# apache/arrow

Hardware: AMD Instinct MI355X
Metric: filter_take_mrows_per_s (higher is better)
Workload: dtype int64; 1 GPU; Filter+Take int64[1000000000] + validity (10% null), boolean mask 10% true, FilterOptions::DROP; take indices = the mask's row numbers (monotonic; indices_nonzero: uint64 through CallFunction, GetTakeIndices: uint32 in the mirror), no boundscheck; inputs = splitmix64 streams of SURVEY.md 8(d) (seeds 1,2,3); rows=1000000000, selected_rows=99992053, parallelism=single-gpu

## Files before the change

arrow_amd/_lib.py:

```python
from __future__ import annotations

import ctypes as C
import os

_HERE = os.path.dirname(os.path.abspath(__file__))
LIB_PATH = os.path.join(_HERE, "libarrow_amd.so")

ARX_OK = 0
ARX_OUT_OF_MEMORY = -1
ARX_INVALID = -4
ARX_CAPACITY_ERROR = -6
ARX_INDEX_ERROR = -7
ARX_NOT_IMPLEMENTED = -10
ARX_DEVICE_ERROR = -100

ABI_VERSION = 5

FILTER_DROP, FILTER_EMIT_NULL = 0, 1
JOIN_COLUMN, JOIN_LITERAL, JOIN_NULL = 0, 1, 2
JOIN_NULL_HANDLING = {"emit_null": 0, "skip": 1, "replace": 2}
JOIN_MAX_OPERANDS = 32
SORT_ASCENDING, SORT_DESCENDING = 0, 1
NULLS_AT_START, NULLS_AT_END = 0, 1


class ArrowAmdError(Exception):
    """Base class; subclasses mirror pyarrow.lib.ArrowInvalid & friends."""


class ArrowInvalid(ArrowAmdError, ValueError):
    pass


class ArrowIndexError(ArrowAmdError, IndexError):
    pass


class ArrowCapacityError(ArrowAmdError):
    pass


class ArrowNotImplementedError(ArrowAmdError, NotImplementedError):
    pass


class ArrowDeviceError(ArrowAmdError, RuntimeError):
    pass


class ArrowMemoryError(ArrowAmdError, MemoryError):
    pass


_ERRORS = {
    ARX_INVALID: ArrowInvalid,
    ARX_CAPACITY_ERROR: ArrowCapacityError,
    ARX_INDEX_ERROR: ArrowIndexError,
    ARX_NOT_IMPLEMENTED: ArrowNotImplementedError,
    ARX_DEVICE_ERROR: ArrowDeviceError,
    ARX_OUT_OF_MEMORY: ArrowMemoryError,
}


class ArxSpan(C.Structure):

    _fields_ = [
        ("validity", C.c_void_p),
        ("data", C.c_void_p),
        ("offset", C.c_int64),
        ("length", C.c_int64),
        ("null_count", C.c_int64),
    ]


class ArxSortKeyWindow(C.Structure):

    _fields_ = [("key_min", C.c_uint64), ("shift", C.c_int32), ("reserved", C.c_int32)]


class ArxRangePlan(C.Structure):

    _fields_ = [("key_min", C.c_int32), ("width", C.c_int32), ("partitions", C.c_int32), ("reserved", C.c_int32),
                ("slots", C.c_int64), ("state_bytes", C.c_uint64), ("workspace_bytes", C.c_uint64)]


class ArxBinarySpan(C.Structure):

    _fields_ = [
        ("validity", C.c_void_p),
        ("offsets", C.c_void_p),
        ("data", C.c_void_p),
        ("offset", C.c_int64),
        ("length", C.c_int64),
        ("null_count", C.c_int64),
    ]


class ArxJoinOperand(C.Structure):

    _fields_ = [
        ("kind", C.c_int32),
        ("reserved", C.c_int32),
        ("column", ArxBinarySpan),
        ("literal", C.c_void_p),
        ("literal_length", C.c_int64),
    ]


_p, _i64, _int, _u64, _u32, _sz = C.c_void_p, C.c_int64, C.c_int, C.c_uint64, C.c_uint32, C.c_size_t
_span = C.POINTER(ArxSpan)
_bspan = C.POINTER(ArxBinarySpan)

SIGNATURES = {
    "arx_last_error": (C.c_char_p, []),
    "arx_abi_version": (_int, []),
    "arx_device_count": (_int, []),
    "arx_set_option": (_int, [C.c_char_p, _i64]),
    "arx_get_option": (_int, [C.c_char_p, C.POINTER(_i64)]),
    "arx_get_counter": (_i64, [C.c_char_p]),
    "arx_filter_workspace_bytes": (_sz, [_i64]),
    "arx_filter_count": (_int, [_span, _int, _p, _sz, C.POINTER(_i64), _p]),
    "arx_filter_count_async": (_int, [_span, _int, _p, _sz, _p]),
    "arx_filter_count_nulls": (_int, [_span, _span, _int, _p, _sz, C.POINTER(_i64), C.POINTER(_i64), _p]),
    "arx_filter_exec": (_int, [_span, _int, _span, _int, _p, _i64, _p, _p, _p]),
    "arx_mask_to_indices": (_int, [_span, _int, _p, _i64, _int, _p, _p, _p]),
    "arx_filter_compact_form": (_int, [_int, _int, _int, _int, _i64, _i64]),
    "arx_take_workspace_bytes": (_sz, []),
    "arx_check_index_bounds": (_int, [_span, _int, _u64, _p, _sz, _p]),
    "arx_take": (_int, [_span, _int, _span, _int, _p, _p, _p, _p]),
    "arx_take_rows": (_int, [_span, _i64, _span, _int, _p, _p, _p, _p]),
    "arx_take_bits": (_int, [_span, _span, _int, _p, _p, _p, _p]),
    "arx_binary_take_workspace_bytes": (_sz, [_i64]),
    "arx_binary_take_offsets": (_int, [_bspan, _span, _int, _p, _sz, _p, _p, _p, C.POINTER(_i64), _p]),
    "arx_binary_take_data": (_int, [_bspan, _i64, _p, _sz, _p, _i64, _p, _p]),
    "arx_large_binary_take_workspace_bytes": (_sz, [_i64]),
    "arx_large_binary_take_offsets": (_int, [_bspan, _span, _int, _p, _sz, _p, _p, _p, C.POINTER(_i64), _p]),
    "arx_large_binary_take_data": (_int, [_bspan, _i64, _p, _sz, _p, _i64, _p, _p]),
    "arx_list_take_data": (_int, [_bspan, _int, _i64, _p, _sz, _p, _i64, _p, _p]),
    "arx_large_list_take_data": (_int, [_bspan, _int, _i64, _p, _sz, _p, _i64, _p, _p]),
    "arx_plain_byte_array_offsets": (_int, [_p, _sz, _i64, C.c_int32, _p]),
    "arx_rle_scan_runs": (_int, [_p, _sz, _int, _i64, _u32, _u64, _p, _i64, C.POINTER(_i64), C.POINTER(_i64)]),
    "arx_rle_decode_u32": (_int, [_p, _sz, _p, _i64, _int, _i64, _p, _p]),
    "arx_rle_decode_equals_bitmap": (_int, [_p, _sz, _p, _i64, _int, _i64, _u32, _p, _p]),
    "arx_expand_by_mask": (_int, [_p, _int, _span, _p, _p, _p]),
    "arx_rle_levels_to_bitmap": (_int, [_p, _p, _i64, _p, _p, _p, _p]),
    "arx_rle_scan_runs_equals": (_int, [_p, _sz, _int, _i64, _u32, _u32, _u64, _p, _i64, C.POINTER(_i64), C.POINTER(_i64)]),
    "arx_levels_to_list_workspace_bytes": (_sz, [_i64]),
    "arx_def_rep_levels_to_list": (_int, [_p, _p, _i64, _int, _int, _int, _i64, _p, _p, _p, _p, _sz, _p]),
    "arx_levels_ge_bitmap": (_int, [_p, _i64, _u32, _p, _p, _p]),
    "arx_lz4_decompress_streams": (_int, [_p, _p, _p, _i64, _p, _p, _p]),
    "arx_lz4_frame_scan": (_int, [_p, _sz, _u64, _p, _i64, C.POINTER(_i64), C.POINTER(_u64)]),
    "arx_bitmap_copy": (_int, [_p, _i64, _i64, _p, _p]),
    "arx_buffer_copy": (_int, [_p, _p, _i64, _p]),
    "arx_delta_scan_miniblocks": (_int, [_p, _sz, _u64, _p, _i64, C.POINTER(_i64), C.POINTER(_i64), C.POINTER(_i64),
                                         C.POINTER(_i64), C.POINTER(_sz)]),
    "arx_delta_decode_workspace_bytes": (_sz, [_i64]),
    "arx_delta_decode": (_int, [_p, _p, _i64, _i64, _i64, _i64, _int, _p, _sz, _p, _p]),
    "arx_lengths_to_offsets_i32": (_int, [_p, _i64, C.c_int32, _p, _p, _sz, _p]),
    "arx_byte_stream_split_decode": (_int, [_p, _i64, _int, _p, _p]),
    "arx_delta_byte_array_lengths": (_int, [_p, _p, _i64, _p, _i64, _p, _p, _p]),
    "arx_delta_byte_array_expand": (_int, [_p, _p, _p, _i64, _p, C.c_int32, _p, _p, _i64, _p, _p, _p]),
    "arx_bitmap_copy_at": (_int, [_p, _i64, _i64, _p, _i64, _p]),
    "arx_binary_rebase_offsets": (_int, [_p, _i64, C.c_int32, _p, _p]),
    "arx_bitmap_and": (_int, [_p, _i64, _p, _i64, _i64, _p, _p]),
    "arx_reduce_i64_init": (_int, [_p, _p]),
    "arx_reduce_i64_consume": (_int, [_span, _p, _p]),
    "arx_reduce_float_minmax": (_int, [_span, _int, _p, _p]),
    "arx_coalesce2": (_int, [_int, _span, _span, _p, _i64, _p, _p, _p]),
    "arx_sum_float_workspace_bytes": (_sz, [_i64, _i64]),
    "arx_sum_float": (_int, [_span, _int, _p, _sz, C.POINTER(C.c_double), C.POINTER(_i64), _p]),
    "arx_boolean_kleene": (_int, [_int, _span, _span, _p, _p, _p]),
    "arx_boolean_invert": (_int, [_p, _i64, _i64, _p, _p]),
    "arx_bitmap_popcount": (_int, [_p, _i64, _i64, _p, _sz, C.POINTER(_i64), _p]),
    "arx_bytes_to_bitmap": (_int, [_p, _i64, _p, _p, _p]),
    "arx_groupby_key_range_i32": (_int, [_span, _p, _p]),
    "arx_groupby_range_plan": (_int, [_i64, C.c_int32, C.c_int32, _p]),
    "arx_groupby_key_range_sampled_i32": (_int, [_span, _i64, _p, _p]),
    "arx_groupby_range_sum_i64_consume": (_int, [_p, _p, _span, _span, _p, _sz, _p]),
    "arx_groupby_range_merge": (_int, [_p, _p, C.c_int32, _i64, _int, _i64, _p]),
    "arx_groupby_range_finalize_workspace_bytes": (_sz, [_i64]),
    "arx_groupby_range_finalize": (_int, [_p, C.c_int32, C.c_int32, _i64, C.c_uint32, _p, _sz, _p, _p, _p, _p, _p, _p]),
    "arx_hash_bool_finalize": (_int, [_p, _p, _p, _i64, _int, _int, C.c_uint32, _p, _p, _p, _p]),
    "arx_sort_indices_workspace_bytes": (_sz, [_i64]),
    "arx_sort_partition_records_global": (_int, [_span, _int, _int, _int, _p, _p, _int, C.c_uint32, _p, _sz, _p, _p, _p]),
    "arx_sort_records": (_int, [_p, _i64, _p, _sz, _p, _p]),
    "arx_sort_indices": (_int, [_span, _int, _int, _int, _p, _sz, _p, _p]),
    "arx_rank_workspace_bytes": (_sz, [_i64]),
    "arx_rank": (_int, [_span, _int, _p, _int, _p, _sz, _p, _p]),
    "arx_sort_indices_64": (_int, [_span, _int, _int, _int, _p, _sz, _p, _p]),
    "arx_sort_key_histogram": (_int, [_span, _int, _int, _int, _p, _p]),
    "arx_sort_partition_by_bins": (_int, [_span, _int, _int, _int, _p, _int, _p, _sz, _p, _p, _p,
                                          C.POINTER(_i64), _p]),
    "arx_bitmap_to_indices": (_int, [_p, _i64, _i64, _int, _p, _sz, _p, C.POINTER(_i64), _p]),
    "arx_sort_partition_records": (_int, [_span, _int, _int, _int, _int, _p, _int, _p, _sz, _p, _p, C.POINTER(_i64), _p]),
    "arx_sort_key_range": (_int, [_span, _int, _int, _p, _p]),
    "arx_sort_key_histogram_window": (_int, [_span, _int, _int, _int, _p, _p, _p]),
    "arx_sort_key_range_sampled": (_int, [_span, _int, _int, _int, _p, _p]),
    "arx_sort_key_histogram_window_sampled": (_int, [_span, _int, _int, _int, _p, _int, _p, _p]),
    "arx_sort_partition_records_window": (_int, [_span, _int, _int, _int, _int, _p, _p, _int, _p, _sz, _p, _p,
                                                 C.POINTER(_i64), _p]),
    "arx_sort_unpack_records": (_int, [_p, _i64, _p, _int, _int, _p, _p, _p, _p]),
    "arx_groupby_export_partitioned": (_int, [_p, _int, _p, _sz, _p, _p, _p]),
    "arx_groupby_partials_capacity": (_i64, [_i64, _i64, _int]),
    "arx_groupby_sum_i64_consume_partials": (_int, [_p, _i64, _span, _span, _p, _sz, _int, _p, _i64, _p, _p]),
    "arx_groupby_partition_rows": (_int, [_span, _span, _int, _p, _sz, _p, _p, _p]),
    "arx_groupby_unpack_rows": (_int, [_p, _i64, _p, _p, _p, _p, _p]),
    "arx_hash_sum_consume_workspace_bytes": (_sz, [_i64, _i64]),
    "arx_hash_sum_i64_consume_ws": (_int, [_span, _int, _i64, _p, _i64, _i64, _p, _p, _p, _p, _sz, _p]),
    "arx_hash_mean_i64_finalize": (_int, [_p, _p, _i64, C.c_uint64, _p, _p, _p]),
    "arx_compare_numeric": (_int, [_int, _int, _p, _p, _p, _p, _i64, _p, _p]),
    "arx_arith_numeric": (_int, [_int, _int, _int, _p, _p, _p, _i64, _p, _p, _p, _i64, _i64, _p, _p, _p]),
    "arx_divide_numeric": (_int, [_int, _int, _p, _p, _p, _i64, _p, _p, _p, _i64, _i64, _p, _p, _p]),
    "arx_unary_numeric": (_int, [_int, _int, _int, _span, _p, _p, _p]),
    "arx_round_numeric": (_int, [_int, _int, _int, _span, _i64, _p, _p, _p, _p]),
    "arx_round_status": (_int, [_int, _int, _int, _span, _i64, _p, _p, _p]),
    "arx_delta_decode_pages": (_int, [_p, _p, _p, _i64, _i64, _int, _p, _sz, _p, _p]),
    "arx_copy_segments": (_int, [_p, _i64, _u64, _p]),
    "arx_bitmap_copy_segments": (_int, [_p, _i64, _i64, _p]),
    "arx_take_columns": (_int, [_p, _p, _int, _span, _int, _p, _p, _p, _p]),
    "arx_grouper_state_bytes": (_sz, [_i64]),
    "arx_grouper_init": (_int, [_p, _i64, _p]),
    "arx_grouper_consume_workspace_bytes": (_sz, [_i64]),
    "arx_grouper_consume": (_int, [_p, _i64, _p, _p, _int, _p, _sz, _p, _p]),
    "arx_grouper_lookup": (_int, [_p, _i64, _p, _p, _int, _p, _sz, _p, _p, _p]),
    "arx_grouper_num_groups": (_int, [_p, _p, _p]),
    "arx_group_ids_skip_group": (_int, [_p, _i64, _u32, _p]),
    "arx_grouper_get_uniques": (_int, [_p, _i64, _p, _int, _int, _p, _p, _p, _p]),
    "arx_binary_key_lengths": (_int, [_bspan, _p, _p, _p, _p]),
    "arx_binary_key_chunk": (_int, [_bspan, _i64, _p, _p, _p]),
    "arx_binary_sort_chunk": (_int, [_bspan, _i64, _p, _p]),
    "arx_binary_key_hash": (_int, [_bspan, _int, _p, _p]),
    "arx_set_lookup_state_bytes": (_sz, [_i64, _int]),
    "arx_set_lookup_build": (_int, [_p, _span, _int, _p]),
    "arx_set_lookup_build_binary": (_int, [_p, _bspan, _int, _int, _p]),
    "arx_set_lookup_is_in": (_int, [_p, _i64, _int, _span, _int, _p, _p]),
    "arx_set_lookup_index_in": (_int, [_p, _i64, _int, _span, _int, _p, _p, _p]),
    "arx_set_lookup_is_in_binary": (_int, [_p, _bspan, _int, _int, _bspan, _int, _int, _p, _p]),
    "arx_set_lookup_index_in_binary": (_int, [_p, _bspan, _int, _int, _bspan, _int, _int, _p, _p, _p]),
    "arx_match_substring": (_int, [_bspan, _int, _int, _p, _i64, _i64, _int, _p, _p]),
    "arx_string_length": (_int, [_bspan, _int, _int, _i64, _int, _p, _p]),
    "arx_string_slice_workspace_bytes": (_sz, [_i64, _int]),
    "arx_string_slice_offsets": (_int, [_bspan, _int, _int, _i64, _i64, _i64, _int, _p, _sz, _p, C.POINTER(_i64), _p]),
    "arx_string_slice_data": (_int, [_bspan, _int, _p, _sz, _p, _i64, _p, _p]),
    "arx_string_trim_offsets": (_int, [_bspan, _int, _int, _int, _p, _i64, _p, _sz, _p, C.POINTER(_i64), _p]),
    "arx_replace_substring_workspace_bytes": (_sz, [_i64, _int]),
    "arx_replace_substring_offsets": (_int, [_bspan, _int, _p, _i64, _i64, _i64, _i64, _int, _p, _sz, _p, C.POINTER(_i64), _p]),
    "arx_replace_substring_data": (_int, [_bspan, _int, _p, _i64, _p, _i64, _i64, _int, _p, _sz, _p, _i64, _p, _p]),
    "arx_binary_join_workspace_bytes": (_sz, [_i64, _int]),
    "arx_binary_join_offsets": (_int, [C.POINTER(ArxJoinOperand), _int, _i64, _int, _int, _i64, _p, _sz, _p, _p, C.POINTER(_i64),
                                       C.POINTER(_i64), _p]),
    "arx_binary_join_data": (_int, [C.POINTER(ArxJoinOperand), _int, _i64, _int, _int, _p, _i64, _p, _i64, _p, _p]),
    "arx_compare_binary": (_int, [_int, _bspan, _bspan, _int, _p, _i64, _i64, _int, _p, _p]),
    "arx_if_else": (_int, [_int, _span, _span, _p, _span, _p, _i64, _p, _p, _p]),
    "arx_temporal_component": (_int, [_int, _int, _span, _i64, _int, _int, _p, _p, _p]),
    "arx_hash_join_workspace_bytes": (_sz, [_i64]),
    "arx_hash_join_key_validity": (_int, [_span, _int, _i64, _p, _p]),
    "arx_hash_join_bool_key": (_int, [_span, _p, _p]),
    "arx_hash_join_group_offsets": (_int, [_p, _p, _i64, _i64, _p, _p, _sz, _p]),
    "arx_hash_join_probe_count": (_int, [_p, _p, _i64, _p, _i64, _int, _p, _i64, _p, _p, _sz, C.POINTER(_i64), _p]),
    "arx_hash_join_expand": (_int, [_p, _p, _p, _i64, _p, _p, _int, _i64, _p, _p, _p, _p]),
    "arx_hash_join_build_mask": (_int, [_p, _p, _i64, _p, _int, _p, _p]),
    "arx_hash_join_append_build_rows": (_int, [_p, _i64, _i64, _p, _p, _p, _p, _p]),
    "arx_hash_join_filter_count": (_int, [_span, _p, _p, _i64, _int, _p, _p, _i64, _p, _p, _p, _p, _sz, C.POINTER(_i64), _p]),
    "arx_hash_join_filter_compact": (_int, [_p, _p, _i64, _p, _p, _i64, _p, _p, _int, _i64, _p, _p, _p, _p]),
    "arx_hash_join_flags_to_mask": (_int, [_p, _i64, _int, _p, _p]),
    "arx_binary_key_verify": (_int, [_bspan, _p, _p, C.POINTER(_i64), _p, _p]),
    "arx_group_first_rows": (_int, [_p, _i64, _i64, _p, _p]),
    "arx_group_edge_rows": (_int, [_p, _p, _i64, _i64, _i64, _int, _p, _p, _p]),
    "arx_ree_bool_expand": (_int, [_p, _int, _i64, _span, _i64, _i64, _p, _p, _p]),
    "arx_snappy_decompress_pages": (_int, [_p, _p, _i64, _p, _p, _p]),
    "arx_gzip_decompress_pages": (_int, [_p, _p, _i64, _p, _p, _p]),
    "arx_cast_numeric": (_int, [_span, _int, _int, _int, _int, _p, _sz, _p, _p]),
    "arx_groupby_mean_i64_finalize": (_int, [_p, _p, _p, _p, _p, _i64, _int, _u32, _p, _p, _p, _p]),
    "arx_groupby_sum_i64_merge_records": (_int, [_p, _i64, _p, _i64, _p]),
    "arx_groupby_state_bytes": (_sz, [_i64]),
    "arx_groupby_init": (_int, [_p, _i64, _p]),
# ... 78 lines not shown
```

arrow_amd/csrc/plugin/common.inc:

```

std::atomic<int64_t> g_gpu_calls{0};
std::atomic<int64_t> g_stock_calls{0};
std::atomic<int64_t> g_min_rows{1 << 16};
std::atomic<int64_t> g_min_rows_streaming{INT64_MAX};
std::atomic<int64_t> g_filter_morsel_rows{[] {
  const char* env = std::getenv("ARROW_AMD_FILTER_MORSEL_ROWS");
  return env != nullptr ? static_cast<int64_t>(std::strtoll(env, nullptr, 10)) : int64_t(1) << 20;
}()};

std::atomic<bool> g_parquet_pinned_staging{true};
std::atomic<bool> g_parquet_device_levels{true};
std::atomic<int> g_parquet_read_threads{4};
std::atomic<int64_t> g_parquet_read_part_bytes{int64_t(1) << 23};
std::atomic<bool> g_parquet_device_snappy{[] {
  const char* env = std::getenv("ARROW_AMD_PARQUET_DEVICE_SNAPPY");
  return env == nullptr || std::strtoll(env, nullptr, 10) != 0;
}()};
std::atomic<int64_t> g_parquet_device_snappy_pages{0};
std::atomic<bool> g_parquet_device_gzip{true};
std::atomic<int64_t> g_parquet_device_gzip_pages{0};
std::atomic<int64_t> g_parquet_copied_pages{0};

std::atomic<int64_t> g_aggregate_flush_rows{[] {
  const char* env = std::getenv("ARROW_AMD_AGGREGATE_FLUSH_ROWS");
// ... 6 lines not shown
std::atomic<int64_t> g_aggregate_range_sample_rows{int64_t(1) << 20};
std::atomic<int64_t> g_aggregate_range_plans{0};
std::atomic<int64_t> g_aggregate_range_declined{0};
std::atomic<int64_t> g_select_k_min_rows{int64_t(1) << 22};
std::atomic<int64_t> g_select_k_threshold_runs{0};
std::atomic<bool> g_sharded_range_state{true};
std::atomic<int64_t> g_sharded_range_min_rows{int64_t(1) << 22};
std::atomic<int64_t> g_sharded_range_runs{0};
std::atomic<int64_t> g_sharded_range_declined{0};
std::atomic<bool> g_sharded_sort_records{true};
std::atomic<int> g_sharded_sort_sample_shift{4};
std::atomic<int64_t> g_sharded_sort_sample_min_rows{int64_t(1) << 20};
std::atomic<int64_t> g_sharded_sort_records_runs{0};
std::atomic<int64_t> g_coalesce_rows{int64_t(1) << 26};
std::atomic<int64_t> g_coalesced_batches{0};
std::atomic<int64_t> g_table_source_rows{int64_t(1) << 27};
std::atomic<bool> g_pinned_results{[] {
  const char* env = std::getenv("ARROW_AMD_PINNED_RESULTS");
  return env == nullptr || std::strtoll(env, nullptr, 10) != 0;
}()};
std::atomic<bool> g_results_kernel_copy{true};
std::atomic<bool> g_aggregate_device_output{false};
std::atomic<bool> g_aggregate_stage_nulls{true};
std::atomic<int64_t> g_aggregate_flushes{0};
std::atomic<int64_t> g_string_key_hash_bits{64};
std::atomic<int64_t> g_string_key_hash_collisions{0};

enum Fn { kFnFilter = 0, kFnTake, kFnGreater, kFnSort, kFnCast, kFnHashSum, kFnAdd, kFnBoolean, kFnCompare, kFnParquet,
          kFnReduce, kFnOrderBy, kFnTakeColumns, kFnUnique, kFnCoalesce, kFnIsIn, kFnIndexIn, kFnHashJoin,
          kFnMatchSubstring, kFnStartsWith, kFnEndsWith, kFnIfElse, kFnYear, kFnQuarter, kFnMonth, kFnDay, kFnDayOfWeek,
          kFnDayOfYear, kFnIsoYear, kFnIsoWeek, kFnHour, kFnMinute, kFnSecond, kFnMillisecond, kFnMicrosecond, kFnNanosecond,
          kFnBinaryLength, kFnUtf8Length, kFnBinarySlice, kFnUtf8SliceCodeunits, kFnAsciiTrimWhitespace, kFnAsciiLtrimWhitespace,
          kFnAsciiRtrimWhitespace, kFnUtf8TrimWhitespace, kFnUtf8LtrimWhitespace, kFnUtf8RtrimWhitespace, kFnAsciiTrim, kFnAsciiLtrim,
          kFnAsciiRtrim, kFnUtf8Trim, kFnUtf8Ltrim, kFnUtf8Rtrim, kFnCompareString, kFnReplaceSubstring, kFnUnaryArith, kFnRound,
          kFnBinaryJoinElementWise,
          kNumFn };
const char* const kFnNames[kNumFn] = {"array_filter", "array_take", "greater", "array_sort_indices",
                                      "cast", "hash_sum", "add", "boolean", "compare", "parquet", "reduce", "order_by",
                                      "take_columns", "unique", "coalesce", "is_in", "index_in", "hashjoin",
                                      "match_substring", "starts_with", "ends_with", "if_else", "year", "quarter", "month", "day",
                                      "day_of_week", "day_of_year", "iso_year", "iso_week", "hour", "minute", "second",
                                      "millisecond", "microsecond", "nanosecond", "binary_length", "utf8_length", "binary_slice",
                                      "utf8_slice_codeunits", "ascii_trim_whitespace", "ascii_ltrim_whitespace",
                                      "ascii_rtrim_whitespace", "utf8_trim_whitespace", "utf8_ltrim_whitespace",
                                      "utf8_rtrim_whitespace", "ascii_trim", "ascii_ltrim", "ascii_rtrim", "utf8_trim", "utf8_ltrim",
                                      "utf8_rtrim", "compare_string", "replace_substring", "unary_arith", "round",
                                      "binary_join_element_wise"};
std::atomic<int64_t> g_fn_gpu[kNumFn];
std::atomic<int64_t> g_fn_stock[kNumFn];
void CountGpu(Fn f) {
  g_gpu_calls.fetch_add(1, std::memory_order_relaxed);
  g_fn_gpu[f].fetch_add(1, std::memory_order_relaxed);
}
void CountStock(Fn f) {
  g_stock_calls.fetch_add(1, std::memory_order_relaxed);
  g_fn_stock[f].fetch_add(1, std::memory_order_relaxed);
}
thread_local std::string t_error;

Status FromArx(int rc) {
  if (rc == ARX_OK) return Status::OK();
  const std::string msg = arx_last_error();
  switch (rc) {
    case ARX_INVALID: return Status::Invalid(msg);
    case ARX_CAPACITY_ERROR: return Status::CapacityError(msg);
    case ARX_INDEX_ERROR: return Status::IndexError(msg);
    case ARX_NOT_IMPLEMENTED: return Status::NotImplemented(msg);
    case ARX_OUT_OF_MEMORY: return Status::OutOfMemory(msg);
    default: return Status::UnknownError(msg);
  }
}

#define HIP_RETURN_NOT_OK(call)                                                        \
  do {                                                                                 \
    hipError_t e__ = (call);                                                           \
    if (e__ != hipSuccess)                                                             \
      return Status::IOError("HIP: ", hipGetErrorString(e__), " in " #call);           \
  } while (0)

thread_local hipStream_t t_stream = nullptr;

class DeviceScratch {
 public:
  ~DeviceScratch() {
    for (auto& s : slots_) {
      if (s.ptr) (void)hipFree(s.ptr);
    }
  }
  hipStream_t PeekStream() const { return stream_; }
  Status Stream(hipStream_t* out) {
    if (!stream_) {
      HIP_RETURN_NOT_OK(hipStreamCreateWithFlags(&stream_, hipStreamNonBlocking));
      t_stream = stream_;
    }
    *out = stream_;
    return Status::OK();
  }
  Status Get(int slot, size_t bytes, void** out) {
    if (slots_.size() <= static_cast<size_t>(slot)) slots_.resize(slot + 1);
    Slot& s = slots_[slot];
    bytes = (bytes + 255) & ~size_t(255);
    if (s.size < bytes) {
      if (s.ptr) HIP_RETURN_NOT_OK(hipFree(s.ptr));
      s.ptr = nullptr;
      s.size = 0;
      const size_t want = std::max<size_t>(bytes + bytes / 4, 1 << 20);
      HIP_RETURN_NOT_OK(hipMalloc(&s.ptr, want));
      s.size = want;
    }
    *out = s.ptr;
    return Status::OK();
  }

 private:
  struct Slot { void* ptr = nullptr; size_t size = 0; };
  std::vector<Slot> slots_;
  hipStream_t stream_ = nullptr;
};
thread_local DeviceScratch t_scratch;

class PinnedStaging {
 public:
  ~PinnedStaging() {
    if (ptr_) (void)hipHostFree(ptr_);
  }
  Status Reserve(size_t bytes, uint8_t** out) {
    if (size_ < bytes) {
      if (ptr_) HIP_RETURN_NOT_OK(hipHostFree(ptr_));
      ptr_ = nullptr;
      size_ = 0;
      const size_t want = std::max<size_t>(bytes + bytes / 4, size_t(1) << 20);
      HIP_RETURN_NOT_OK(hipHostMalloc(&ptr_, want, hipHostMallocDefault));
      size_ = want;
    }
    *out = static_cast<uint8_t*>(ptr_);
    return Status::OK();
  }
  void Trim(size_t keep_at_most) {
    if (size_ > keep_at_most && ptr_ != nullptr) {
      (void)hipHostFree(ptr_);
      ptr_ = nullptr;
      size_ = 0;
    }
  }

 private:
  void* ptr_ = nullptr;
  size_t size_ = 0;
};
thread_local PinnedStaging t_pinned;

enum Slot { kValues = 0, kValidity, kArg2, kArg2Validity, kOutData, kOutValidity, kWs, kCounter, kBinWs, kFlag };

Status Upload(const ArraySpan& a, int byte_width_or_0_for_bool, int data_slot, int validity_slot,
              hipStream_t st, ArxSpan* out) {
  const int64_t o8 = a.offset % 8;
  const int64_t first = a.offset - o8;
  out->offset = o8;
  out->length = a.length;
  out->null_count = a.null_count;
  out->validity = nullptr;
  out->data = nullptr;
  const int64_t span_elems = o8 + a.length;
  if (a.buffers[1].data != nullptr && a.length > 0) {
    const uint8_t* src;
    size_t bytes;
    if (byte_width_or_0_for_bool == 0) {
      src = a.buffers[1].data + first / 8;
      bytes = static_cast<size_t>(arrow::bit_util::BytesForBits(span_elems));
    } else {
      src = a.buffers[1].data + first * byte_width_or_0_for_bool;
      bytes = static_cast<size_t>(span_elems) * byte_width_or_0_for_bool;
    }
    void* d = nullptr;
    ARROW_RETURN_NOT_OK(t_scratch.Get(data_slot, bytes + 16, &d));
    HIP_RETURN_NOT_OK(hipMemcpyAsync(d, src, bytes, hipMemcpyHostToDevice, st));
    out->data = d;
  }
  if (a.buffers[0].data != nullptr && a.null_count != 0 && a.length > 0) {
    const size_t bytes = static_cast<size_t>(arrow::bit_util::BytesForBits(span_elems));
    void* d = nullptr;
    ARROW_RETURN_NOT_OK(t_scratch.Get(validity_slot, bytes + 16, &d));
    HIP_RETURN_NOT_OK(hipMemcpyAsync(d, a.buffers[0].data + first / 8, bytes, hipMemcpyHostToDevice, st));
    out->validity = d;
  } else if (a.null_count != 0 && a.buffers[0].data == nullptr) {
    out->null_count = 0;
  }
  return Status::OK();
}

bool IsHost(const ArraySpan& a) {
  for (int i = 0; i < 2; ++i) {
    if (a.buffers[i].owner != nullptr && *a.buffers[i].owner != nullptr &&
        !(*a.buffers[i].owner)->is_cpu()) {
      return false;
    }
  }
  return true;
}

int FixedByteWidth(const arrow::DataType& t) {
  switch (t.id()) {
    case Type::INT8: case Type::UINT8: return 1;
    case Type::INT16: case Type::UINT16: case Type::HALF_FLOAT: return 2;
    case Type::INT32: case Type::UINT32: case Type::FLOAT: case Type::DATE32: case Type::TIME32:
    case Type::INTERVAL_MONTHS: case Type::DECIMAL32: return 4;
    case Type::INT64: case Type::UINT64: case Type::DOUBLE: case Type::DATE64: case Type::TIME64:
    case Type::TIMESTAMP: case Type::DURATION: case Type::INTERVAL_DAY_TIME: case Type::DECIMAL64: return 8;
    case Type::DECIMAL128: case Type::INTERVAL_MONTH_DAY_NANO: return 16;
    case Type::DECIMAL256: return 32;
    case Type::FIXED_SIZE_BINARY: {
      const int w = static_cast<const arrow::FixedSizeBinaryType&>(t).byte_width();
      return (w == 1 || w == 2 || w == 4 || w == 8 || w == 16 || w == 32) ? w : 0;
    }
    default: return 0;
  }
}

int BinaryOffsetWidth(Type::type id) { return (id == Type::LARGE_STRING || id == Type::LARGE_BINARY) ? 8 : 4; }

template <typename Options>
struct ShimState : public cp::KernelState {
  std::unique_ptr<cp::KernelState> stock;
  Options options;
};

struct StockKernel {
  cp::KernelInit init;
  cp::ArrayKernelExec exec = nullptr;
  cp::VectorKernel::ChunkedExec exec_chunked = nullptr;
};

template <class Exec, class Batch, class Out>
Status RunStock(Fn fn, Exec exec, std::optional<cp::KernelState*> stock_state, cp::KernelContext* ctx, const Batch& batch,
                Out* out) {
  CountStock(fn);
  if (!stock_state.has_value()) return exec(ctx, batch, out);
  cp::KernelState* mine = ctx->state();
  ctx->SetState(*stock_state);
  Status st = exec(ctx, batch, out);
  ctx->SetState(mine);
  return st;
}
Status RunStock(Fn fn, const StockKernel& k, cp::KernelState* stock_state, cp::KernelContext* ctx,
                const cp::ExecSpan& batch, cp::ExecResult* out) {
  return RunStock(fn, k.exec, std::optional<cp::KernelState*>(stock_state), ctx, batch, out);
}
```

arrow_amd/csrc/plugin/parquet.inc:

```

class RunTable {
 public:
  const ArxRleRun* data() const { return runs_.get(); }
  ArxRleRun* data() { return runs_.get(); }
  size_t size() const { return size_; }
  void clear() { size_ = 0; }
  void push_back(const ArxRleRun& r) {
    Reserve(size_ + 1);
    runs_[size_++] = r;
  }
  void Reserve(size_t n) {
    if (n <= cap_) return;
    const size_t cap = std::max(n, cap_ + cap_ / 2);
    std::unique_ptr<ArxRleRun[]> grown(new ArxRleRun[cap]);
    if (size_ > 0) std::memcpy(grown.get(), runs_.get(), size_ * sizeof(ArxRleRun));
    runs_ = std::move(grown);
    cap_ = cap;
  }
  void SetSize(size_t n) { size_ = n; }

 private:
  std::unique_ptr<ArxRleRun[]> runs_;
  size_t size_ = 0, cap_ = 0;
};
// ... 63 lines not shown
                      int64_t prefix_len, uint8_t* out) {
  if (prefix_len > 0) std::memcpy(out, prefix, static_cast<size_t>(prefix_len));
  ARROW_ASSIGN_OR_RAISE(const int64_t got, codec->Decompress(n, src, len, out + prefix_len));
  if (got != len) return Status::IOError("Corrupt snappy compressed data.");
  return Status::OK();
}

Status PrefetchBodies(const std::vector<std::shared_ptr<parquet::Page>>& pages, int max_def, PrefetchedBodies* out,
                      const uint8_t** arena_out, size_t* arena_bytes_out) {
  const arrow::Compression::type raw_codec = t_raw_codec;
  *arena_out = nullptr;
  *arena_bytes_out = 0;
  struct Job { const uint8_t* src; int64_t n, want, len; const uint8_t* prefix; int64_t prefix_len; size_t at; };
  std::vector<Job> jobs;
  size_t arena_bytes = 0;
  int64_t packed_bytes = 0;
  auto add = [&](const uint8_t* src, int64_t n, int64_t want, const uint8_t* prefix, int64_t prefix_len) {
    if (src == nullptr || n <= 0) return;
    PrefetchedBody& e = (*out)[src];
    e.src_len = n;
    e.want_len = want;
    e.prefix_len = prefix_len;
    auto len = SnappyBodyLength(src, n, want, raw_codec);
    if (!len.ok()) {
      e.status = len.status();
      return;
    }
    jobs.push_back(Job{src, n, want, *len, prefix, prefix_len, arena_bytes});
    arena_bytes += (static_cast<size_t>(prefix_len + *len) + 63) & ~size_t(63);
    packed_bytes += n;
  };
  for (const auto& page : pages) {
    if (page->type() == parquet::PageType::DICTIONARY_PAGE) {
      const auto& dp = static_cast<const parquet::DictionaryPage&>(*page);
      add(dp.data(), dp.size(), -1, nullptr, 0);
    } else if (page->type() == parquet::PageType::DATA_PAGE) {
      const auto& dp = static_cast<const parquet::DataPage&>(*page);
      if (!(max_def == 0 && dp.encoding() == parquet::Encoding::PLAIN)) add(dp.data(), dp.size(), dp.uncompressed_size(), nullptr, 0);
    } else if (page->type() == parquet::PageType::DATA_PAGE_V2) {
      const auto& v2 = static_cast<const parquet::DataPageV2&>(*page);
      const int64_t lev = static_cast<int64_t>(v2.definition_levels_byte_length()) + v2.repetition_levels_byte_length();
      if (lev < 0 || lev > v2.size() || lev > v2.uncompressed_size()) continue;
      if (v2.is_compressed() && v2.size() - lev > 0 && v2.encoding() != parquet::Encoding::PLAIN) {
        add(v2.data() + lev, v2.size() - lev, v2.uncompressed_size() - lev, v2.data(), lev);
      }
    }
  }
  if (jobs.empty()) return Status::OK();
  uint8_t* arena = nullptr;
  std::shared_ptr<std::vector<uint8_t>> pageable;
  if (g_parquet_pinned_staging.load()) {
    ARROW_RETURN_NOT_OK(t_pinned_bodies.Reserve(arena_bytes + 64, &arena));
  } else {
    thread_local std::vector<uint8_t> t_pageable_bodies;
    if (t_pageable_bodies.size() < arena_bytes + 64) t_pageable_bodies.resize(arena_bytes + arena_bytes / 4 + 64);
    arena = t_pageable_bodies.data();
  }
  const int threads = static_cast<int>(std::max<int64_t>(
      1, std::min<int64_t>({static_cast<int64_t>(g_parquet_read_threads.load()), static_cast<int64_t>(jobs.size()),
                            packed_bytes / std::max<int64_t>(1, g_parquet_read_part_bytes.load() / 8) + 1})));
  std::vector<Status> job_status(jobs.size());
  std::atomic<size_t> next{0};
  auto work = [&]() {
    auto codec = arrow::util::Codec::Create(raw_codec);
    for (size_t j = next.fetch_add(1); j < jobs.size(); j = next.fetch_add(1)) {
      const Job& job = jobs[j];
      job_status[j] = codec.ok() ? SnappyBodyInto(codec->get(), job.src, job.n, job.len, job.prefix, job.prefix_len, arena + job.at)
                                 : codec.status();
    }
  };
  std::vector<std::thread> helpers;
  for (int t = 1; t < threads; ++t) helpers.emplace_back(work);
  work();
  for (auto& t : helpers) t.join();
  *arena_out = arena;
  *arena_bytes_out = arena_bytes;
  for (size_t j = 0; j < jobs.size(); ++j) {
    PrefetchedBody& e = (*out)[jobs[j].src];
    e.status = job_status[j];
    e.body = HostBody{arena + jobs[j].at, jobs[j].prefix_len + jobs[j].len, pageable};
  }
  return Status::OK();
}

class UploadArena {
 public:
  ~UploadArena() {
    if (ptr_) (void)hipHostFree(ptr_);
  }
  struct Scope {
    explicit Scope(UploadArena* a) : arena(a) { arena->Begin(); }
    ~Scope() {
      if (hipStream_t st = t_scratch.PeekStream()) (void)hipStreamSynchronize(st);
      arena->active_ = false;
      t_pinned.Trim(size_t(1) << 30);
      t_pinned_bodies.Trim(size_t(1) << 30);
    }
    UploadArena* arena;
  };
  const void* Stage(const void* src, size_t nbytes) {
    if (!active_ || nbytes < (size_t(1) << 16)) return src;
    const size_t need = (nbytes + 63) & ~size_t(63);
    wanted_ += need;
    if (used_ + need > size_) return src;
    uint8_t* dst = static_cast<uint8_t*>(ptr_) + used_;
    std::memcpy(dst, src, nbytes);
    used_ += need;
    return dst;
  }

 private:
  void Begin() {
    if (wanted_ > size_ && g_parquet_pinned_staging.load()) {
      if (ptr_) (void)hipHostFree(ptr_);
      ptr_ = nullptr;
      size_ = 0;
      const size_t want = wanted_ + wanted_ / 4;
      if (hipHostMalloc(&ptr_, want, hipHostMallocDefault) == hipSuccess) size_ = want; else ptr_ = nullptr;
    }
    used_ = 0;
    wanted_ = 0;
    active_ = g_parquet_pinned_staging.load();
  }
  void* ptr_ = nullptr;
  size_t size_ = 0, used_ = 0, wanted_ = size_t(8) << 20;
  bool active_ = false;
};
thread_local UploadArena t_upload;

arrow::Result<std::shared_ptr<Buffer>> ToDevice(const void* host, size_t nbytes, hipStream_t st) {
  ARROW_ASSIGN_OR_RAISE(auto buf, AllocDevice(static_cast<int64_t>(nbytes)));
  if (nbytes > 0) {
    HIP_RETURN_NOT_OK(hipMemcpyAsync(reinterpret_cast<void*>(buf->mutable_address()), t_upload.Stage(host, nbytes), nbytes,
                                     hipMemcpyHostToDevice, st));
  }
  return buf;
}

Status ParquetValidity(const ParquetStream& levels, int max_def, int64_t rows, int64_t dense, hipStream_t st,
                       std::shared_ptr<Buffer>* validity, ArxSpan* mask, void** ws, std::shared_ptr<Buffer> keep[2]) {
  ARROW_ASSIGN_OR_RAISE(keep[0], ToDevice(levels.bytes.data(), levels.bytes.size(), st));
  ARROW_ASSIGN_OR_RAISE(keep[1], ToDevice(levels.runs.data(), levels.runs.size() * sizeof(ArxRleRun), st));
  ARROW_ASSIGN_OR_RAISE(*validity, AllocDevice(((rows + 63) / 64) * 8));
  void* d_valid = reinterpret_cast<void*>((*validity)->mutable_address());
  ARROW_RETURN_NOT_OK(FromArx(arx_rle_decode_equals_bitmap(reinterpret_cast<const void*>(keep[0]->address()),
                                                           levels.bytes.size(),
                                                           reinterpret_cast<const ArxRleRun*>(keep[1]->address()),
                                                           static_cast<int64_t>(levels.runs.size()), 1, rows,
                                                           static_cast<uint32_t>(max_def), d_valid, st)));
  *mask = ArxSpan{nullptr, d_valid, 0, rows, 0};
  const size_t ws_bytes = arx_filter_workspace_bytes(rows);
  ARROW_RETURN_NOT_OK(t_scratch.Get(kBinWs, ws_bytes, ws));
  int64_t counted = 0;
  ARROW_RETURN_NOT_OK(FromArx(arx_filter_count(mask, ARX_FILTER_DROP, *ws, ws_bytes, &counted, st)));
  if (counted != dense) return Status::Invalid("Parquet: ", counted, " non-null levels but ", dense, " values");
  return Status::OK();
}

struct ByteArrayPage {
  std::vector<uint8_t> bytes;
  int64_t count;
  bool delta_length;
  bool delta_byte_array = false;
};

Status DecodeInt32DeltaStreams(const std::vector<const uint8_t*>& bytes, const std::vector<size_t>& sizes,
                               const std::vector<int64_t>& expect, const char* what, int32_t* d_out, std::vector<size_t>* used,
                               hipStream_t st) {
  std::vector<uint8_t> all;
  std::vector<ArxDeltaMiniblock> mbs;
  std::vector<ArxDeltaPage> table(bytes.size());
  used->assign(bytes.size(), 0);
  int64_t start = 0, tiles = 0;
  for (size_t j = 0; j < bytes.size(); ++j) {
    int64_t nmb = 0, vpm = 0, total = 0, first_value = 0;
    size_t u = 0;
    ARROW_RETURN_NOT_OK(FromArx(arx_delta_scan_miniblocks(bytes[j], sizes[j], all.size(), nullptr, 0, &nmb, &vpm, &total, &first_value, &u)));
    if (total != expect[j]) return Status::Invalid("Parquet: DELTA_BYTE_ARRAY page holds ", total, " ", what, ", its header says ", expect[j]);
    const size_t at = mbs.size();
    mbs.resize(at + static_cast<size_t>(nmb));
    ARROW_RETURN_NOT_OK(FromArx(arx_delta_scan_miniblocks(bytes[j], sizes[j], all.size(), mbs.data() + at, nmb, &nmb, &vpm, &total,
                                                          &first_value, nullptr)));
    table[j] = ArxDeltaPage{start, static_cast<int64_t>(at), std::max<int64_t>(vpm, 1), first_value, total, tiles};
    all.insert(all.end(), bytes[j], bytes[j] + u);
    all.resize((all.size() + 7) & ~size_t(7), 0);
    (*used)[j] = u;
    start += total;
    tiles += (total + 4095) / 4096;
  }
  if (start == 0) return Status::OK();
  all.resize(all.size() + 16, 0);
  if (mbs.empty()) mbs.push_back(ArxDeltaMiniblock{});
  ARROW_ASSIGN_OR_RAISE(auto d_all, ToDevice(all.data(), all.size(), st));
  ARROW_ASSIGN_OR_RAISE(auto d_mbs, ToDevice(mbs.data(), mbs.size() * sizeof(ArxDeltaMiniblock), st));
  ARROW_ASSIGN_OR_RAISE(auto d_table, ToDevice(table.data(), table.size() * sizeof(ArxDeltaPage), st));
  const size_t ws_bytes = arx_delta_decode_workspace_bytes(std::max<int64_t>(tiles, 1) * 4096);
  void* ws = nullptr;
  ARROW_RETURN_NOT_OK(t_scratch.Get(kWs, ws_bytes, &ws));
  ARROW_RETURN_NOT_OK(FromArx(arx_delta_decode_pages(reinterpret_cast<const void*>(d_all->address()),
                                                     reinterpret_cast<const ArxDeltaMiniblock*>(d_mbs->address()),
                                                     reinterpret_cast<const ArxDeltaPage*>(d_table->address()),
                                                     static_cast<int64_t>(table.size()), tiles, 4, ws, ws_bytes, d_out, st)));
  HIP_RETURN_NOT_OK(hipStreamSynchronize(st));
  return Status::OK();
}

arrow::Result<std::shared_ptr<ArrayData>> ParquetBitsOrBytesToDevice(
    const std::shared_ptr<arrow::DataType>& type, bool is_bool, int max_def, int64_t rows, int64_t dense,
    int64_t dense_from_dict, const std::vector<uint8_t>& dict, int64_t dict_count, const ParquetStream& levels,
    const ParquetStream& indices, const ParquetStream& bools,
    const std::vector<ByteArrayPage>& plain_ba, hipStream_t st) {
  std::shared_ptr<Buffer> keep[12];
  std::vector<std::shared_ptr<Buffer>> keep_more;
  std::vector<uint32_t> page_entries;
  ArxSpan bool_src{};
  ArxBinarySpan bin_src{};
  if (is_bool) {
    ARROW_ASSIGN_OR_RAISE(keep[0], AllocDevice(((std::max<int64_t>(dense, 1) + 63) / 64) * 8));
    if (dense > 0) {
      ARROW_ASSIGN_OR_RAISE(keep[1], ToDevice(bools.bytes.data(), bools.bytes.size(), st));
      ARROW_ASSIGN_OR_RAISE(keep[2], ToDevice(bools.runs.data(), bools.runs.size() * sizeof(ArxRleRun), st));
      ARROW_RETURN_NOT_OK(FromArx(arx_rle_decode_equals_bitmap(
          reinterpret_cast<const void*>(keep[1]->address()), bools.bytes.size(),
          reinterpret_cast<const ArxRleRun*>(keep[2]->address()), static_cast<int64_t>(bools.runs.size()), 1, dense, 1u,
          reinterpret_cast<void*>(keep[0]->mutable_address()), st)));
    }
    bool_src = ArxSpan{nullptr, reinterpret_cast<const void*>(keep[0]->address()), 0, dense, 0};
  } else {
    std::vector<int32_t> offs(1, 0);
    std::vector<uint8_t> data;
    size_t pos = 0;
    for (int64_t i = 0; i < dict_count; ++i) {
      if (pos + 4 > dict.size()) return Status::Invalid("Parquet: byte-array dictionary entry runs past the page");
      const uint32_t len = arrow::util::SafeLoadAs<uint32_t>(dict.data() + pos);
      if (len > dict.size() - pos - 4) return Status::Invalid("Parquet: byte-array dictionary entry runs past the page");
      data.insert(data.end(), dict.begin() + pos + 4, dict.begin() + pos + 4 + len);
      pos += 4 + len;
      offs.push_back(static_cast<int32_t>(data.size()));
    }
    struct DeltaLengthFixup { size_t entry; int32_t base; const ByteArrayPage* page; size_t header_bytes; };
    std::vector<DeltaLengthFixup> fixups;
    std::vector<const ByteArrayPage*> dba_pages;
    int64_t dba_total = 0;
    constexpr uint32_t kDbaMark = 0x80000000u;
    for (const auto& page : plain_ba) {
      const int32_t base = static_cast<int32_t>(data.size());
      const size_t first = offs.size() - 1;
      if (page.delta_byte_array) {
        if (page.count == 0) continue;
        for (int64_t j = 0; j < page.count; ++j) page_entries.push_back(kDbaMark | static_cast<uint32_t>(dba_total + j));
        dba_pages.push_back(&page);
        dba_total += page.count;
        continue;
      }
      if (!page.delta_length) {
        offs.resize(first + 2 * page.count + 1);
        ARROW_RETURN_NOT_OK(FromArx(arx_plain_byte_array_offsets(page.bytes.data(), page.bytes.size(), page.count, base,
                                                                 offs.data() + first)));
        data.insert(data.end(), page.bytes.begin(), page.bytes.begin() + (offs.back() - base));
        for (int64_t j = 0; j < page.count; ++j) page_entries.push_back(static_cast<uint32_t>(first + 1 + 2 * j));
        continue;
      }
      if (page.count == 0) continue;
      int64_t nmb = 0, vpm = 0, total = 0, first_value = 0;
      size_t header_bytes = 0;
      ARROW_RETURN_NOT_OK(FromArx(arx_delta_scan_miniblocks(page.bytes.data(), page.bytes.size(), 0, nullptr, 0, &nmb, &vpm,
                                                            &total, &first_value, &header_bytes)));
      if (total != page.count) {
        return Status::Invalid("Parquet: DELTA_LENGTH_BYTE_ARRAY page holds ", total, " lengths, its header says ", page.count);
      }
      if (data.size() + (page.bytes.size() - header_bytes) > static_cast<size_t>(INT32_MAX)) {
        return Status::Invalid("Parquet: column chunk exceeds the int32 offset range");
      }
      fixups.push_back(DeltaLengthFixup{first, base, &page, header_bytes});
      offs.resize(first + page.count + 1, 0);
      data.insert(data.end(), page.bytes.begin() + header_bytes, page.bytes.end());
      offs.back() = static_cast<int32_t>(data.size());
      for (int64_t j = 0; j < page.count; ++j) page_entries.push_back(static_cast<uint32_t>(first + j));
    }
    const size_t host_entries = offs.size() - 1;
    if (dba_total > 0) {
      if (host_entries + static_cast<size_t>(dba_total) >= kDbaMark) return Status::Invalid("Parquet: too many byte-array values in one chunk");
      for (auto& e : page_entries) {
        if (e & kDbaMark) e = static_cast<uint32_t>(host_entries) + (e & ~kDbaMark);
      }
      offs.resize(host_entries + dba_total + 1, static_cast<int32_t>(data.size()));
    }
    ARROW_ASSIGN_OR_RAISE(keep[0], ToDevice(offs.data(), offs.size() * 4, st));
    if (dba_total == 0) {
      ARROW_ASSIGN_OR_RAISE(keep[1], ToDevice(data.data(), data.size(), st));
    } else {
      const int64_t npages = static_cast<int64_t>(dba_pages.size());
      ARROW_ASSIGN_OR_RAISE(auto d_prefix, AllocDevice(dba_total * 4));
      ARROW_ASSIGN_OR_RAISE(auto d_slen, AllocDevice(dba_total * 4));
      std::vector<int64_t> firsts(1, 0), suffix_firsts(1, 0);
      std::vector<uint8_t> suffix;
      {
        std::vector<const uint8_t*> heads, rests;
        std::vector<size_t> head_sizes, rest_sizes, used, sused;
        std::vector<int64_t> counts;
        for (const ByteArrayPage* page : dba_pages) {
          heads.push_back(page->bytes.data());
          head_sizes.push_back(page->bytes.size());
          counts.push_back(page->count);
        }
        ARROW_RETURN_NOT_OK(DecodeInt32DeltaStreams(heads, head_sizes, counts, "prefix lengths",
                                                    reinterpret_cast<int32_t*>(d_prefix->mutable_address()), &used, st));
// ... 609 lines not shown
                  std::to_string(prefetch_misses) + " | ";
  }
  std::shared_ptr<Buffer> dense_buf = dense_early;
  if (!raw) {
    ARROW_ASSIGN_OR_RAISE(dense_buf, AllocDevice(dense * width));
  }
  if (raw && dense > cc->num_values()) return Status::Invalid("Parquet: more values in the pages than the chunk announces");
  uint8_t* d_dense = reinterpret_cast<uint8_t*>(dense_buf->mutable_address());
  std::shared_ptr<Buffer> keep[8];
  std::shared_ptr<Buffer> keep_snappy[3];
  std::shared_ptr<Buffer> keep_segs;
  if (!plain_segs.empty()) {
    ARROW_ASSIGN_OR_RAISE(keep_segs, ToDevice(plain_segs.data(), plain_segs.size() * sizeof(ArxCopySeg), st));
    ARROW_RETURN_NOT_OK(FromArx(arx_copy_segments(reinterpret_cast<const ArxCopySeg*>(keep_segs->address()),
                                                  static_cast<int64_t>(plain_segs.size()), plain_seg_max, st)));
  }
  if (!snappy_pages.empty()) {
    if (raw_plain_values != dense - dense_from_dict || !delta_pages.empty() || !split_pages.empty()) {
      return Status::NotImplemented("arrow_amd: PLAIN and DELTA_BINARY_PACKED / BYTE_STREAM_SPLIT pages in one column chunk");
    }
    std::memset(snappy_src + snappy_len, 0, 8);
    if (chunk_dev) {
      keep_snappy[0] = chunk_dev;
      if (snappy_len > chunk_bytes + 8) {
        HIP_RETURN_NOT_OK(hipMemcpyAsync(reinterpret_cast<uint8_t*>(chunk_dev->mutable_address()) + chunk_bytes + 8,
                                         snappy_src + chunk_bytes + 8, snappy_len - chunk_bytes, hipMemcpyHostToDevice, st));
      }
    } else {
      ARROW_ASSIGN_OR_RAISE(keep_snappy[0], ToDevice(snappy_src, snappy_len + 8, st));
    }
    ARROW_ASSIGN_OR_RAISE(keep_snappy[1], ToDevice(snappy_pages.data(), snappy_pages.size() * sizeof(ArxSnappyPage), st));
    ARROW_ASSIGN_OR_RAISE(keep_snappy[2], AllocDevice(static_cast<int64_t>(snappy_pages.size()) * 4));
    ARROW_RETURN_NOT_OK(FromArx((gzip_chunk ? arx_gzip_decompress_pages : arx_snappy_decompress_pages)(
        reinterpret_cast<const void*>(keep_snappy[0]->address()), reinterpret_cast<const ArxSnappyPage*>(keep_snappy[1]->address()),
        static_cast<int64_t>(snappy_pages.size()), d_dense, reinterpret_cast<uint32_t*>(keep_snappy[2]->mutable_address()), st)));
    std::vector<uint32_t> status(snappy_pages.size());
    HIP_RETURN_NOT_OK(hipMemcpyAsync(status.data(), reinterpret_cast<const void*>(keep_snappy[2]->address()), status.size() * 4,
                                     hipMemcpyDeviceToHost, st));
    HIP_RETURN_NOT_OK(hipStreamSynchronize(st));
    for (uint32_t code : status) {
      if (code != 0 && gzip_chunk) {
        return Status::IOError("zlib inflate failed: invalid deflate stream (device decoder status ", code, ")");
      }
      if (code != 0) return Status::IOError("Corrupt snappy compressed data.");
    }
    (gzip_chunk ? g_parquet_device_gzip_pages : g_parquet_device_snappy_pages).fetch_add(static_cast<int64_t>(snappy_pages.size()));
  }
  if (dense_from_dict > 0) {
    ARROW_ASSIGN_OR_RAISE(keep[0], ToDevice(indices.bytes.data(), indices.bytes.size(), st));
    ARROW_ASSIGN_OR_RAISE(keep[1], ToDevice(indices.runs.data(), indices.runs.size() * sizeof(ArxRleRun), st));
    ARROW_ASSIGN_OR_RAISE(keep[2], ToDevice(dict.data(), static_cast<size_t>(dict_count) * width, st));
    ARROW_ASSIGN_OR_RAISE(keep[3], AllocDevice(dense_from_dict * 4));
    uint32_t* d_idx = reinterpret_cast<uint32_t*>(keep[3]->mutable_address());
    ARROW_RETURN_NOT_OK(FromArx(arx_rle_decode_u32(reinterpret_cast<const void*>(keep[0]->address()), indices.bytes.size(),
                                                   reinterpret_cast<const ArxRleRun*>(keep[1]->address()),
                                                   static_cast<int64_t>(indices.runs.size()), 0, dense_from_dict, d_idx, st)));
    ArxSpan dv{nullptr, reinterpret_cast<const void*>(keep[2]->address()), 0, dict_count, 0};
    ArxSpan di{nullptr, d_idx, 0, dense_from_dict, 0};
    void* bws = nullptr;
    ARROW_RETURN_NOT_OK(t_scratch.Get(kWs, arx_take_workspace_bytes(), &bws));
    ARROW_RETURN_NOT_OK(FromArx(arx_check_index_bounds(&di, ARX_UINT32, static_cast<uint64_t>(dict_count), bws,
                                                       arx_take_workspace_bytes(), st)));
    ARROW_RETURN_NOT_OK(FromArx(arx_take(&dv, width, &di, ARX_UINT32, d_dense, nullptr, nullptr, st)));
  }
  std::shared_ptr<Buffer> keep_split;
  if (!split_pages.empty()) {
    ARROW_ASSIGN_OR_RAISE(keep_split, ToDevice(split_bytes.data(), split_bytes.size(), st));
    for (const auto& sp : split_pages) {
      ARROW_RETURN_NOT_OK(FromArx(arx_byte_stream_split_decode(
          reinterpret_cast<const uint8_t*>(keep_split->address()) + sp.byte_start, sp.count, width,
          d_dense + sp.dense_start * width, st)));
    }
  }
  if (!plain.empty()) {
    if (!delta_pages.empty() || !split_pages.empty()) {
      return Status::NotImplemented("arrow_amd: PLAIN and DELTA_BINARY_PACKED / BYTE_STREAM_SPLIT pages in one column chunk");
    }
    HIP_RETURN_NOT_OK(hipMemcpyAsync(d_dense + dense_from_dict * width, plain.data(), plain.size(), hipMemcpyHostToDevice, st));
  }
  if (!delta_pages.empty()) {
    delta_bytes.resize(delta_bytes.size() + 16, 0);
    if (delta_mbs.empty()) delta_mbs.push_back(ArxDeltaMiniblock{});
    ARROW_ASSIGN_OR_RAISE(keep[6], ToDevice(delta_bytes.data(), delta_bytes.size(), st));
    ARROW_ASSIGN_OR_RAISE(keep[7], ToDevice(delta_mbs.data(), delta_mbs.size() * sizeof(ArxDeltaMiniblock), st));
    std::vector<ArxDeltaPage> table(delta_pages.size());
    int64_t tiles = 0;
    for (size_t j = 0; j < delta_pages.size(); ++j) {
      const auto& dp = delta_pages[j];
      table[j] = ArxDeltaPage{dp.dense_start, dp.first_mb, std::max<int64_t>(dp.per_miniblock, 1), dp.first_value, dp.count, tiles};
      tiles += (dp.count + 4095) / 4096;
    }
    std::shared_ptr<Buffer> keep_pages;
    ARROW_ASSIGN_OR_RAISE(keep_pages, ToDevice(table.data(), table.size() * sizeof(ArxDeltaPage), st));
    const size_t ws_bytes = arx_delta_decode_workspace_bytes(std::max<int64_t>(tiles, 1) * 4096);
    void* ws = nullptr;
    ARROW_RETURN_NOT_OK(t_scratch.Get(kWs, ws_bytes, &ws));
    ARROW_RETURN_NOT_OK(FromArx(arx_delta_decode_pages(
        reinterpret_cast<const void*>(keep[6]->address()), reinterpret_cast<const ArxDeltaMiniblock*>(keep[7]->address()),
        reinterpret_cast<const ArxDeltaPage*>(keep_pages->address()), static_cast<int64_t>(table.size()), tiles, width, ws,
        ws_bytes, d_dense, st)));
    HIP_RETURN_NOT_OK(hipStreamSynchronize(st));
  }
  std::shared_ptr<Buffer> validity, values = dense_buf;
  int64_t null_count = 0;
  if (levels_on_device && !level_pages.empty()) {
    if (!chunk_dev) {
      ARROW_ASSIGN_OR_RAISE(chunk_dev, AllocDevice(static_cast<int64_t>(chunk_bytes) + 8));
      HIP_RETURN_NOT_OK(hipMemcpyAsync(reinterpret_cast<void*>(chunk_dev->mutable_address()), snappy_src, chunk_bytes + 8,
                                       hipMemcpyHostToDevice, st));
    }
    const size_t np = level_pages.size();
    ARROW_ASSIGN_OR_RAISE(validity, AllocDevice(((rows + 63) / 64) * 8 + 8));
    HIP_RETURN_NOT_OK(hipMemsetAsync(reinterpret_cast<void*>(validity->mutable_address()), 0,
                                     static_cast<size_t>((rows + 63) / 64) * 8 + 8, st));
    ARROW_ASSIGN_OR_RAISE(keep[4], ToDevice(level_pages.data(), np * sizeof(ArxLevelPage), st));
    ARROW_ASSIGN_OR_RAISE(keep[5], AllocDevice(static_cast<int64_t>(np) * 8));
    uint32_t* d_ones = reinterpret_cast<uint32_t*>(keep[5]->mutable_address());
    ARROW_RETURN_NOT_OK(FromArx(arx_rle_levels_to_bitmap(reinterpret_cast<const void*>(chunk_dev->address()),
                                                         reinterpret_cast<const ArxLevelPage*>(keep[4]->address()),
                                                         static_cast<int64_t>(np),
                                                         reinterpret_cast<void*>(validity->mutable_address()), d_ones,
                                                         d_ones + np, st)));
    std::vector<uint32_t> back(2 * np);
    HIP_RETURN_NOT_OK(hipMemcpyAsync(back.data(), d_ones, 2 * np * 4, hipMemcpyDeviceToHost, st));
    HIP_RETURN_NOT_OK(hipStreamSynchronize(st));
    for (size_t i = 0; i < np; ++i) {
      if (back[np + i] != 0) return Status::Invalid("Parquet: RLE block ended before all its values (corrupt data page?)");
      if (back[i] != level_valid[i]) {
        return Status::Invalid("Parquet: ", back[i], " non-null levels in a page whose header announces ", level_valid[i]);
      }
    }
    if (dense == rows) validity = nullptr;
  }
  if (max_def > 0 && dense < rows) {
    void* d_valid = nullptr;
    if (levels_on_device) {
      d_valid = reinterpret_cast<void*>(validity->mutable_address());
    } else {
      ARROW_ASSIGN_OR_RAISE(keep[4], ToDevice(levels.bytes.data(), levels.bytes.size(), st));
      ARROW_ASSIGN_OR_RAISE(keep[5], ToDevice(levels.runs.data(), levels.runs.size() * sizeof(ArxRleRun), st));
      ARROW_ASSIGN_OR_RAISE(validity, AllocDevice(((rows + 63) / 64) * 8));
      d_valid = reinterpret_cast<void*>(validity->mutable_address());
      ARROW_RETURN_NOT_OK(FromArx(arx_rle_decode_equals_bitmap(reinterpret_cast<const void*>(keep[4]->address()),
                                                               levels.bytes.size(),
                                                               reinterpret_cast<const ArxRleRun*>(keep[5]->address()),
                                                               static_cast<int64_t>(levels.runs.size()), 1, rows,
                                                               static_cast<uint32_t>(max_def), d_valid, st)));
    }
    ArxSpan mask{nullptr, d_valid, 0, rows, 0};
    const size_t ws_bytes = arx_filter_workspace_bytes(rows);
    void* ws = nullptr;
    ARROW_RETURN_NOT_OK(t_scratch.Get(kBinWs, ws_bytes, &ws));
    int64_t counted = 0;
    ARROW_RETURN_NOT_OK(FromArx(arx_filter_count(&mask, ARX_FILTER_DROP, ws, ws_bytes, &counted, st)));
    if (counted != dense) return Status::Invalid("Parquet: ", counted, " non-null levels but ", dense, " values");
    ARROW_ASSIGN_OR_RAISE(values, AllocDevice(rows * width));
    ARROW_RETURN_NOT_OK(FromArx(arx_expand_by_mask(d_dense, width, &mask, ws,
                                                   reinterpret_cast<void*>(values->mutable_address()), st)));
    null_count = rows - dense;
  }
  HIP_RETURN_NOT_OK(hipStreamSynchronize(st));
  trace.Lap("uploads + device decode");
  CountGpu(kFnParquet);
  return ArrayData::Make(std::move(type), rows, {std::move(validity), std::move(values)}, null_count);
}
```

arrow_amd/csrc/plugin/selection.inc:

```
StockKernel g_stock_filter;

arrow::Result<std::unique_ptr<cp::KernelState>> FilterInit(cp::KernelContext* ctx,
                                                           const cp::KernelInitArgs& args) {
  auto state = std::make_unique<ShimState<cp::FilterOptions>>();
  if (g_stock_filter.init) {
    ARROW_ASSIGN_OR_RAISE(state->stock, g_stock_filter.init(ctx, args));
  }
  if (args.options != nullptr) {
    state->options = *static_cast<const cp::FilterOptions*>(args.options);
  }
  return state;
}

Status BooleanTakeOnDevice(const ArxSpan& dv, const ArxSpan& di, int tid, hipStream_t st, ArrayData* out_arr) {
  const int64_t m = di.length;
  const int64_t bytes = ((m + 63) / 64) * 8;
  const bool allocate_validity = dv.null_count != 0 || di.null_count != 0;
  out_arr->length = m;
  out_arr->buffers.resize(2);
  out_arr->buffers[0] = nullptr;
  ARROW_ASSIGN_OR_RAISE(out_arr->buffers[1], AllocDevice(bytes));
  void* d_valid = nullptr;
  void* d_counter = nullptr;
  if (allocate_validity) {
    ARROW_ASSIGN_OR_RAISE(out_arr->buffers[0], AllocDevice(bytes));
    d_valid = reinterpret_cast<void*>(out_arr->buffers[0]->mutable_address());
    ARROW_RETURN_NOT_OK(t_scratch.Get(kCounter, 64, &d_counter));
    HIP_RETURN_NOT_OK(hipMemsetAsync(d_counter, 0, 8, st));
  }
  ARROW_RETURN_NOT_OK(FromArx(arx_take_bits(&dv, &di, tid, reinterpret_cast<void*>(out_arr->buffers[1]->mutable_address()),
                                            d_valid, static_cast<int64_t*>(d_counter), st)));
  int64_t valid_count = m;
  if (allocate_validity) HIP_RETURN_NOT_OK(hipMemcpyAsync(&valid_count, d_counter, 8, hipMemcpyDeviceToHost, st));
  HIP_RETURN_NOT_OK(hipStreamSynchronize(st));
  out_arr->null_count = m - valid_count;
  return Status::OK();
}

bool ReeFilterOnRocm(const ArraySpan& filter) {
  return filter.type->id() == Type::RUN_END_ENCODED && filter.child_data.size() == 2 &&
         OnRocm(filter.child_data[0]) && OnRocm(filter.child_data[1]);
}
Status ExpandReeFilterOnDevice(const ArraySpan& filter, hipStream_t st, ArxSpan* dm) {
  const ArraySpan& run_ends = filter.child_data[0];
  const ArraySpan& run_values = filter.child_data[1];
  const int rw = FixedByteWidth(*run_ends.type);
  if (run_values.type->id() != Type::BOOL || (rw != 2 && rw != 4 && rw != 8)) {
    return Status::NotImplemented("arrow_amd: filter of type ", filter.type->ToString());
  }
  ArxSpan ends{}, vals{};
  ARROW_RETURN_NOT_OK(DeviceSpan(run_ends, &ends));
  ARROW_RETURN_NOT_OK(DeviceSpan(run_values, &vals));
  const int64_t n = filter.length;
  const size_t bytes = static_cast<size_t>((n + 63) / 64) * 8 + 64;
  void *d_bits = nullptr, *d_valid = nullptr;
  ARROW_RETURN_NOT_OK(t_scratch.Get(kArg2, bytes, &d_bits));
  const bool may_have_nulls = vals.validity != nullptr && vals.null_count != 0;
  if (may_have_nulls) ARROW_RETURN_NOT_OK(t_scratch.Get(kArg2Validity, bytes, &d_valid));
  ARROW_RETURN_NOT_OK(FromArx(arx_ree_bool_expand(static_cast<const uint8_t*>(ends.data) + ends.offset * rw, rw, run_ends.length,
                                                  &vals, filter.offset, n, d_bits, d_valid, st)));
  *dm = ArxSpan{d_valid, d_bits, 0, n, may_have_nulls ? arrow::kUnknownNullCount : 0};
  return Status::OK();
}

Status FilterExec(cp::KernelContext* ctx, const cp::ExecSpan& batch, cp::ExecResult* out) {
  auto* state = static_cast<ShimState<cp::FilterOptions>*>(ctx->state());
  const ArraySpan& values = batch[0].array;
  const ArraySpan& filter = batch[1].array;
  const int w = FixedByteWidth(*values.type);
  const int null_sel = state->options.null_selection_behavior == cp::FilterOptions::EMIT_NULL
                           ? ARX_FILTER_EMIT_NULL : ARX_FILTER_DROP;
  const bool ree = filter.type->id() == Type::RUN_END_ENCODED;
  const bool on_device = OnRocm(values) || OnRocm(filter) || (ree && ReeFilterOnRocm(filter));
  if (on_device && ree && (!OnRocm(values) || !ReeFilterOnRocm(filter))) {
    return Status::NotImplemented("arrow_amd: a run-end encoded filter and its values must both be device-resident");
  }
  if (on_device) {
    if (values.type->id() == Type::BOOL && ree) {
      return Status::NotImplemented("arrow_amd: run-end encoded filter of boolean values on device-resident arrays");
    }
    if (values.type->id() == Type::BOOL && filter.type->id() == Type::BOOL) {
      if (filter.length > 0xFFFFFFFFll) {
        return Status::NotImplemented("Filter length exceeds UINT32_MAX, consider a different strategy for selecting elements");
      }
      hipStream_t st;
      ARROW_RETURN_NOT_OK(t_scratch.Stream(&st));
      ArxSpan dv{}, dm{};
      ARROW_RETURN_NOT_OK(DeviceSpan(values, &dv));
      ARROW_RETURN_NOT_OK(DeviceSpan(filter, &dm));
      const size_t ws_bytes = arx_filter_workspace_bytes(filter.length);
      void* ws = nullptr;
      ARROW_RETURN_NOT_OK(t_scratch.Get(kWs, ws_bytes, &ws));
      int64_t out_len = 0;
      ARROW_RETURN_NOT_OK(FromArx(arx_filter_count(&dm, null_sel, ws, ws_bytes, &out_len, st)));
      const bool emit = null_sel == ARX_FILTER_EMIT_NULL && dm.null_count != 0;
      void* d_idx = nullptr;
      void* d_idx_valid = nullptr;
      ARROW_RETURN_NOT_OK(t_scratch.Get(kArg2, static_cast<size_t>(out_len) * 4 + 64, &d_idx));
      if (emit) ARROW_RETURN_NOT_OK(t_scratch.Get(kArg2Validity, static_cast<size_t>((out_len + 63) / 64) * 8 + 64, &d_idx_valid));
      ARROW_RETURN_NOT_OK(FromArx(arx_mask_to_indices(&dm, null_sel, ws, out_len, 4, d_idx, d_idx_valid, st)));
      ArxSpan di{d_idx_valid, d_idx, 0, out_len, emit ? arrow::kUnknownNullCount : 0};
      ARROW_RETURN_NOT_OK(BooleanTakeOnDevice(dv, di, ARX_UINT32, st, out->array_data().get()));
      CountGpu(kFnFilter);
      return Status::OK();
    }
    if (w == 0 || (filter.type->id() != Type::BOOL && !ree)) {
      return Status::NotImplemented("arrow_amd: filter of ", values.type->ToString(),
                                    " on device-resident arrays");
    }
    hipStream_t st;
    ARROW_RETURN_NOT_OK(t_scratch.Stream(&st));
    ArxSpan dv{}, dm{};
    ARROW_RETURN_NOT_OK(DeviceSpan(values, &dv));
    if (ree) {
      ARROW_RETURN_NOT_OK(ExpandReeFilterOnDevice(filter, st, &dm));
    } else {
      ARROW_RETURN_NOT_OK(DeviceSpan(filter, &dm));
    }
    const size_t ws_bytes = arx_filter_workspace_bytes(filter.length);
    void* ws = nullptr;
    ARROW_RETURN_NOT_OK(t_scratch.Get(kWs, ws_bytes, &ws));
    ArrayData* out_arr = out->array_data().get();
    const bool allocate_validity = dv.null_count != 0 || dm.null_count != 0;
    if (filter.length > 0 && filter.length <= g_filter_morsel_rows.load()) {
      const int64_t n = filter.length;
      ARROW_RETURN_NOT_OK(FromArx(arx_filter_count_async(&dm, null_sel, ws, ws_bytes, st)));
      out_arr->buffers.resize(2);
      ARROW_ASSIGN_OR_RAISE(out_arr->buffers[1], AllocDevice(n * w));
      out_arr->buffers[0] = nullptr;
      void* d_valid = nullptr;
      if (allocate_validity) {
        ARROW_ASSIGN_OR_RAISE(out_arr->buffers[0], AllocDevice(((n + 63) / 64) * 8));
        d_valid = reinterpret_cast<void*>(out_arr->buffers[0]->mutable_address());
      }
      ARROW_RETURN_NOT_OK(FromArx(arx_filter_exec(&dv, w, &dm, null_sel, ws, n,
                                                  reinterpret_cast<void*>(out_arr->buffers[1]->mutable_address()),
                                                  d_valid, st)));
      int64_t selected = 0, set_bits = 0;
      HIP_RETURN_NOT_OK(hipMemcpyAsync(&selected, ws, 8, hipMemcpyDeviceToHost, st));
      if (allocate_validity) {
        void* cws = nullptr;
        ARROW_RETURN_NOT_OK(t_scratch.Get(kCounter, 64, &cws));
        ARROW_RETURN_NOT_OK(FromArx(arx_bitmap_popcount(d_valid, 0, n, cws, 64, &set_bits, st)));
      } else {
        HIP_RETURN_NOT_OK(hipStreamSynchronize(st));
      }
      out_arr->length = selected;
      out_arr->null_count = allocate_validity ? selected - set_bits : 0;
      static_cast<RocmBuffer*>(out_arr->buffers[1].get())->Shrink(selected * w);
      if (allocate_validity) static_cast<RocmBuffer*>(out_arr->buffers[0].get())->Shrink(((selected + 63) / 64) * 8);
      CountGpu(kFnFilter);
      return Status::OK();
    }
    int64_t out_len = 0, out_nulls = 0;
    if (allocate_validity) {
      ARROW_RETURN_NOT_OK(FromArx(arx_filter_count_nulls(&dv, &dm, null_sel, ws, ws_bytes, &out_len, &out_nulls, st)));
    } else {
      ARROW_RETURN_NOT_OK(FromArx(arx_filter_count(&dm, null_sel, ws, ws_bytes, &out_len, st)));
    }
    out_arr->length = out_len;
    out_arr->buffers.resize(2);
    ARROW_ASSIGN_OR_RAISE(out_arr->buffers[1], AllocDevice(out_len * w));
    out_arr->buffers[0] = nullptr;
    void* d_valid = nullptr;
    if (allocate_validity) {
      ARROW_ASSIGN_OR_RAISE(out_arr->buffers[0], AllocDevice(((out_len + 63) / 64) * 8));
      d_valid = reinterpret_cast<void*>(out_arr->buffers[0]->mutable_address());
    }
    ARROW_RETURN_NOT_OK(FromArx(arx_filter_exec(&dv, w, &dm, null_sel, ws, out_len,
                                                reinterpret_cast<void*>(out_arr->buffers[1]->mutable_address()),
                                                d_valid, st)));
    out_arr->null_count = allocate_validity ? out_nulls : 0;
    HIP_RETURN_NOT_OK(hipStreamSynchronize(st));
    CountGpu(kFnFilter);
    return Status::OK();
  }
  if (w == 0 || filter.type->id() != Type::BOOL || values.length < g_min_rows.load() ||
      !IsHost(values) || !IsHost(filter)) {
    return RunStock(kFnFilter, g_stock_filter, state->stock.get(), ctx, batch, out);
  }
  hipStream_t st;
  ARROW_RETURN_NOT_OK(t_scratch.Stream(&st));
  ArxSpan dv{}, dm{};
  ARROW_RETURN_NOT_OK(Upload(values, w, kValues, kValidity, st, &dv));
  ARROW_RETURN_NOT_OK(Upload(filter, 0, kArg2, kArg2Validity, st, &dm));
  const size_t ws_bytes = arx_filter_workspace_bytes(filter.length);
  void* ws = nullptr;
  ARROW_RETURN_NOT_OK(t_scratch.Get(kWs, ws_bytes, &ws));
  int64_t out_len = 0;
  ARROW_RETURN_NOT_OK(FromArx(arx_filter_count(&dm, null_sel, ws, ws_bytes, &out_len, st)));

  ArrayData* out_arr = out->array_data().get();
  const bool filter_null_count_is_zero = filter.null_count == 0;
  if (values.null_count == 0 && (null_sel == ARX_FILTER_DROP || filter_null_count_is_zero)) {
    out_arr->null_count = 0;
  } else {
    out_arr->null_count = arrow::kUnknownNullCount;
  }
  const bool allocate_validity = values.null_count != 0 || !filter_null_count_is_zero;
  out_arr->length = out_len;
  out_arr->buffers.resize(2);
  ARROW_ASSIGN_OR_RAISE(out_arr->buffers[1], ctx->Allocate(out_len * w));
  void* d_out = nullptr;
  void* d_out_valid = nullptr;
  ARROW_RETURN_NOT_OK(t_scratch.Get(kOutData, static_cast<size_t>(out_len) * w + 16, &d_out));
  const size_t vbytes = static_cast<size_t>((out_len + 63) / 64) * 8;
  if (allocate_validity) {
    ARROW_ASSIGN_OR_RAISE(out_arr->buffers[0], ctx->AllocateBitmap(out_len));
    ARROW_RETURN_NOT_OK(t_scratch.Get(kOutValidity, vbytes + 16, &d_out_valid));
  } else {
    out_arr->buffers[0] = nullptr;
  }
  ARROW_RETURN_NOT_OK(FromArx(arx_filter_exec(&dv, w, &dm, null_sel, ws, out_len, d_out, d_out_valid, st)));
  if (out_len > 0) {
    HIP_RETURN_NOT_OK(hipMemcpyAsync(out_arr->buffers[1]->mutable_data(), d_out,
                                     static_cast<size_t>(out_len) * w, hipMemcpyDeviceToHost, st));
    if (allocate_validity) {
      HIP_RETURN_NOT_OK(hipMemcpyAsync(out_arr->buffers[0]->mutable_data(), d_out_valid,
                                       static_cast<size_t>(arrow::bit_util::BytesForBits(out_len)),
                                       hipMemcpyDeviceToHost, st));
    }
  }
  HIP_RETURN_NOT_OK(hipStreamSynchronize(st));
  CountGpu(kFnFilter);
  return Status::OK();
}

int IndexTypeId(const arrow::DataType& t);

StockKernel g_stock_filter_bin, g_stock_take_bin, g_stock_filter_large_bin, g_stock_take_large_bin;

arrow::Result<std::unique_ptr<cp::KernelState>> BinaryFilterInit(cp::KernelContext* ctx,
                                                                 const cp::KernelInitArgs& args) {
  auto state = std::make_unique<ShimState<cp::FilterOptions>>();
  const bool large_in = !args.inputs.empty() && args.inputs[0].type != nullptr && BinaryOffsetWidth(args.inputs[0].type->id()) == 8;
  const StockKernel& stock_k = large_in ? g_stock_filter_large_bin : g_stock_filter_bin;
  if (stock_k.init) {
    ARROW_ASSIGN_OR_RAISE(state->stock, stock_k.init(ctx, args));
  }
  if (args.options != nullptr) state->options = *static_cast<const cp::FilterOptions*>(args.options);
  return state;
}

arrow::Result<std::unique_ptr<cp::KernelState>> BinaryTakeInit(cp::KernelContext* ctx,
                                                               const cp::KernelInitArgs& args) {
  auto state = std::make_unique<ShimState<cp::TakeOptions>>();
  const bool large_in = !args.inputs.empty() && args.inputs[0].type != nullptr && BinaryOffsetWidth(args.inputs[0].type->id()) == 8;
  const StockKernel& stock_k = large_in ? g_stock_take_large_bin : g_stock_take_bin;
  if (stock_k.init) {
    ARROW_ASSIGN_OR_RAISE(state->stock, stock_k.init(ctx, args));
  }
  if (args.options != nullptr) state->options = *static_cast<const cp::TakeOptions*>(args.options);
  return state;
}

Status CheckBoundsOnDevice(const ArxSpan& indices, int index_type, int64_t values_length, hipStream_t st) {
  void* ws = nullptr;
  ARROW_RETURN_NOT_OK(t_scratch.Get(kWs, arx_take_workspace_bytes(), &ws));
  return FromArx(arx_check_index_bounds(&indices, index_type, static_cast<uint64_t>(values_length), ws,
                                        arx_take_workspace_bytes(), st));
}

bool OnRocm3(const ArraySpan& a) {
  if (OnRocm(a)) return true;
  return a.buffers[2].owner != nullptr && *a.buffers[2].owner != nullptr &&
         (*a.buffers[2].owner)->device_type() == arrow::DeviceAllocationType::kROCM;
}

Status DeviceBinarySpan(const ArraySpan& a, ArxBinarySpan* out) {
  const void* addr[3] = {nullptr, nullptr, nullptr};
  for (int i = 0; i < 3; ++i) {
    const auto* owner = a.buffers[i].owner;
    if (owner == nullptr || *owner == nullptr) continue;
    if ((*owner)->device_type() != arrow::DeviceAllocationType::kROCM) {
      return Status::Invalid("arrow_amd: mixed host / device buffers in one array");
    }
    addr[i] = reinterpret_cast<const void*>((*owner)->address());
  }
  out->validity = addr[0];
  out->offsets = static_cast<const int32_t*>(addr[1]);
  out->data = addr[2];
  out->offset = a.offset;
  out->length = a.length;
  out->null_count = addr[0] == nullptr ? 0 : (a.null_count > 0 ? a.null_count : arrow::kUnknownNullCount);
  return Status::OK();
}

Status BinaryTakeOnDevice(const ArxBinarySpan& dv, const ArxSpan& di, int tid, hipStream_t st, ArrayData* out_arr, bool large = false) {
  const int64_t m = di.length;
  const bool allocate_validity = dv.null_count != 0 || di.null_count != 0;
  out_arr->length = m;
  out_arr->buffers.resize(3);
  out_arr->buffers[0] = nullptr;
  ARROW_ASSIGN_OR_RAISE(out_arr->buffers[1], AllocDevice((m + 1) * (large ? 8 : 4)));
  void* d_valid = nullptr;
  void* d_counter = nullptr;
  if (allocate_validity) {
    ARROW_ASSIGN_OR_RAISE(out_arr->buffers[0], AllocDevice(((m + 63) / 64) * 8));
    d_valid = reinterpret_cast<void*>(out_arr->buffers[0]->mutable_address());
    ARROW_RETURN_NOT_OK(t_scratch.Get(kCounter, 64, &d_counter));
    HIP_RETURN_NOT_OK(hipMemsetAsync(d_counter, 0, 8, st));
  }
  const size_t ws_bytes = large ? arx_large_binary_take_workspace_bytes(m) : arx_binary_take_workspace_bytes(m);
  void* ws = nullptr;
  ARROW_RETURN_NOT_OK(t_scratch.Get(kBinWs, ws_bytes, &ws));
  void* d_off = reinterpret_cast<void*>(out_arr->buffers[1]->mutable_address());
  int64_t total = 0;
  if (large) {
    ARROW_RETURN_NOT_OK(FromArx(arx_large_binary_take_offsets(&dv, &di, tid, ws, ws_bytes, static_cast<int64_t*>(d_off), d_valid,
                                                              static_cast<int64_t*>(d_counter), &total, st)));
  } else {
    ARROW_RETURN_NOT_OK(FromArx(arx_binary_take_offsets(&dv, &di, tid, ws, ws_bytes, static_cast<int32_t*>(d_off), d_valid,
                                                        static_cast<int64_t*>(d_counter), &total, st)));
  }
  ARROW_ASSIGN_OR_RAISE(out_arr->buffers[2], AllocDevice(total));
  void* d_data = reinterpret_cast<void*>(out_arr->buffers[2]->mutable_address());
  if (large) {
    ARROW_RETURN_NOT_OK(FromArx(arx_large_binary_take_data(&dv, m, ws, ws_bytes, static_cast<const int64_t*>(d_off), total, d_data, st)));
  } else {
    ARROW_RETURN_NOT_OK(FromArx(arx_binary_take_data(&dv, m, ws, ws_bytes, static_cast<const int32_t*>(d_off), total, d_data, st)));
  }
  int64_t valid_count = m;
  if (allocate_validity) {
    HIP_RETURN_NOT_OK(hipMemcpyAsync(&valid_count, d_counter, 8, hipMemcpyDeviceToHost, st));
  }
  HIP_RETURN_NOT_OK(hipStreamSynchronize(st));
  out_arr->null_count = m - valid_count;
  return Status::OK();
}

bool IsInt32Binary(const arrow::DataType& t) { return t.id() == Type::STRING || t.id() == Type::BINARY; }

Status BinaryTakeExec(cp::KernelContext* ctx, const cp::ExecSpan& batch, cp::ExecResult* out) {
  auto* state = static_cast<ShimState<cp::TakeOptions>*>(ctx->state());
  const ArraySpan& values = batch[0].array;
  const ArraySpan& indices = batch[1].array;
  if (!OnRocm3(values) && !OnRocm(indices)) {
    return RunStock(kFnTake, BinaryOffsetWidth(values.type->id()) == 8 ? g_stock_take_large_bin : g_stock_take_bin, state->stock.get(), ctx, batch, out);
  }
  const int tid = IndexTypeId(*indices.type);
  const bool large = BinaryOffsetWidth(values.type->id()) == 8;
  if (tid < 0 || !(IsInt32Binary(*values.type) || large)) {
    return Status::NotImplemented("arrow_amd: take of ", values.type->ToString(), " by ",
                                  indices.type->ToString(), " on device-resident arrays");
  }
  hipStream_t st;
  ARROW_RETURN_NOT_OK(t_scratch.Stream(&st));
  ArxBinarySpan dv{};
  ArxSpan di{};
  ARROW_RETURN_NOT_OK(DeviceBinarySpan(values, &dv));
  ARROW_RETURN_NOT_OK(DeviceSpan(indices, &di));
  if (state->options.boundscheck) ARROW_RETURN_NOT_OK(CheckBoundsOnDevice(di, tid, values.length, st));
  ARROW_RETURN_NOT_OK(BinaryTakeOnDevice(dv, di, tid, st, out->array_data().get(), large));
  CountGpu(kFnTake);
  return Status::OK();
}

Status BinaryFilterExec(cp::KernelContext* ctx, const cp::ExecSpan& batch, cp::ExecResult* out) {
  auto* state = static_cast<ShimState<cp::FilterOptions>*>(ctx->state());
  const ArraySpan& values = batch[0].array;
  const ArraySpan& filter = batch[1].array;
  if (!OnRocm3(values) && !OnRocm(filter)) {
    return RunStock(kFnFilter, BinaryOffsetWidth(values.type->id()) == 8 ? g_stock_filter_large_bin : g_stock_filter_bin, state->stock.get(), ctx, batch, out);
  }
  const bool large = BinaryOffsetWidth(values.type->id()) == 8;
  if (filter.type->id() != Type::BOOL || !(IsInt32Binary(*values.type) || large)) {
    return Status::NotImplemented("arrow_amd: filter of ", values.type->ToString(), " on device-resident arrays");
  }
  if (filter.length > 0xFFFFFFFFll) {
    return Status::NotImplemented("Filter length exceeds UINT32_MAX, consider a different strategy for selecting elements");
  }
  const int null_sel = state->options.null_selection_behavior == cp::FilterOptions::EMIT_NULL
                           ? ARX_FILTER_EMIT_NULL : ARX_FILTER_DROP;
  hipStream_t st;
  ARROW_RETURN_NOT_OK(t_scratch.Stream(&st));
  ArxBinarySpan dv{};
  ArxSpan dm{};
  ARROW_RETURN_NOT_OK(DeviceBinarySpan(values, &dv));
  ARROW_RETURN_NOT_OK(DeviceSpan(filter, &dm));
  const size_t ws_bytes = arx_filter_workspace_bytes(filter.length);
  void* ws = nullptr;
  ARROW_RETURN_NOT_OK(t_scratch.Get(kWs, ws_bytes, &ws));
  int64_t out_len = 0;
  ARROW_RETURN_NOT_OK(FromArx(arx_filter_count(&dm, null_sel, ws, ws_bytes, &out_len, st)));
  const bool emit = null_sel == ARX_FILTER_EMIT_NULL && dm.null_count != 0;
  void* d_idx = nullptr;
  void* d_idx_valid = nullptr;
  ARROW_RETURN_NOT_OK(t_scratch.Get(kArg2, static_cast<size_t>(out_len) * 4 + 64, &d_idx));
  if (emit) ARROW_RETURN_NOT_OK(t_scratch.Get(kArg2Validity, static_cast<size_t>((out_len + 63) / 64) * 8 + 64, &d_idx_valid));
  ARROW_RETURN_NOT_OK(FromArx(arx_mask_to_indices(&dm, null_sel, ws, out_len, 4, d_idx, d_idx_valid, st)));
  ArxSpan di{d_idx_valid, d_idx, 0, out_len, emit ? arrow::kUnknownNullCount : 0};
  ARROW_RETURN_NOT_OK(BinaryTakeOnDevice(dv, di, ARX_UINT32, st, out->array_data().get(), large));
  CountGpu(kFnFilter);
  return Status::OK();
}

StockKernel g_stock_take;

arrow::Result<std::unique_ptr<cp::KernelState>> TakeInit(cp::KernelContext* ctx,
                                                         const cp::KernelInitArgs& args) {
  auto state = std::make_unique<ShimState<cp::TakeOptions>>();
  if (g_stock_take.init) {
    ARROW_ASSIGN_OR_RAISE(state->stock, g_stock_take.init(ctx, args));
  }
  if (args.options != nullptr) state->options = *static_cast<const cp::TakeOptions*>(args.options);
  return state;
}

int IndexTypeId(const arrow::DataType& t) {
  switch (t.id()) {
    case Type::UINT8: return ARX_UINT8;
    case Type::INT8: return ARX_INT8;
    case Type::UINT16: return ARX_UINT16;
    case Type::INT16: return ARX_INT16;
    case Type::UINT32: return ARX_UINT32;
    case Type::INT32: return ARX_INT32;
    case Type::UINT64: return ARX_UINT64;
    case Type::INT64: return ARX_INT64;
    default: return -1;
  }
}

Status TakeExec(cp::KernelContext* ctx, const cp::ExecSpan& batch, cp::ExecResult* out) {
  auto* state = static_cast<ShimState<cp::TakeOptions>*>(ctx->state());
  const ArraySpan& values = batch[0].array;
  const ArraySpan& indices = batch[1].array;
  const int w = FixedByteWidth(*values.type);
  const int tid = IndexTypeId(*indices.type);
  static const int kIdxWidth[8] = {1, 1, 2, 2, 4, 4, 8, 8};
  if (OnRocm(values) || OnRocm(indices)) {
    if (values.type->id() == Type::BOOL && tid >= 0) {
      hipStream_t st;
      ARROW_RETURN_NOT_OK(t_scratch.Stream(&st));
      ArxSpan dv{}, di{};
      ARROW_RETURN_NOT_OK(DeviceSpan(values, &dv));
      ARROW_RETURN_NOT_OK(DeviceSpan(indices, &di));
      if (state->options.boundscheck) ARROW_RETURN_NOT_OK(CheckBoundsOnDevice(di, tid, values.length, st));
      ARROW_RETURN_NOT_OK(BooleanTakeOnDevice(dv, di, tid, st, out->array_data().get()));
      CountGpu(kFnTake);
      return Status::OK();
    }
    if (w == 0 || tid < 0) {
      return Status::NotImplemented("arrow_amd: take of ", values.type->ToString(), " by ",
                                    indices.type->ToString(), " on device-resident arrays");
    }
    hipStream_t st;
    ARROW_RETURN_NOT_OK(t_scratch.Stream(&st));
    ArxSpan dv{}, di{};
    ARROW_RETURN_NOT_OK(DeviceSpan(values, &dv));
    ARROW_RETURN_NOT_OK(DeviceSpan(indices, &di));
    if (state->options.boundscheck) ARROW_RETURN_NOT_OK(CheckBoundsOnDevice(di, tid, values.length, st));
    const int64_t m = indices.length;
    const bool allocate_validity = dv.null_count != 0 || di.null_count != 0;
    ArrayData* out_arr = out->array_data().get();
    out_arr->length = m;
    out_arr->buffers.resize(2);
    ARROW_ASSIGN_OR_RAISE(out_arr->buffers[1], AllocDevice(m * w));
    out_arr->buffers[0] = nullptr;
    void* d_valid = nullptr;
    void* d_counter = nullptr;
    if (allocate_validity) {
      ARROW_ASSIGN_OR_RAISE(out_arr->buffers[0], AllocDevice(((m + 63) / 64) * 8));
      d_valid = reinterpret_cast<void*>(out_arr->buffers[0]->mutable_address());
      ARROW_RETURN_NOT_OK(t_scratch.Get(kCounter, 64, &d_counter));
      HIP_RETURN_NOT_OK(hipMemsetAsync(d_counter, 0, 8, st));
    }
    ARROW_RETURN_NOT_OK(FromArx(arx_take(&dv, w, &di, tid,
                                         reinterpret_cast<void*>(out_arr->buffers[1]->mutable_address()), d_valid,
                                         static_cast<int64_t*>(d_counter), st)));
    int64_t valid_count = m;
    if (allocate_validity) {
      HIP_RETURN_NOT_OK(hipMemcpyAsync(&valid_count, d_counter, 8, hipMemcpyDeviceToHost, st));
    }
    HIP_RETURN_NOT_OK(hipStreamSynchronize(st));
    out_arr->null_count = m - valid_count;
    CountGpu(kFnTake);
    return Status::OK();
  }
  if (w == 0 || tid < 0 || indices.length < g_min_rows.load() || !IsHost(values) || !IsHost(indices)) {
    return RunStock(kFnTake, g_stock_take, state->stock.get(), ctx, batch, out);
  }
  hipStream_t st;
  ARROW_RETURN_NOT_OK(t_scratch.Stream(&st));
  ArxSpan dv{}, di{};
  ARROW_RETURN_NOT_OK(Upload(values, w, kValues, kValidity, st, &dv));
  ARROW_RETURN_NOT_OK(Upload(indices, kIdxWidth[tid], kArg2, kArg2Validity, st, &di));
  if (state->options.boundscheck) ARROW_RETURN_NOT_OK(CheckBoundsOnDevice(di, tid, values.length, st));
  const int64_t m = indices.length;
  const bool allocate_validity = values.MayHaveNulls() || indices.MayHaveNulls();
  ArrayData* out_arr = out->array_data().get();
  out_arr->length = m;
  out_arr->buffers.resize(2);
  ARROW_ASSIGN_OR_RAISE(out_arr->buffers[1], ctx->Allocate(m * w));
  void* d_out = nullptr;
  void* d_out_valid = nullptr;
  void* d_counter = nullptr;
  ARROW_RETURN_NOT_OK(t_scratch.Get(kOutData, static_cast<size_t>(m) * w + 16, &d_out));
  if (allocate_validity) {
    ARROW_ASSIGN_OR_RAISE(out_arr->buffers[0], ctx->AllocateBitmap(m));
    ARROW_RETURN_NOT_OK(t_scratch.Get(kOutValidity, static_cast<size_t>((m + 63) / 64) * 8 + 16, &d_out_valid));
    ARROW_RETURN_NOT_OK(t_scratch.Get(kCounter, 64, &d_counter));
    HIP_RETURN_NOT_OK(hipMemsetAsync(d_counter, 0, 8, st));
  } else {
    out_arr->buffers[0] = nullptr;
  }
  ARROW_RETURN_NOT_OK(FromArx(arx_take(&dv, w, &di, tid, d_out, d_out_valid,
                                       static_cast<int64_t*>(d_counter), st)));
  HIP_RETURN_NOT_OK(hipMemcpyAsync(out_arr->buffers[1]->mutable_data(), d_out, static_cast<size_t>(m) * w,
                                   hipMemcpyDeviceToHost, st));
  int64_t valid_count = m;
  if (allocate_validity) {
    HIP_RETURN_NOT_OK(hipMemcpyAsync(out_arr->buffers[0]->mutable_data(), d_out_valid,
                                     static_cast<size_t>(arrow::bit_util::BytesForBits(m)),
                                     hipMemcpyDeviceToHost, st));
    HIP_RETURN_NOT_OK(hipMemcpyAsync(&valid_count, d_counter, 8, hipMemcpyDeviceToHost, st));
  }
  HIP_RETURN_NOT_OK(hipStreamSynchronize(st));
  out_arr->null_count = m - valid_count;
  CountGpu(kFnTake);
  return Status::OK();
}
```

arrow_amd/csrc/plugin/selection_nested.inc:

```
StockKernel g_stock_filter_fsl, g_stock_take_fsl, g_stock_filter_list, g_stock_take_list, g_stock_filter_large_list, g_stock_take_large_list;

const StockKernel& NestedStock(Type::type id, bool take) {
  switch (id) {
    case Type::FIXED_SIZE_LIST: return take ? g_stock_take_fsl : g_stock_filter_fsl;
    case Type::LARGE_LIST: return take ? g_stock_take_large_list : g_stock_filter_large_list;
    default: return take ? g_stock_take_list : g_stock_filter_list;
  }
}

arrow::Result<std::unique_ptr<cp::KernelState>> NestedFilterInit(cp::KernelContext* ctx, const cp::KernelInitArgs& args) {
  auto state = std::make_unique<ShimState<cp::FilterOptions>>();
  const Type::type id = !args.inputs.empty() && args.inputs[0].type != nullptr ? args.inputs[0].type->id() : Type::LIST;
  const StockKernel& stock_k = NestedStock(id, false);
  if (stock_k.init) {
    ARROW_ASSIGN_OR_RAISE(state->stock, stock_k.init(ctx, args));
  }
  if (args.options != nullptr) state->options = *static_cast<const cp::FilterOptions*>(args.options);
  return state;
}

arrow::Result<std::unique_ptr<cp::KernelState>> NestedTakeInit(cp::KernelContext* ctx, const cp::KernelInitArgs& args) {
  auto state = std::make_unique<ShimState<cp::TakeOptions>>();
  const Type::type id = !args.inputs.empty() && args.inputs[0].type != nullptr ? args.inputs[0].type->id() : Type::LIST;
  const StockKernel& stock_k = NestedStock(id, true);
  if (stock_k.init) {
    ARROW_ASSIGN_OR_RAISE(state->stock, stock_k.init(ctx, args));
  }
  if (args.options != nullptr) state->options = *static_cast<const cp::TakeOptions*>(args.options);
  return state;
}

arrow::Result<const void*> DeviceAddress(const arrow::BufferSpan& b) {
  if (b.owner == nullptr || *b.owner == nullptr) return nullptr;
  if ((*b.owner)->device_type() != arrow::DeviceAllocationType::kROCM) {
    return Status::Invalid("arrow_amd: mixed host / device buffers in one array");
  }
  return reinterpret_cast<const void*>((*b.owner)->address());
}

Status RequireNoNulls(const ArraySpan& child, const arrow::DataType& outer, hipStream_t st) {
  if (child.buffers[0].owner == nullptr || *child.buffers[0].owner == nullptr) return Status::OK();
  int64_t nulls = child.null_count;
  if (nulls <= 0) {
    const auto& bitmap = **child.buffers[0].owner;
    if (bitmap.device_type() != arrow::DeviceAllocationType::kROCM) return Status::Invalid("arrow_amd: mixed host / device buffers in one array");
    void* ws = nullptr;
    ARROW_RETURN_NOT_OK(t_scratch.Get(kCounter, 64, &ws));
    int64_t set_bits = 0;
    ARROW_RETURN_NOT_OK(FromArx(arx_bitmap_popcount(reinterpret_cast<const void*>(bitmap.address()), child.offset, child.length, ws, 64,
                                                    &set_bits, st)));
    nulls = child.length - set_bits;
  }
  if (nulls != 0) {
    return Status::NotImplemented("arrow_amd: filter / take of device-resident ", outer.ToString(), " whose nested values have nulls");
  }
  return Status::OK();
}

Status FixedRowLayout(const ArraySpan& a, hipStream_t st, int64_t* row_bytes, const uint8_t** row0, const arrow::DataType** leaf_type) {
  const arrow::DataType& t = *a.type;
  if (t.id() != Type::FIXED_SIZE_LIST) {
    const int w = t.id() == Type::FIXED_SIZE_BINARY ? static_cast<const arrow::FixedSizeBinaryType&>(t).byte_width() : FixedByteWidth(t);
    if (w <= 0) return Status::NotImplemented("arrow_amd: filter / take of device-resident fixed_size_list with ", t.ToString(), " values");
    ARROW_ASSIGN_OR_RAISE(const void* base_addr, DeviceAddress(a.buffers[1]));
    const uint8_t* base = static_cast<const uint8_t*>(base_addr);
    if (base == nullptr && a.length > 0) return Status::Invalid("arrow_amd: a fixed-width array without a data buffer");
    *row_bytes = w;
    *row0 = base != nullptr ? base + a.offset * w : nullptr;
    *leaf_type = &t;
    return Status::OK();
  }
  const int64_t k = static_cast<const arrow::FixedSizeListType&>(t).list_size();
  const ArraySpan& child = a.child_data[0];
  ARROW_RETURN_NOT_OK(RequireNoNulls(child, t, st));
  int64_t child_bytes = 0;
  const uint8_t* child0 = nullptr;
  ARROW_RETURN_NOT_OK(FixedRowLayout(child, st, &child_bytes, &child0, leaf_type));
  *row_bytes = k * child_bytes;
  *row0 = child0 != nullptr ? child0 + a.offset * *row_bytes : nullptr;
  return Status::OK();
}

std::shared_ptr<ArrayData> NestFixedChildren(const arrow::DataType& t, int64_t rows, std::shared_ptr<Buffer> data) {
  if (t.id() != Type::FIXED_SIZE_LIST) {
    return ArrayData::Make(t.GetSharedPtr(), rows, {nullptr, std::move(data)}, 0);
  }
  const auto& fsl = static_cast<const arrow::FixedSizeListType&>(t);
  auto child = NestFixedChildren(*fsl.value_type(), rows * fsl.list_size(), std::move(data));
  return ArrayData::Make(t.GetSharedPtr(), rows, {nullptr}, {std::move(child)}, 0);
}

Status FslTakeOnDevice(const ArraySpan& values, const ArxSpan& di, int tid, hipStream_t st, ArrayData* out_arr) {
  int64_t row_bytes = 0;
  const uint8_t* row0 = nullptr;
  const arrow::DataType* leaf = nullptr;
  const ArraySpan& child = values.child_data[0];
  ARROW_RETURN_NOT_OK(RequireNoNulls(child, *values.type, st));
  int64_t child_bytes = 0;
  ARROW_RETURN_NOT_OK(FixedRowLayout(child, st, &child_bytes, &row0, &leaf));
  const int64_t k = static_cast<const arrow::FixedSizeListType&>(*values.type).list_size();
  row_bytes = k * child_bytes;
  if (row_bytes == 0) return Status::NotImplemented("arrow_amd: filter / take of device-resident ", values.type->ToString(), " (rows of 0 bytes)");
  ARROW_ASSIGN_OR_RAISE(const void* validity, DeviceAddress(values.buffers[0]));
  ArxSpan dv{validity, row0, values.offset, values.length,
             validity == nullptr ? 0 : (values.null_count > 0 ? values.null_count : arrow::kUnknownNullCount)};
  const int64_t m = di.length;
  const bool allocate_validity = dv.validity != nullptr || di.null_count != 0;
  ARROW_ASSIGN_OR_RAISE(auto data, AllocDevice(std::max<int64_t>(m * row_bytes, 1) + 16));
  std::shared_ptr<Buffer> valid_buf;
  void* d_valid = nullptr;
  void* d_counter = nullptr;
  if (allocate_validity) {
    ARROW_ASSIGN_OR_RAISE(valid_buf, AllocDevice(((m + 63) / 64) * 8));
    d_valid = reinterpret_cast<void*>(valid_buf->mutable_address());
    ARROW_RETURN_NOT_OK(t_scratch.Get(kCounter, 64, &d_counter));
    HIP_RETURN_NOT_OK(hipMemsetAsync(d_counter, 0, 8, st));
  }
  if (m > 0) {
    ARROW_RETURN_NOT_OK(FromArx(arx_take_rows(&dv, row_bytes, &di, tid, reinterpret_cast<void*>(data->mutable_address()), d_valid,
                                              static_cast<int64_t*>(d_counter), st)));
  }
  int64_t valid_count = m;
  if (allocate_validity) HIP_RETURN_NOT_OK(hipMemcpyAsync(&valid_count, d_counter, 8, hipMemcpyDeviceToHost, st));
  HIP_RETURN_NOT_OK(hipStreamSynchronize(st));
  const auto& fsl = static_cast<const arrow::FixedSizeListType&>(*values.type);
  out_arr->length = m;
  out_arr->offset = 0;
  out_arr->buffers = {valid_buf};
  out_arr->child_data = {NestFixedChildren(*fsl.value_type(), m * k, std::move(data))};
  out_arr->null_count = m - valid_count;
  return Status::OK();
}

Status ListTakeOnDevice(const ArraySpan& values, const ArxSpan& di, int tid, hipStream_t st, ArrayData* out_arr) {
  const bool large = values.type->id() == Type::LARGE_LIST;
  const ArraySpan& child = values.child_data[0];
  const int w = FixedByteWidth(*child.type);
  int shift = 0;
  while ((1 << shift) < w) ++shift;
  if (w <= 0 || (1 << shift) != w) {
    return Status::NotImplemented("arrow_amd: filter / take of device-resident ", values.type->ToString(),
                                  " (nested values of a fixed width of 1 .. 32 bytes)");
  }
  ARROW_RETURN_NOT_OK(RequireNoNulls(child, *values.type, st));
  ARROW_ASSIGN_OR_RAISE(const void* child_addr, DeviceAddress(child.buffers[1]));
  const uint8_t* child0 = static_cast<const uint8_t*>(child_addr);
  ArxBinarySpan dv{};
  ARROW_ASSIGN_OR_RAISE(dv.validity, DeviceAddress(values.buffers[0]));
  ARROW_ASSIGN_OR_RAISE(const void* offsets_addr, DeviceAddress(values.buffers[1]));
  dv.offsets = static_cast<const int32_t*>(offsets_addr);
  dv.data = child0 != nullptr ? child0 + child.offset * w : nullptr;
  dv.offset = values.offset;
  dv.length = values.length;
  dv.null_count = dv.validity == nullptr ? 0 : (values.null_count > 0 ? values.null_count : arrow::kUnknownNullCount);
  if (dv.offsets == nullptr) return Status::Invalid("arrow_amd: a list array without an offsets buffer");
  const int64_t m = di.length;
  const bool allocate_validity = dv.null_count != 0 || di.null_count != 0;
  std::shared_ptr<Buffer> valid_buf, off_buf, data_buf;
  ARROW_ASSIGN_OR_RAISE(off_buf, AllocDevice((m + 1) * (large ? 8 : 4)));
  void* d_valid = nullptr;
  void* d_counter = nullptr;
  if (allocate_validity) {
    ARROW_ASSIGN_OR_RAISE(valid_buf, AllocDevice(((m + 63) / 64) * 8));
    d_valid = reinterpret_cast<void*>(valid_buf->mutable_address());
    ARROW_RETURN_NOT_OK(t_scratch.Get(kCounter, 64, &d_counter));
    HIP_RETURN_NOT_OK(hipMemsetAsync(d_counter, 0, 8, st));
  }
  const size_t ws_bytes = large ? arx_large_binary_take_workspace_bytes(m) : arx_binary_take_workspace_bytes(m);
  void* ws = nullptr;
  ARROW_RETURN_NOT_OK(t_scratch.Get(kBinWs, ws_bytes, &ws));
  void* d_off = reinterpret_cast<void*>(off_buf->mutable_address());
  int64_t total = 0;
  if (large) {
    ARROW_RETURN_NOT_OK(FromArx(arx_large_binary_take_offsets(&dv, &di, tid, ws, ws_bytes, static_cast<int64_t*>(d_off), d_valid,
                                                              static_cast<int64_t*>(d_counter), &total, st)));
  } else {
    ARROW_RETURN_NOT_OK(FromArx(arx_binary_take_offsets(&dv, &di, tid, ws, ws_bytes, static_cast<int32_t*>(d_off), d_valid,
                                                        static_cast<int64_t*>(d_counter), &total, st)));
  }
  ARROW_ASSIGN_OR_RAISE(data_buf, AllocDevice(std::max<int64_t>(total * w, 1) + 16));
  void* d_data = reinterpret_cast<void*>(data_buf->mutable_address());
  if (large) {
    ARROW_RETURN_NOT_OK(FromArx(arx_large_list_take_data(&dv, shift, m, ws, ws_bytes, static_cast<const int64_t*>(d_off), total, d_data, st)));
  } else {
    ARROW_RETURN_NOT_OK(FromArx(arx_list_take_data(&dv, shift, m, ws, ws_bytes, static_cast<const int32_t*>(d_off), total, d_data, st)));
  }
  int64_t valid_count = m;
  if (allocate_validity) HIP_RETURN_NOT_OK(hipMemcpyAsync(&valid_count, d_counter, 8, hipMemcpyDeviceToHost, st));
  HIP_RETURN_NOT_OK(hipStreamSynchronize(st));
  out_arr->length = m;
  out_arr->offset = 0;
  out_arr->buffers = {valid_buf, off_buf};
  out_arr->child_data = {ArrayData::Make(child.type->GetSharedPtr(), total, {nullptr, std::move(data_buf)}, 0)};
  out_arr->null_count = m - valid_count;
  return Status::OK();
}

Status NestedTakeOnDevice(const ArraySpan& values, const ArxSpan& di, int tid, hipStream_t st, ArrayData* out_arr) {
  if (values.type->id() == Type::FIXED_SIZE_LIST) return FslTakeOnDevice(values, di, tid, st, out_arr);
  return ListTakeOnDevice(values, di, tid, st, out_arr);
}

Status NestedTakeExec(cp::KernelContext* ctx, const cp::ExecSpan& batch, cp::ExecResult* out) {
  auto* state = static_cast<ShimState<cp::TakeOptions>*>(ctx->state());
  const ArraySpan& values = batch[0].array;
  const ArraySpan& indices = batch[1].array;
  if (!SpanTouchesRocm(values) && !OnRocm(indices)) {
    return RunStock(kFnTake, NestedStock(values.type->id(), true), state->stock.get(), ctx, batch, out);
  }
  const int tid = IndexTypeId(*indices.type);
  if (tid < 0) {
    return Status::NotImplemented("arrow_amd: take of ", values.type->ToString(), " by ", indices.type->ToString(), " on device-resident arrays");
  }
  hipStream_t st;
  ARROW_RETURN_NOT_OK(t_scratch.Stream(&st));
  ArxSpan di{};
  ARROW_RETURN_NOT_OK(DeviceSpan(indices, &di));
  if (state->options.boundscheck) ARROW_RETURN_NOT_OK(CheckBoundsOnDevice(di, tid, values.length, st));
  ARROW_RETURN_NOT_OK(NestedTakeOnDevice(values, di, tid, st, out->array_data().get()));
  CountGpu(kFnTake);
  return Status::OK();
}

Status NestedFilterExec(cp::KernelContext* ctx, const cp::ExecSpan& batch, cp::ExecResult* out) {
  auto* state = static_cast<ShimState<cp::FilterOptions>*>(ctx->state());
  const ArraySpan& values = batch[0].array;
  const ArraySpan& filter = batch[1].array;
  if (!SpanTouchesRocm(values) && !OnRocm(filter)) {
    return RunStock(kFnFilter, NestedStock(values.type->id(), false), state->stock.get(), ctx, batch, out);
  }
  if (filter.type->id() != Type::BOOL) {
    return Status::NotImplemented("arrow_amd: filter of ", values.type->ToString(), " by ", filter.type->ToString(), " on device-resident arrays");
  }
  if (filter.length > 0xFFFFFFFFll) {
    return Status::NotImplemented("Filter length exceeds UINT32_MAX, consider a different strategy for selecting elements");
  }
  const int null_sel = state->options.null_selection_behavior == cp::FilterOptions::EMIT_NULL ? ARX_FILTER_EMIT_NULL : ARX_FILTER_DROP;
  hipStream_t st;
  ARROW_RETURN_NOT_OK(t_scratch.Stream(&st));
  ArxSpan dm{};
  ARROW_RETURN_NOT_OK(DeviceSpan(filter, &dm));
  const size_t ws_bytes = arx_filter_workspace_bytes(filter.length);
  void* ws = nullptr;
  ARROW_RETURN_NOT_OK(t_scratch.Get(kWs, ws_bytes, &ws));
  int64_t out_len = 0;
  ARROW_RETURN_NOT_OK(FromArx(arx_filter_count(&dm, null_sel, ws, ws_bytes, &out_len, st)));
  const bool emit = null_sel == ARX_FILTER_EMIT_NULL && dm.null_count != 0;
  void* d_idx = nullptr;
  void* d_idx_valid = nullptr;
  ARROW_RETURN_NOT_OK(t_scratch.Get(kArg2, static_cast<size_t>(out_len) * 4 + 64, &d_idx));
  if (emit) ARROW_RETURN_NOT_OK(t_scratch.Get(kArg2Validity, static_cast<size_t>((out_len + 63) / 64) * 8 + 64, &d_idx_valid));
  ARROW_RETURN_NOT_OK(FromArx(arx_mask_to_indices(&dm, null_sel, ws, out_len, 4, d_idx, d_idx_valid, st)));
  ArxSpan di{d_idx_valid, d_idx, 0, out_len, emit ? arrow::kUnknownNullCount : 0};
  ARROW_RETURN_NOT_OK(NestedTakeOnDevice(values, di, ARX_UINT32, st, out->array_data().get()));
  CountGpu(kFnFilter);
  return Status::OK();
}
```

arrow_amd/csrc/plugin/vector_hash.inc:

```
enum HashVectorKind { kHashUnique = 0, kHashValueCounts, kHashDictEncode };

struct DeviceHashState : public cp::KernelState {
  HashVectorKind kind = kHashUnique;
  std::unique_ptr<cp::KernelState> stock;
  bool used_stock = false, used_device = false;
  bool encode_nulls = false;
  std::shared_ptr<arrow::DataType> type;
  int width = 0;
  std::shared_ptr<Buffer> table_buf, counts_buf;
  void* table = nullptr;
  int64_t max_groups = 0, num_groups = 0, counts_cap = 0;
};

StockKernel g_stock_unique, g_stock_value_counts, g_stock_dict_encode;
cp::VectorKernel::FinalizeFunc g_stock_unique_finalize = nullptr, g_stock_value_counts_finalize = nullptr,
                               g_stock_dict_encode_finalize = nullptr;

template <HashVectorKind KIND>
const StockKernel& StockHashKernel() {
  return KIND == kHashUnique ? g_stock_unique : KIND == kHashValueCounts ? g_stock_value_counts : g_stock_dict_encode;
}

Status HashUniques(DeviceHashState* s, hipStream_t st, std::shared_ptr<Buffer>* values, std::shared_ptr<Buffer>* validity,
                   int64_t* null_count) {
// ... 19 lines not shown
    int64_t nulls = 0;
    ARROW_RETURN_NOT_OK(HashUniques(s, st, &values, &validity, &nulls));
    ArxSpan sp{reinterpret_cast<const void*>(validity->address()), reinterpret_cast<const void*>(values->address()), 0,
               s->num_groups, nulls};
    const int32_t w = s->width;
    const size_t ws_bytes = arx_grouper_consume_workspace_bytes(s->num_groups);
    void *ws = nullptr, *ids = nullptr;
    ARROW_RETURN_NOT_OK(t_scratch.Get(kWs, ws_bytes + 256, &ws));
    ws = Align256(ws);
    ARROW_RETURN_NOT_OK(t_scratch.Get(kArg2, static_cast<size_t>(s->num_groups) * 4 + 64, &ids));
    ARROW_RETURN_NOT_OK(FromArx(arx_grouper_consume(fresh, fresh_max, &sp, &w, 1, ws, ws_bytes, static_cast<uint32_t*>(ids), st)));
  }
  s->table_buf = std::move(fresh_table.buffer);
  s->table = fresh;
  s->max_groups = fresh_max;
  return Status::OK();
}

template <HashVectorKind KIND>
Status HashVectorExec(cp::KernelContext* ctx, const cp::ExecSpan& batch, cp::ExecResult* out) {
  auto* s = static_cast<DeviceHashState*>(ctx->state());
  const ArraySpan& values = batch[0].array;
  if (!OnRocm(values)) {
    if (s->used_device) return Status::NotImplemented("arrow_amd: host and device-resident chunks in one hash kernel call");
    s->used_stock = true;
    return RunStock(kFnUnique, StockHashKernel<KIND>(), s->stock.get(), ctx, batch, out);
  }
  if (s->used_stock) return Status::NotImplemented("arrow_amd: host and device-resident chunks in one hash kernel call");
  if (s->width != 1 && s->width != 2 && s->width != 4 && s->width != 8) {
    return Status::NotImplemented("arrow_amd: ", KIND == kHashUnique ? "unique" : KIND == kHashValueCounts ? "value_counts" : "dictionary_encode",
                                  " of device-resident ", values.type->ToString(), " arrays");
  }
  s->used_device = true;
  const int64_t n = values.length;
  hipStream_t st;
  ARROW_RETURN_NOT_OK(t_scratch.Stream(&st));
  ArrayData* out_arr = out->array_data().get();
  if (KIND == kHashDictEncode) {
    out_arr->type = arrow::int32();
    out_arr->length = n;
    out_arr->null_count = 0;
    out_arr->buffers.assign(2, nullptr);
    ARROW_ASSIGN_OR_RAISE(out_arr->buffers[1], AllocDevice(std::max<int64_t>(n, 1) * 4));
  }
  if (n == 0) return Status::OK();
  ARROW_RETURN_NOT_OK(HashEnsureCapacity(s, n, st));
  ArxSpan sp{};
  ARROW_RETURN_NOT_OK(DeviceSpan(values, &sp));
  const int32_t w = s->width;
  const size_t ws_bytes = arx_grouper_consume_workspace_bytes(n);
  void *ws = nullptr, *ids = nullptr;
  ARROW_RETURN_NOT_OK(t_scratch.Get(kWs, ws_bytes + 256, &ws));
  ws = Align256(ws);
  if (KIND == kHashDictEncode) {
    ids = reinterpret_cast<void*>(out_arr->buffers[1]->mutable_address());
  } else {
    ARROW_RETURN_NOT_OK(t_scratch.Get(kArg2, static_cast<size_t>(n) * 4 + 64, &ids));
  }
  ARROW_RETURN_NOT_OK(FromArx(arx_grouper_consume(s->table, s->max_groups, &sp, &w, 1, ws, ws_bytes, static_cast<uint32_t*>(ids), st)));
  ARROW_RETURN_NOT_OK(FromArx(arx_grouper_num_groups(s->table, &s->num_groups, st)));
  if (KIND == kHashValueCounts) {
    if (s->num_groups > s->counts_cap) {
      const int64_t cap = std::max<int64_t>({s->num_groups, 2 * s->counts_cap, 1 << 12});
      ARROW_ASSIGN_OR_RAISE(auto fresh, AllocDevice(cap * 8));
      HIP_RETURN_NOT_OK(hipMemsetAsync(reinterpret_cast<void*>(fresh->mutable_address()), 0, static_cast<size_t>(cap) * 8, st));
      if (s->counts_buf != nullptr && s->counts_cap > 0) {
        HIP_RETURN_NOT_OK(hipMemcpyAsync(reinterpret_cast<void*>(fresh->mutable_address()),
                                         reinterpret_cast<const void*>(s->counts_buf->address()),
                                         static_cast<size_t>(s->counts_cap) * 8, hipMemcpyDeviceToDevice, st));
      }
      HIP_RETURN_NOT_OK(hipStreamSynchronize(st));
      s->counts_buf = std::move(fresh);
      s->counts_cap = cap;
    }
    ARROW_RETURN_NOT_OK(FromArx(arx_hash_count_consume(nullptr, 0, 0, ARX_COUNT_ALL, static_cast<const uint32_t*>(ids), n,
                                                       reinterpret_cast<int64_t*>(s->counts_buf->mutable_address()), st)));
  }
  if (KIND == kHashDictEncode && !s->encode_nulls && sp.validity != nullptr) {
    if (values.offset == 0) {
      out_arr->buffers[0] = values.GetBuffer(0);
    } else {
      ARROW_ASSIGN_OR_RAISE(out_arr->buffers[0], AllocDevice(((n + 63) / 64) * 8));
      ARROW_RETURN_NOT_OK(FromArx(arx_bitmap_copy(sp.validity, sp.offset, n,
                                                  reinterpret_cast<void*>(out_arr->buffers[0]->mutable_address()), st)));
    }
    ARROW_ASSIGN_OR_RAISE(out_arr->null_count, DeviceNullCount(*out_arr->buffers[0], n, st));
    if (out_arr->null_count == 0) out_arr->buffers[0] = nullptr;
  }
  HIP_RETURN_NOT_OK(hipStreamSynchronize(st));
  CountGpu(kFnUnique);
  return Status::OK();
}

arrow::Result<std::shared_ptr<ArrayData>> HashDictionary(DeviceHashState* s, bool drop_null, hipStream_t st, int64_t* null_id);

template <HashVectorKind KIND>
Status HashVectorFinalize(cp::KernelContext* ctx, std::vector<arrow::Datum>* out) {
  auto* s = static_cast<DeviceHashState*>(ctx->state());
  if (!s->used_device) {
    cp::VectorKernel::FinalizeFunc stock = KIND == kHashUnique ? g_stock_unique_finalize
                                           : KIND == kHashValueCounts ? g_stock_value_counts_finalize
                                                                      : g_stock_dict_encode_finalize;
    ctx->SetState(s->stock.get());
    Status status = stock(ctx, out);
    ctx->SetState(s);
    return status;
  }
  hipStream_t st;
  ARROW_RETURN_NOT_OK(t_scratch.Stream(&st));
  int64_t null_id = -1;
  if (KIND == kHashUnique) {
    ARROW_ASSIGN_OR_RAISE(auto uniques, HashDictionary(s, false, st, &null_id));
    *out = {arrow::Datum(std::move(uniques))};
  } else if (KIND == kHashValueCounts) {
    ARROW_ASSIGN_OR_RAISE(auto uniques, HashDictionary(s, false, st, &null_id));
    const int64_t g = s->num_groups;
    ARROW_ASSIGN_OR_RAISE(auto counts_buf, AllocDevice(std::max<int64_t>(g, 1) * 8));
    if (g > 0) {
      ARROW_RETURN_NOT_OK(FromArx(arx_buffer_copy(reinterpret_cast<const void*>(s->counts_buf->address()),
                                                  reinterpret_cast<void*>(counts_buf->mutable_address()), g * 8, st)));
      HIP_RETURN_NOT_OK(hipStreamSynchronize(st));
    }
    auto counts = ArrayData::Make(arrow::int64(), g, {nullptr, std::move(counts_buf)}, 0);
    auto type = arrow::struct_({arrow::field("values", s->type), arrow::field("counts", arrow::int64())});
    auto boxed = ArrayData::Make(std::move(type), g, {nullptr}, {std::move(uniques), std::move(counts)}, 0);
    *out = {arrow::Datum(std::move(boxed))};
  } else {
    ARROW_ASSIGN_OR_RAISE(auto dict, HashDictionary(s, !s->encode_nulls, st, &null_id));
    auto dict_type = arrow::dictionary(arrow::int32(), s->type);
    for (auto& datum : *out) {
      std::shared_ptr<ArrayData> idx = datum.array();
      if (null_id >= 0 && idx->length > 0) {
        ARROW_RETURN_NOT_OK(FromArx(arx_group_ids_skip_group(reinterpret_cast<uint32_t*>(idx->buffers[1]->mutable_address()),
                                                             idx->length, static_cast<uint32_t>(null_id), st)));
      }
      auto encoded = idx->Copy();
      encoded->type = dict_type;
      encoded->dictionary = dict;
      datum = arrow::Datum(std::move(encoded));
    }
    HIP_RETURN_NOT_OK(hipStreamSynchronize(st));
  }
  return Status::OK();
}

Status CompactByBitmap(const ArxSpan& dv, int width, const void* mask_bits, int64_t mask_offset, int64_t n, hipStream_t st,
                       std::shared_ptr<Buffer>* out_values, std::shared_ptr<Buffer>* out_validity, int64_t* out_length,
                       int64_t* out_null_count) {
  ArxSpan dm{nullptr, mask_bits, mask_offset, n, 0};
  const size_t ws_bytes = arx_filter_workspace_bytes(n);
  void* ws = nullptr;
  ARROW_RETURN_NOT_OK(t_scratch.Get(kWs, ws_bytes, &ws));
  int64_t out_len = 0;
  ARROW_RETURN_NOT_OK(FromArx(arx_filter_count(&dm, ARX_FILTER_DROP, ws, ws_bytes, &out_len, st)));
  ARROW_ASSIGN_OR_RAISE(*out_values, AllocDevice(std::max<int64_t>(out_len, 1) * width));
  void* d_valid = nullptr;
  *out_validity = nullptr;
  if (dv.validity != nullptr && dv.null_count != 0) {
    ARROW_ASSIGN_OR_RAISE(*out_validity, AllocDevice(((out_len + 63) / 64) * 8 + 8));
    d_valid = reinterpret_cast<void*>((*out_validity)->mutable_address());
  }
  ARROW_RETURN_NOT_OK(FromArx(arx_filter_exec(&dv, width, &dm, ARX_FILTER_DROP, ws, out_len,
                                              reinterpret_cast<void*>((*out_values)->mutable_address()), d_valid, st)));
  *out_length = out_len;
  *out_null_count = 0;
  if (d_valid != nullptr) {
    ARROW_ASSIGN_OR_RAISE(*out_null_count, DeviceNullCount(**out_validity, out_len, st));
  }
  HIP_RETURN_NOT_OK(hipStreamSynchronize(st));
  return Status::OK();
}

arrow::Result<std::shared_ptr<ArrayData>> HashDictionary(DeviceHashState* s, bool drop_null, hipStream_t st, int64_t* null_id) {
  std::shared_ptr<Buffer> values, validity;
  int64_t nulls = 0;
  ARROW_RETURN_NOT_OK(HashUniques(s, st, &values, &validity, &nulls));
  HIP_RETURN_NOT_OK(hipStreamSynchronize(st));
  const int64_t g = s->num_groups;
  *null_id = -1;
  if (nulls == 0) return ArrayData::Make(s->type, g, {nullptr, std::move(values)}, 0);
  if (!drop_null) return ArrayData::Make(s->type, g, {std::move(validity), std::move(values)}, nulls);
  void* d_idx = nullptr;
  ARROW_RETURN_NOT_OK(t_scratch.Get(kArg2, 256, &d_idx));
  {
    ARROW_ASSIGN_OR_RAISE(auto inv, AllocDevice(((g + 63) / 64) * 8 + 8));
    ARROW_RETURN_NOT_OK(FromArx(arx_boolean_invert(reinterpret_cast<const void*>(validity->address()), 0, g,
                                                   reinterpret_cast<void*>(inv->mutable_address()), st)));
    ArxSpan dm{nullptr, reinterpret_cast<const void*>(inv->address()), 0, g, 0};
    const size_t ws_bytes = arx_filter_workspace_bytes(g);
    void* ws = nullptr;
    ARROW_RETURN_NOT_OK(t_scratch.Get(kWs, ws_bytes, &ws));
    int64_t cnt = 0;
    ARROW_RETURN_NOT_OK(FromArx(arx_filter_count(&dm, ARX_FILTER_DROP, ws, ws_bytes, &cnt, st)));
    if (cnt != 1) return Status::Invalid("arrow_amd: internal error (", cnt, " null entries among the unique values)");
    ARROW_RETURN_NOT_OK(FromArx(arx_mask_to_indices(&dm, ARX_FILTER_DROP, ws, cnt, 4, d_idx, nullptr, st)));
    uint32_t pos = 0;
    HIP_RETURN_NOT_OK(hipMemcpyAsync(&pos, d_idx, 4, hipMemcpyDeviceToHost, st));
    HIP_RETURN_NOT_OK(hipStreamSynchronize(st));
    *null_id = pos;
  }
  ArxSpan dv{nullptr, reinterpret_cast<const void*>(values->address()), 0, g, 0};
  std::shared_ptr<Buffer> kept, kept_validity;
  int64_t kept_len = 0, kept_nulls = 0;
  ARROW_RETURN_NOT_OK(CompactByBitmap(dv, s->width, reinterpret_cast<const void*>(validity->address()), 0, g, st, &kept,
                                      &kept_validity, &kept_len, &kept_nulls));
  return ArrayData::Make(s->type, kept_len, {nullptr, std::move(kept)}, 0);
}

class RocmDropNullMetaFunction : public cp::MetaFunction {
 public:
  explicit RocmDropNullMetaFunction(std::shared_ptr<cp::Function> stock)
      : cp::MetaFunction("drop_null", cp::Arity::Unary(), stock->doc()), stock_(std::move(stock)) {}

  arrow::Result<arrow::Datum> ExecuteImpl(const std::vector<arrow::Datum>& args, const cp::FunctionOptions* options,
                                          cp::ExecContext* ctx) const override {
    if (args.size() == 1 && args[0].is_array() && DataOnRocm(*args[0].array())) {
      const ArrayData& in = *args[0].array();
      const int w = FixedByteWidth(*in.type);
      if (w == 0) return Status::NotImplemented("arrow_amd: drop_null of device-resident ", in.type->ToString(), " arrays");
      if (in.buffers[0] == nullptr || in.null_count.load() == 0 || in.length == 0) return args[0];
      hipStream_t st;
      ARROW_RETURN_NOT_OK(t_scratch.Stream(&st));
      ArxSpan dv{};
      ARROW_RETURN_NOT_OK(DeviceSpan(ArraySpan(in), &dv));
      const void* bits = dv.validity;
      dv.validity = nullptr;
      dv.null_count = 0;
      std::shared_ptr<Buffer> values, validity;
      int64_t len = 0, nulls = 0;
      ARROW_RETURN_NOT_OK(CompactByBitmap(dv, w, bits, in.offset, in.length, st, &values, &validity, &len, &nulls));
      CountGpu(kFnFilter);
      return arrow::Datum(ArrayData::Make(in.type, len, {nullptr, std::move(values)}, 0));
    }
    return stock_->Execute(args, options, ctx);
  }

 private:
  std::shared_ptr<cp::Function> stock_;
};

StockKernel g_stock_nonzero;

int NonZeroNumericTypeId(Type::type id) {
  switch (id) {
    case Type::INT8: return ARX_NUM_INT8;
    case Type::UINT8: return ARX_NUM_UINT8;
    case Type::INT16: return ARX_NUM_INT16;
    case Type::UINT16: return ARX_NUM_UINT16;
    case Type::INT32: return ARX_NUM_INT32;
    case Type::UINT32: return ARX_NUM_UINT32;
    case Type::INT64: return ARX_NUM_INT64;
    case Type::UINT64: return ARX_NUM_UINT64;
    case Type::FLOAT: return ARX_NUM_FLOAT32;
    case Type::DOUBLE: return ARX_NUM_FLOAT64;
    default: return -1;
  }
}

Status IndicesNonZeroExecRocm(cp::KernelContext* ctx, const cp::ExecSpan& batch, cp::ExecResult* out) {
  const ArraySpan& in = batch[0].array;
  if (!OnRocm(in)) {
    CountStock(kFnFilter);
    return g_stock_nonzero.exec(ctx, batch, out);
  }
  const int64_t n = in.length;
  if (n > 0xFFFFFFFFll) return Status::NotImplemented("arrow_amd: indices_nonzero of more than UINT32_MAX device rows");
  hipStream_t st;
  ARROW_RETURN_NOT_OK(t_scratch.Stream(&st));
  ArxSpan dv{};
  ARROW_RETURN_NOT_OK(DeviceSpan(in, &dv));
  ArxSpan dm{dv.validity, nullptr, dv.offset, n, dv.null_count};
  std::shared_ptr<Buffer> bits, rebased;
  if (in.type->id() == Type::BOOL) {
    dm.data = dv.data;
  } else {
    const int num = NonZeroNumericTypeId(in.type->id());
    if (num < 0) return Status::NotImplemented("arrow_amd: indices_nonzero of device-resident ", in.type->ToString(), " arrays");
    static const int widths[10] = {1, 1, 2, 2, 4, 4, 8, 8, 4, 8};
    ARROW_ASSIGN_OR_RAISE(bits, AllocDevice(((n + 63) / 64) * 8 + 8));
    const uint64_t zero = 0;
    const uint8_t* base = static_cast<const uint8_t*>(dv.data) + dv.offset * widths[num];
    if (n > 0) {
      ARROW_RETURN_NOT_OK(FromArx(arx_compare_numeric(ARX_CMP_NOT_EQUAL, num, base, nullptr, nullptr, &zero, n,
                                                      reinterpret_cast<uint64_t*>(bits->mutable_address()), st)));
    }
    dm.data = reinterpret_cast<const void*>(bits->address());
    dm.offset = 0;
    if (dm.validity != nullptr && dv.offset != 0) {
      ARROW_ASSIGN_OR_RAISE(rebased, AllocDevice(((n + 63) / 64) * 8 + 8));
      ARROW_RETURN_NOT_OK(FromArx(arx_bitmap_copy(dv.validity, dv.offset, n, reinterpret_cast<void*>(rebased->mutable_address()), st)));
      dm.validity = reinterpret_cast<const void*>(rebased->address());
    }
  }
  const size_t ws_bytes = arx_filter_workspace_bytes(n);
  void* ws = nullptr;
  ARROW_RETURN_NOT_OK(t_scratch.Get(kWs, ws_bytes, &ws));
  int64_t cnt = 0;
  if (n > 0) ARROW_RETURN_NOT_OK(FromArx(arx_filter_count(&dm, ARX_FILTER_DROP, ws, ws_bytes, &cnt, st)));
  void* d_idx = nullptr;
  ARROW_RETURN_NOT_OK(t_scratch.Get(kArg2, static_cast<size_t>(cnt) * 4 + 64, &d_idx));
  ARROW_ASSIGN_OR_RAISE(auto out_values, AllocDevice(std::max<int64_t>(cnt, 1) * 8));
  bool direct = false;
  if (cnt > 0) {
    direct = arx_mask_to_indices(&dm, ARX_FILTER_DROP, ws, cnt, 8, reinterpret_cast<void*>(out_values->mutable_address()), nullptr, st) == ARX_OK;
  }
  if (cnt > 0 && !direct) {
    ARROW_RETURN_NOT_OK(FromArx(arx_mask_to_indices(&dm, ARX_FILTER_DROP, ws, cnt, 4, d_idx, nullptr, st)));
    ArxSpan di{nullptr, d_idx, 0, cnt, 0};
    void* flag = nullptr;
    ARROW_RETURN_NOT_OK(t_scratch.Get(kFlag, 64, &flag));
    ARROW_RETURN_NOT_OK(FromArx(arx_cast_numeric(&di, ARX_NUM_UINT32, ARX_NUM_UINT64, 1, 1, flag, 64,
                                                 reinterpret_cast<void*>(out_values->mutable_address()), st)));
  }
  HIP_RETURN_NOT_OK(hipStreamSynchronize(st));
  CountGpu(kFnFilter);
  out->value = ArrayData::Make(arrow::uint64(), cnt, {nullptr, std::move(out_values)}, 0);
  return Status::OK();
}

Status RegisterIndicesNonZero(cp::FunctionRegistry* reg) {
  ARROW_ASSIGN_OR_RAISE(auto fn, reg->GetFunction("indices_nonzero"));
  if (fn->kind() != cp::Function::VECTOR) return Status::Invalid("indices_nonzero is not a vector function");
  auto* vfn = static_cast<cp::VectorFunction*>(fn.get());
  for (const auto& ty : {arrow::boolean(), arrow::int8(), arrow::uint8(), arrow::int16(), arrow::uint16(), arrow::int32(),
                         arrow::uint32(), arrow::int64(), arrow::uint64(), arrow::float32(), arrow::float64()}) {
    ARROW_ASSIGN_OR_RAISE(const cp::Kernel* k0, vfn->DispatchExact({ty}));
    cp::VectorKernel copy = *static_cast<const cp::VectorKernel*>(k0);
    if (g_stock_nonzero.exec == nullptr) g_stock_nonzero.exec = copy.exec;
    if (g_stock_nonzero.exec != copy.exec) continue;
    copy.exec = IndicesNonZeroExecRocm;
    ARROW_RETURN_NOT_OK(vfn->AddKernel(std::move(copy)));
  }
  return Status::OK();
}

struct HashValueType {
  std::shared_ptr<arrow::DataType> probe;
  cp::InputType match;
};
std::vector<HashValueType> HashVectorTypes() {
  using arrow::TimeUnit;
  std::vector<HashValueType> t;
  for (const auto& ty : {arrow::int8(), arrow::uint8(), arrow::int16(), arrow::uint16(), arrow::int32(), arrow::uint32(),
                         arrow::int64(), arrow::uint64(), arrow::float32(), arrow::float64(), arrow::date32(), arrow::date64()}) {
    t.push_back({ty, cp::InputType(ty)});
  }
  t.push_back({arrow::time32(TimeUnit::SECOND), cp::InputType(Type::TIME32)});
  t.push_back({arrow::time64(TimeUnit::NANO), cp::InputType(Type::TIME64)});
  t.push_back({arrow::timestamp(TimeUnit::NANO), cp::InputType(Type::TIMESTAMP)});
  t.push_back({arrow::duration(TimeUnit::NANO), cp::InputType(Type::DURATION)});
  return t;
}

template <HashVectorKind KIND>
Status RegisterHashVector(cp::FunctionRegistry* reg, const char* name, StockKernel* stock,
                          cp::VectorKernel::FinalizeFunc* stock_finalize) {
  ARROW_ASSIGN_OR_RAISE(auto fn, reg->GetFunction(name));
  if (fn->kind() != cp::Function::VECTOR) return Status::Invalid(name, " is not a vector function");
  auto* vfn = static_cast<cp::VectorFunction*>(fn.get());
  const std::vector<HashValueType> types = HashVectorTypes();
  for (const auto& vt : types) {
    ARROW_ASSIGN_OR_RAISE(const cp::Kernel* k0, vfn->DispatchExact({vt.probe}));
    cp::VectorKernel copy = *static_cast<const cp::VectorKernel*>(k0);
    if (stock->exec == nullptr) {
      stock->exec = copy.exec;
      *stock_finalize = copy.finalize;
    } else if (stock->exec != copy.exec) {
      continue;
    }
    stock->init = nullptr;
    const cp::KernelInit stock_init = copy.init;
    copy.init = [stock_init](cp::KernelContext* ctx, const cp::KernelInitArgs& args)
        -> arrow::Result<std::unique_ptr<cp::KernelState>> {
      auto state = std::make_unique<DeviceHashState>();
      state->kind = KIND;
      state->type = args.inputs[0].GetSharedPtr();
      state->width = FixedByteWidth(*state->type);
      if (KIND == kHashDictEncode && args.options != nullptr) {
        state->encode_nulls = static_cast<const cp::DictionaryEncodeOptions*>(args.options)->null_encoding_behavior ==
                              cp::DictionaryEncodeOptions::ENCODE;
      }
      ARROW_ASSIGN_OR_RAISE(state->stock, stock_init(ctx, args));
      return state;
    };
    copy.signature = cp::KernelSignature::Make({vt.match}, copy.signature->out_type());
    copy.exec = HashVectorExec<KIND>;
    copy.finalize = HashVectorFinalize<KIND>;
    copy.mem_allocation = cp::MemAllocation::NO_PREALLOCATE;
    ARROW_RETURN_NOT_OK(vfn->AddKernel(std::move(copy)));
  }
  return Status::OK();
}
```

arrow_amd/csrc/selection.hip:

```cpp
#include "arx_common.h"

#include <string.h>

#include <algorithm>
#include <type_traits>

namespace arx {

struct FilterWsHeader {
  int64_t total;
  int64_t ntiles;
  int64_t ngroups;
  int64_t length;
  int64_t valid;
  int64_t pad[3];
};
static_assert(sizeof(FilterWsHeader) == 64, "header is one 64-byte line");

struct FilterWsView {
  FilterWsHeader* hdr;
  int64_t* group_excl;
  int64_t* group_total;
  uint32_t* tile_counts;
  int64_t* group_valid;
};

static inline int64_t num_tiles(int64_t length) { return ceil_div(length, kTileRows); }
static inline int64_t num_groups(int64_t length) {
  return ceil_div(num_tiles(length), kTilesPerGroup);
}

static inline FilterWsView ws_view(void* ws, int64_t length) {
  FilterWsView v;
  const int64_t ng = num_groups(length);
  uint8_t* p = static_cast<uint8_t*>(ws);
  v.hdr = reinterpret_cast<FilterWsHeader*>(p);
  v.group_excl = reinterpret_cast<int64_t*>(p + 64);
  v.group_total = v.group_excl + ng;
  v.tile_counts = reinterpret_cast<uint32_t*>(v.group_total + ng);
  v.group_valid = reinterpret_cast<int64_t*>(v.tile_counts + ng * kTilesPerGroup);
  return v;
}

__device__ __forceinline__ uint64_t emit_word(const Bits& mask, const Bits& mvalid, int64_t w,
                                              bool emit_null, bool invert,
                                              uint64_t* mask_valid_out) {
  uint64_t m = load_word(mask, w);
  const uint64_t mv = load_word(mvalid, w);
  *mask_valid_out = mv;
  if (emit_null || invert) {
    const uint64_t in_range = load_word(Bits{nullptr, 0, mask.length, 0}, w);
    if (invert) m = ~m & in_range;
    if (emit_null) return (m | ~mv) & in_range;
  }
  return m & mv;
}

template <bool VALID>
__global__ __launch_bounds__(kBlock) void count_kernel(Bits mask, Bits mvalid, Bits vvalid, int emit_null,
                                                       int invert, int64_t ntiles,
                                                       uint32_t* tile_counts,
                                                       int64_t* group_total, int64_t* group_valid) {
  __shared__ uint32_t wave_sums[kWavesPerBlock];
  __shared__ uint32_t wave_valid[kWavesPerBlock];
  const int lane = lane_id();
  const int wave = threadIdx.x >> 6;
  const int64_t group = blockIdx.x;
  const int64_t t0 = group * kTilesPerGroup + wave * 16;
  uint32_t mine = 0;
  uint32_t kv = 0;
#pragma unroll 4
  for (int i = 0; i < 16; ++i) {
    const int64_t t = t0 + i;
    uint32_t k = 0;
    if (t < ntiles) {
      uint64_t mv;
      const uint64_t e = emit_word(mask, mvalid, t * 64 + lane, emit_null != 0, invert != 0, &mv);
      k = __popcll(e);
      if constexpr (VALID) kv += __popcll(e & mv & load_word(vvalid, t * 64 + lane));
    }
    const uint32_t s = wave_reduce_sum_u32(k);
    if (lane == i) mine = s;
  }
  if (lane < 16) tile_counts[t0 + lane] = mine;
  const uint32_t wsum = wave_reduce_sum_u32(lane < 16 ? mine : 0u);
  if (lane == 0) wave_sums[wave] = wsum;
  if constexpr (VALID) {
    const uint32_t vsum = wave_reduce_sum_u32(kv);
    if (lane == 0) wave_valid[wave] = vsum;
  }
  __syncthreads();
  if (threadIdx.x == 0) {
    int64_t s = 0, v = 0;
    for (int i = 0; i < kWavesPerBlock; ++i) {
      s += wave_sums[i];
      if constexpr (VALID) v += wave_valid[i];
    }
    group_total[group] = s;
    if constexpr (VALID) group_valid[group] = v;
  }
}

__global__ __launch_bounds__(1024) void scan_kernel(const int64_t* group_total, int64_t ngroups,
                                                    int64_t* group_excl, FilterWsHeader* hdr,
                                                    const int64_t* group_valid = nullptr) {
  __shared__ int64_t wave_tot[16];
  __shared__ int64_t carry_s;
  __shared__ unsigned long long valid_s;
  const int tid = threadIdx.x;
  const int lane = tid & 63;
  const int wave = tid >> 6;
  if (tid == 0) carry_s = 0;
  if (tid == 0) valid_s = 0;
  __syncthreads();
  if (group_valid != nullptr) {
    int64_t mine = 0;
    for (int64_t i = tid; i < ngroups; i += 1024) mine += group_valid[i];
#pragma unroll
    for (int d = 32; d >= 1; d >>= 1) mine += __shfl_xor(mine, d, 64);
    if (lane == 0 && mine != 0) atomicAdd(&valid_s, static_cast<unsigned long long>(mine));
    __syncthreads();
  }
  for (int64_t base = 0; base < ngroups; base += 1024) {
    const int64_t i = base + tid;
    const int64_t v = i < ngroups ? group_total[i] : 0;
    int64_t x = v;
#pragma unroll
    for (int d = 1; d < 64; d <<= 1) {
      const int64_t n = __shfl_up(x, d, 64);
      if (lane >= d) x += n;
    }
    if (lane == 63) wave_tot[wave] = x;
    __syncthreads();
    int64_t wave_prefix = 0;
    for (int k = 0; k < wave; ++k) wave_prefix += wave_tot[k];
    const int64_t carry = carry_s;
    if (i < ngroups) group_excl[i] = carry + wave_prefix + x - v;
    __syncthreads();
    if (tid == 1023) carry_s = carry + wave_prefix + x;
    __syncthreads();
  }
  if (tid == 0) {
    hdr->total = carry_s;
    hdr->valid = static_cast<int64_t>(valid_s);
  }
}

struct CompactArgs {
  const uint8_t* values;
  Bits mask;
  Bits mvalid;
  Bits vvalid;
  int64_t length;
  int64_t ntiles;
  const uint32_t* tile_counts;
  const int64_t* group_excl;
  uint8_t* out_data;
  uint64_t* out_validity;
  int emit_null;
  int invert;
  int values_aligned16;
};

constexpr int kFlushBytes = 2048;

template <int RING>
struct __attribute__((aligned(16))) CompactLds {
  uint8_t ring[kWavesPerBlock][RING];
  uint64_t vbits[kWavesPerBlock][72];
};

template <int W>
struct ElemT;
template <> struct ElemT<1> { using type = uint8_t; };
template <> struct ElemT<2> { using type = uint16_t; };
template <> struct ElemT<4> { using type = uint32_t; };
template <> struct ElemT<8> { using type = uint64_t; };
template <> struct ElemT<16> { using type = uint4; };
struct Elem32 { uint4 lo, hi; };
template <> struct ElemT<32> { using type = Elem32; };

template <int W>
__device__ __forceinline__ typename ElemT<W>::type zero_elem() {
  if constexpr (W == 32) {
    return Elem32{make_uint4(0, 0, 0, 0), make_uint4(0, 0, 0, 0)};
  } else if constexpr (W == 16) {
    return make_uint4(0, 0, 0, 0);
  } else {
    return 0;
  }
}

constexpr int kSelNt = 3;

template <int W>
__device__ __forceinline__ typename ElemT<W>::type sel_load(const typename ElemT<W>::type* p, bool nt) {
  using E = typename ElemT<W>::type;
  if constexpr (W == 32) {
    return *p;
  } else if constexpr (W == 16) {
    return nt ? nt_load16(p) : *p;
  } else {
    return nt ? nt_load<E>(p) : *p;
  }
}
template <int W>
__device__ __forceinline__ void sel_store(typename ElemT<W>::type* p, typename ElemT<W>::type v) {
  using E = typename ElemT<W>::type;
  if constexpr (W == 32) {
    *p = v;
  } else if constexpr (W == 16) {
    if constexpr ((kSelNt & 2) != 0) nt_store16(p, v); else *p = v;
  } else {
    if constexpr ((kSelNt & 2) != 0) nt_store<E>(p, v); else *p = v;
  }
}

__device__ __forceinline__ void wave_lds_sync() {
  __builtin_amdgcn_fence(__ATOMIC_RELEASE, "wavefront");
  __builtin_amdgcn_wave_barrier();
  __builtin_amdgcn_fence(__ATOMIC_ACQUIRE, "wavefront");
}

template <int W, int RING>
__device__ __forceinline__ void flush_region(const uint8_t* ring, uint8_t* gbase, int64_t F,
                                             int64_t lo, int64_t hi, int lane) {
  using E = typename ElemT<W>::type;
  constexpr int R = 16 / W;
  const int ring_off = static_cast<int>(F & (RING - 1));
#pragma unroll
  for (int h = 0; h < kFlushBytes / (16 * kWave); ++h) {
    const int g = h * kWave + lane;
    const int64_t gs = F + g * 16;
    const int64_t ge = gs + 16;
    if (ge <= lo || gs >= hi) continue;
    const uint8_t* src = ring + ring_off + g * 16;
    uint8_t* dst = gbase + gs;
    if (gs >= lo && ge <= hi) {
      sel_store<16>(reinterpret_cast<uint4*>(dst), *reinterpret_cast<const uint4*>(src));
    } else {
#pragma unroll
      for (int e = 0; e < R; ++e) {
        const int64_t es = gs + e * W;
        if (es >= lo && es + W <= hi) {
          *reinterpret_cast<E*>(dst + e * W) = *reinterpret_cast<const E*>(src + e * W);
        }
      }
    }
  }
}

template <int W, int B>
struct Batch {
  using E = typename ElemT<W>::type;
  static constexpr int R = 16 / W;
  uint32_t bits[B];
  uint32_t zbits[B];
  uint32_t rank[B];
  E v[B][R];
};

template <int R, bool EMIT>
__device__ __forceinline__ void select_words(uint64_t Ew, uint32_t p, uint64_t Zw,
                                             int widx_base, int lane, uint64_t* wE, uint32_t* wp,
                                             uint64_t* wZ) {
  constexpr int kLanesPerWord = 64 / R;
  const int q_mine = lane / kLanesPerWord;
  uint64_t e = 0, z = 0;
  uint32_t pp = 0;
#pragma unroll
  for (int q = 0; q < R; ++q) {
    const int src = widx_base + q;
    const uint32_t lo = __builtin_amdgcn_readlane(static_cast<uint32_t>(Ew), src);
    const uint32_t hi = __builtin_amdgcn_readlane(static_cast<uint32_t>(Ew >> 32), src);
    const uint32_t pq = __builtin_amdgcn_readlane(p, src);
    uint64_t zq = 0;
    if constexpr (EMIT) {
      const uint32_t zlo = __builtin_amdgcn_readlane(static_cast<uint32_t>(Zw), src);
      const uint32_t zhi = __builtin_amdgcn_readlane(static_cast<uint32_t>(Zw >> 32), src);
      zq = (static_cast<uint64_t>(zhi) << 32) | zlo;
    }
    if (q == q_mine) {
      e = (static_cast<uint64_t>(hi) << 32) | lo;
      pp = pq;
      z = zq;
    }
  }
  *wE = e;
  *wp = pp;
  *wZ = z;
}

struct TileCtx {
  uint64_t Ew, Zw;
  uint32_t p;
  int lane;
  int64_t tile_row0;
// ... 602 lines not shown

template <typename IdxT, bool HAS_IV>
__global__ __launch_bounds__(kBlock) void take_columns_kernel(TakeColsArgs a) {
  constexpr int U = 4;
  const int lane = lane_id();
  const int64_t nwaves = static_cast<int64_t>(gridDim.x) * kWavesPerBlock;
  const int64_t wave_g = static_cast<int64_t>(blockIdx.x) * kWavesPerBlock +
                         __builtin_amdgcn_readfirstlane(threadIdx.x >> 6);
  const int64_t nchunks = (a.length + 64 * U - 1) / (64 * U);
  const int64_t last = a.length - 1;
  const IdxT* __restrict__ indices = reinterpret_cast<const IdxT*>(a.indices);
  uint64_t nvalid[kTakeMaxCols];
  for (int c = 0; c < kTakeMaxCols; ++c) nvalid[c] = 0;
  for (int64_t ch = wave_g; ch < nchunks; ch += nwaves) {
    const int64_t base = ch * (64 * U);
    int64_t pos[U];
    uint64_t idx[U];
    bool ok0[U];
#pragma unroll
    for (int u = 0; u < U; ++u) {
      const int64_t p = base + u * 64 + lane;
      pos[u] = p <= last ? p : last;
      idx[u] = static_cast<uint64_t>(indices[pos[u]]);
    }
#pragma unroll
    for (int u = 0; u < U; ++u) {
      ok0[u] = (base + u * 64 + lane) <= last;
      if constexpr (HAS_IV) {
        const uint64_t wbits = load_word_nb(a.ivalid, (base >> 6) + u);
        ok0[u] = ok0[u] && ((wbits >> lane) & 1ull);
      }
    }
    for (int c = 0; c < a.num_cols; ++c) {
      uint64_t nv;
      switch (a.width[c]) {
        case 1: nv = take_one_column<1, U>(a, c, pos, idx, ok0, base, last, lane); break;
        case 2: nv = take_one_column<2, U>(a, c, pos, idx, ok0, base, last, lane); break;
        case 4: nv = take_one_column<4, U>(a, c, pos, idx, ok0, base, last, lane); break;
        case 8: nv = take_one_column<8, U>(a, c, pos, idx, ok0, base, last, lane); break;
        case 16: nv = take_one_column<16, U>(a, c, pos, idx, ok0, base, last, lane); break;
        default: nv = take_one_column<32, U>(a, c, pos, idx, ok0, base, last, lane); break;
      }
      nvalid[c] += nv;
    }
  }
  if (a.valid_counts != nullptr && lane == 0) {
    for (int c = 0; c < a.num_cols; ++c) {
      if (nvalid[c] != 0) atomicAdd(a.valid_counts + c, nvalid[c]);
    }
  }
}

template <typename IdxT>
__global__ __launch_bounds__(kBlock) void take_bits_kernel(TakeArgs a, int64_t value_bit_offset) {
  const int lane = lane_id();
  const int64_t nwaves = static_cast<int64_t>(gridDim.x) * kWavesPerBlock;
  const int64_t wave_g = static_cast<int64_t>(blockIdx.x) * kWavesPerBlock +
                         __builtin_amdgcn_readfirstlane(threadIdx.x >> 6);
  const int64_t nwords = (a.length + 63) >> 6;
  const int64_t last = a.length - 1;
  const IdxT* __restrict__ indices = reinterpret_cast<const IdxT*>(a.indices);
  uint64_t* __restrict__ out = reinterpret_cast<uint64_t*>(a.out_data);
  uint64_t nvalid = 0;
  for (int64_t w = wave_g; w < nwords; w += nwaves) {
    const int64_t p = (w << 6) + lane;
    const int64_t pc = p <= last ? p : last;
    const uint64_t idx = static_cast<uint64_t>(indices[pc]);
    bool ok = p <= last && ((load_word(a.ivalid, w) >> lane) & 1ull);
    if (ok && a.src_valid_bytes != nullptr) {
      const uint64_t vb = static_cast<uint64_t>(a.src_valid_offset) + idx;
      ok = (a.src_valid_bytes[vb >> 3] >> (vb & 7)) & 1;
    }
    bool bit = false;
    if (ok) {
      const uint64_t b = static_cast<uint64_t>(value_bit_offset) + idx;
      bit = (a.values[b >> 3] >> (b & 7)) & 1;
    }
    const uint64_t data_bal = __ballot(bit);
    const uint64_t valid_bal = __ballot(ok);
    nvalid += __popcll(valid_bal);
    if (lane == 0) {
      out[w] = data_bal;
      if (a.out_validity != nullptr) a.out_validity[w] = valid_bal;
    }
  }
  if (a.valid_count != nullptr && lane == 0 && nvalid != 0) atomicAdd(a.valid_count, nvalid);
}

struct BoundsWs {
  unsigned long long first_bad_pos;
  long long bad_value_signed;
  unsigned long long bad_value_unsigned;
  int64_t pad[5];
};

template <typename IdxT>
__global__ __launch_bounds__(kBlock) void bounds_kernel(const uint8_t* indices, Bits ivalid,
                                                        int64_t length, uint64_t upper,
                                                        BoundsWs* ws) {
  const int64_t stride = static_cast<int64_t>(gridDim.x) * blockDim.x;
  unsigned long long bad = ~0ull;
  for (int64_t i = static_cast<int64_t>(blockIdx.x) * blockDim.x + threadIdx.x; i < length;
       i += stride) {
    const IdxT v = reinterpret_cast<const IdxT*>(indices)[i];
    const bool valid = (load_word(ivalid, i >> 6) >> (i & 63)) & 1ull;
    bool oob;
    if constexpr (std::is_signed<IdxT>::value) {
      oob = v < 0 || static_cast<uint64_t>(v) >= upper;
    } else {
      oob = static_cast<uint64_t>(v) >= upper;
    }
    if (valid && oob) {
      bad = static_cast<unsigned long long>(i);
      break;
    }
  }
  if (bad != ~0ull) atomicMin(&ws->first_bad_pos, bad);
}

template <typename IdxT>
__global__ void bounds_fetch_kernel(const uint8_t* indices, BoundsWs* ws) {
  const unsigned long long pos = ws->first_bad_pos;
  if (pos == ~0ull) return;
  const IdxT v = reinterpret_cast<const IdxT*>(indices)[pos];
  ws->bad_value_signed = static_cast<long long>(v);
  ws->bad_value_unsigned = static_cast<unsigned long long>(v);
}

static int check_mask(const ArxSpan* mask, int null_selection) {
  if (mask == nullptr) {
    set_error("filter mask is NULL");
    return ARX_INVALID;
  }
  if (mask->length < 0 || mask->offset < 0) {
    set_error("negative length/offset");
    return ARX_INVALID;
  }
  if (mask->length > 0 && mask->data == nullptr) {
    set_error("filter mask has no data buffer");
    return ARX_INVALID;
  }
  if (null_selection != ARX_FILTER_DROP && null_selection != ARX_FILTER_EMIT_NULL) {
    set_error("bad null_selection %d", null_selection);
    return ARX_INVALID;
  }
  return ARX_OK;
}

static inline const void* effective_validity(const ArxSpan* s) {
  return (s->null_count != 0) ? s->validity : nullptr;
}

static int launch_count(const ArxSpan* mask, int null_selection, void* ws, size_t ws_bytes,
                        hipStream_t st, int invert = 0, const ArxSpan* values = nullptr) {
  const int rc = check_mask(mask, null_selection);
  if (rc != ARX_OK) return rc;
  const size_t need = arx_filter_workspace_bytes(mask->length);
  if (ws == nullptr || ws_bytes < need) {
    set_error("filter workspace too small: %zu < %zu", ws_bytes, need);
    return ARX_INVALID;
  }
  if ((reinterpret_cast<uint64_t>(ws) & 63) != 0) {
    set_error("filter workspace must be 64-byte aligned");
    return ARX_INVALID;
  }
  FilterWsView v = ws_view(ws, mask->length);
  const int64_t nt = num_tiles(mask->length);
  const int64_t ng = num_groups(mask->length);
  FilterWsHeader h{};
  h.total = 0;
  h.ntiles = nt;
  h.ngroups = ng;
  h.length = mask->length;
  ARX_HIP(hipMemcpyAsync(v.hdr, &h, sizeof(h), hipMemcpyHostToDevice, st));
  if (mask->length == 0) return ARX_OK;
  const Bits mb = make_bits(mask->data, mask->offset, mask->length);
  const Bits mvb = make_bits(effective_validity(mask), mask->offset, mask->length);
  if (values != nullptr) {
    const Bits vvb = make_bits(effective_validity(values), values->offset, mask->length);
    hipLaunchKernelGGL((count_kernel<true>), dim3(static_cast<unsigned>(ng)), dim3(kBlock), 0, st, mb, mvb, vvb,
                       null_selection, invert, nt, v.tile_counts, v.group_total, v.group_valid);
    ARX_CHECK_LAUNCH("count_kernel");
    hipLaunchKernelGGL(scan_kernel, dim3(1), dim3(1024), 0, st, v.group_total, ng, v.group_excl, v.hdr,
                       static_cast<const int64_t*>(v.group_valid));
  } else {
    hipLaunchKernelGGL((count_kernel<false>), dim3(static_cast<unsigned>(ng)), dim3(kBlock), 0, st, mb, mvb, mvb,
                       null_selection, invert, nt, v.tile_counts, v.group_total, static_cast<int64_t*>(nullptr));
    ARX_CHECK_LAUNCH("count_kernel");
    hipLaunchKernelGGL(scan_kernel, dim3(1), dim3(1024), 0, st, v.group_total, ng, v.group_excl, v.hdr,
                       static_cast<const int64_t*>(nullptr));
  }
  ARX_CHECK_LAUNCH("scan_kernel");
  return ARX_OK;
}

static Knob<int> g_filter_batch{4};
static Knob<int> g_filter_pipe{1};
static Knob<int> g_filter_sparse{-1};
static const KnobRow kSelectionKnobs[] = {
    {"filter_batch", g_filter_batch, knob_snap_down<1, 4>},
    {"filter_pipe", g_filter_pipe, knob_bool},
    {"filter_sparse", g_filter_sparse, knob_tri},
};
KnobTable selection_knobs() { return knob_table(kSelectionKnobs); }

template <int W, bool IOTA, bool EMIT, bool ALIGNED>
static void launch_compact_e(const CompactArgs& a, unsigned grid, hipStream_t st) {
  constexpr int kIters = kTileRows / (kWave * (16 / W));
  constexpr int kBig = kIters >= 8 ? 4 : 2;
  if (ALIGNED && g_filter_batch >= 4 && g_filter_pipe) {
    hipLaunchKernelGGL((compact_kernel<W, IOTA, EMIT, ALIGNED, kBig, true>), dim3(grid),
                       dim3(kBlock), 0, st, a);
  } else {
    hipLaunchKernelGGL((compact_kernel<W, IOTA, EMIT, ALIGNED, 1, false>), dim3(grid), dim3(kBlock),
                       0, st, a);
  }
}

template <int W, bool IOTA>
static void launch_compact_w(const CompactArgs& a, unsigned grid, hipStream_t st) {
  const bool aligned = IOTA || a.values_aligned16 != 0;
  if (a.emit_null) {
    if (aligned) launch_compact_e<W, IOTA, true, true>(a, grid, st);
    else if constexpr (!IOTA) launch_compact_e<W, IOTA, true, false>(a, grid, st);
  } else {
    if (aligned) launch_compact_e<W, IOTA, false, true>(a, grid, st);
    else if constexpr (!IOTA) launch_compact_e<W, IOTA, false, false>(a, grid, st);
  }
}

template <int W, bool IOTA = false>
static void launch_sparse_w(const CompactArgs& a, unsigned grid, hipStream_t st) {
  if (a.emit_null) {
    hipLaunchKernelGGL((compact_sparse_kernel<W, true, IOTA>), dim3(grid), dim3(kBlock), 0, st, a);
  } else {
    hipLaunchKernelGGL((compact_sparse_kernel<W, false, IOTA>), dim3(grid), dim3(kBlock), 0, st, a);
  }
}

static int launch_compact(bool iota, int W, const CompactArgs& a, hipStream_t st,
                          int64_t out_length = -1) {
  const unsigned grid = static_cast<unsigned>(ceil_div(a.ntiles, kWavesPerBlock));
  const int filter_sparse = g_filter_sparse;
  const bool sparse = !iota && !a.invert &&
                      (filter_sparse == 1 ||
                       (filter_sparse < 0 &&
                        (W >= 8 || (out_length >= 0 && out_length * 4 <= a.length))));
  if (iota && !a.invert && filter_sparse != 0 && (W == 2 || W == 4 || W == 8)) {
    if (W == 2) launch_sparse_w<2, true>(a, grid, st);
    else if (W == 4) launch_sparse_w<4, true>(a, grid, st);
    else launch_sparse_w<8, true>(a, grid, st);
    ARX_CHECK_LAUNCH("compact_sparse_kernel<IOTA>");
    return ARX_OK;
  }
  if (sparse) {
    switch (W) {
      case 1: launch_sparse_w<1>(a, grid, st); break;
      case 2: launch_sparse_w<2>(a, grid, st); break;
      case 4: launch_sparse_w<4>(a, grid, st); break;
      case 8: launch_sparse_w<8>(a, grid, st); break;
      case 16: launch_sparse_w<16>(a, grid, st); break;
      case 32: launch_sparse_w<32>(a, grid, st); break;
      default:
        set_error("unsupported byte width %d for the gfx950 filter", W);
        return ARX_NOT_IMPLEMENTED;
    }
    ARX_CHECK_LAUNCH("compact_sparse_kernel");
    return ARX_OK;
  }
  if (iota) {
    switch (W) {
      case 2: launch_compact_w<2, true>(a, grid, st); break;
      case 4: launch_compact_w<4, true>(a, grid, st); break;
      default:
        set_error("unsupported index width %d", W);
        return ARX_NOT_IMPLEMENTED;
    }
  } else {
    switch (W) {
      case 1: launch_compact_w<1, false>(a, grid, st); break;
      case 2: launch_compact_w<2, false>(a, grid, st); break;
      case 4: launch_compact_w<4, false>(a, grid, st); break;
      case 8: launch_compact_w<8, false>(a, grid, st); break;
      case 16: launch_compact_w<16, false>(a, grid, st); break;
      default:
        set_error("unsupported byte width %d for the gfx950 filter", W);
        return ARX_NOT_IMPLEMENTED;
    }
  }
  ARX_CHECK_LAUNCH("compact_kernel");
  return ARX_OK;
}

static int compact_form(bool iota, int W, bool values_aligned16, bool invert, int64_t length, int64_t out_length) {
  const int filter_sparse = g_filter_sparse;
  if (iota) {
    if (!invert && filter_sparse != 0 && (W == 2 || W == 4 || W == 8)) return ARX_COMPACT_GATHER;
    if (W != 2 && W != 4) return ARX_NOT_IMPLEMENTED;
  } else {
    const bool sparse = !invert && (filter_sparse == 1 ||
                                    (filter_sparse < 0 && (W >= 8 || (out_length >= 0 && out_length * 4 <= length))));
    if (sparse) return W == 1 || W == 2 || W == 4 || W == 8 || W == 16 || W == 32 ? ARX_COMPACT_GATHER : ARX_NOT_IMPLEMENTED;
    if (W != 1 && W != 2 && W != 4 && W != 8 && W != 16) return ARX_NOT_IMPLEMENTED;
  }
  if (!iota && !values_aligned16) return ARX_COMPACT_SWEEP_UNALIGNED;
  return g_filter_batch >= 4 && g_filter_pipe ? ARX_COMPACT_SWEEP_PIPELINED : ARX_COMPACT_SWEEP_PLAIN;
}

static int zero_out_validity(void* out_validity, int64_t out_length, hipStream_t st) {
  if (out_validity == nullptr) return ARX_OK;
  if ((reinterpret_cast<uint64_t>(out_validity) & 7) != 0) {
    set_error("out_validity must be 8-byte aligned");
    return ARX_INVALID;
  }
  if (out_length < 0) {
    set_error("out_length (from arx_filter_count) is required when out_validity is given");
    return ARX_INVALID;
  }
  if (out_length > 0) {
    ARX_HIP(hipMemsetAsync(out_validity, 0, static_cast<size_t>(ceil_div(out_length, 64)) * 8, st));
  }
  return ARX_OK;
}

size_t selection_workspace_bytes(int64_t length) { return arx_filter_workspace_bytes(length); }

int selection_bit_positions(const void* bitmap, int64_t bit_offset, int64_t length, bool invert,
                            void* ws, size_t ws_bytes, uint32_t* out, int64_t* out_count_host,
                            hipStream_t st) {
  ArxSpan m{};
  m.validity = nullptr;
  m.data = bitmap;
  m.offset = bit_offset;
  m.length = length;
  m.null_count = 0;
  int rc = launch_count(&m, ARX_FILTER_DROP, ws, ws_bytes, st, invert ? 1 : 0);
  if (rc != ARX_OK) return rc;
  int64_t total = 0;
  ARX_HIP(hipMemcpyAsync(&total, ws, sizeof(int64_t), hipMemcpyDeviceToHost, st));
  ARX_HIP(hipStreamSynchronize(st));
  *out_count_host = total;
  if (total == 0) return ARX_OK;
  FilterWsView v = ws_view(ws, length);
  CompactArgs a{};
  a.values = nullptr;
  a.mask = make_bits(bitmap, bit_offset, length);
  a.mvalid = make_bits(nullptr, 0, length);
  a.vvalid = make_bits(nullptr, 0, length);
  a.length = length;
  a.ntiles = num_tiles(length);
  a.tile_counts = v.tile_counts;
  a.group_excl = v.group_excl;
  a.out_data = reinterpret_cast<uint8_t*>(out);
  a.out_validity = nullptr;
  a.emit_null = 0;
  a.invert = invert ? 1 : 0;
  a.values_aligned16 = 1;
  return launch_compact(true, 4, a, st);
}

}

using namespace arx;

extern "C" {

size_t arx_filter_workspace_bytes(int64_t length) {
  if (length < 0) length = 0;
  const int64_t ng = num_groups(length);
  return static_cast<size_t>(64 + ng * 16 + ng * kTilesPerGroup * 4 + ng * 8 + 64);
}

int arx_filter_count_async(const ArxSpan* mask, int null_selection, void* ws, size_t ws_bytes,
                           void* stream) {
  return launch_count(mask, null_selection, ws, ws_bytes, as_stream(stream));
}

int arx_filter_count_nulls(const ArxSpan* values, const ArxSpan* mask, int null_selection, void* ws, size_t ws_bytes,
                           int64_t* out_length, int64_t* out_null_count, void* stream) {
  if (out_length == nullptr || out_null_count == nullptr || values == nullptr) {
    set_error("values / out_length / out_null_count is NULL");
    return ARX_INVALID;
  }
  if (mask != nullptr && values->length != mask->length) {
    set_error("filter values and mask differ in length (%lld vs %lld)", static_cast<long long>(values->length),
              static_cast<long long>(mask->length));
    return ARX_INVALID;
  }
  hipStream_t st = as_stream(stream);
  const int rc = launch_count(mask, null_selection, ws, ws_bytes, st, 0, values);
  if (rc != ARX_OK) return rc;
  int64_t hdr[5] = {0, 0, 0, 0, 0};
  ARX_HIP(hipMemcpyAsync(hdr, ws, sizeof(hdr), hipMemcpyDeviceToHost, st));
  ARX_HIP(hipStreamSynchronize(st));
  *out_length = hdr[0];
  *out_null_count = mask->length == 0 ? 0 : hdr[0] - hdr[4];
  return ARX_OK;
}

int arx_filter_count(const ArxSpan* mask, int null_selection, void* ws, size_t ws_bytes,
                     int64_t* out_length, void* stream) {
  if (out_length == nullptr) {
    set_error("out_length is NULL");
    return ARX_INVALID;
  }
  hipStream_t st = as_stream(stream);
  const int rc = launch_count(mask, null_selection, ws, ws_bytes, st);
  if (rc != ARX_OK) return rc;
  int64_t total = 0;
  ARX_HIP(hipMemcpyAsync(&total, ws, sizeof(int64_t), hipMemcpyDeviceToHost, st));
  ARX_HIP(hipStreamSynchronize(st));
  *out_length = total;
  return ARX_OK;
}

int arx_filter_exec(const ArxSpan* values, int byte_width, const ArxSpan* mask, int null_selection,
                    const void* ws, int64_t out_length, void* out_data, void* out_validity,
                    void* stream) {
  int rc = check_mask(mask, null_selection);
  if (rc != ARX_OK) return rc;
  if (values == nullptr || ws == nullptr) {
    set_error("values/ws is NULL");
    return ARX_INVALID;
  }
  if (values->length != mask->length) {
    set_error("Array arguments must all be the same length (values %lld vs filter %lld)",
              static_cast<long long>(values->length), static_cast<long long>(mask->length));
    return ARX_INVALID;
  }
  if (mask->length == 0) return ARX_OK;
  if (values->data == nullptr || out_data == nullptr) {
    set_error("values/out data buffer is NULL");
    return ARX_INVALID;
  }
  hipStream_t st = as_stream(stream);
  FilterWsView v = ws_view(const_cast<void*>(ws), mask->length);
  CompactArgs a{};
  a.values = static_cast<const uint8_t*>(values->data) + values->offset * byte_width;
  a.mask = make_bits(mask->data, mask->offset, mask->length);
  a.mvalid = make_bits(effective_validity(mask), mask->offset, mask->length);
  a.vvalid = make_bits(effective_validity(values), values->offset, values->length);
  a.length = mask->length;
  a.ntiles = num_tiles(mask->length);
  a.tile_counts = v.tile_counts;
  a.group_excl = v.group_excl;
  a.out_data = static_cast<uint8_t*>(out_data);
  a.out_validity = static_cast<uint64_t*>(out_validity);
  a.emit_null = null_selection == ARX_FILTER_EMIT_NULL && a.mvalid.base != nullptr;
  a.values_aligned16 = (reinterpret_cast<uint64_t>(a.values) & 15) == 0;
  if ((reinterpret_cast<uint64_t>(out_data) % byte_width) != 0) {
    set_error("out_data is not aligned to the element width");
    return ARX_INVALID;
  }
  rc = zero_out_validity(out_validity, out_length, st);
  if (rc != ARX_OK) return rc;
  return launch_compact(false, byte_width, a, st, out_length);
}

int arx_expand_by_mask(const void* dense, int byte_width, const ArxSpan* mask, const void* ws, void* out_data,
                       void* stream) {
  int rc = check_mask(mask, ARX_FILTER_DROP);
  if (rc != ARX_OK) return rc;
  if (ws == nullptr) {
    set_error("ws is NULL (run arx_filter_count on the mask first)");
    return ARX_INVALID;
  }
  if (mask->length == 0) return ARX_OK;
  if (out_data == nullptr || (reinterpret_cast<uint64_t>(out_data) % byte_width) != 0 ||
      (dense != nullptr && (reinterpret_cast<uint64_t>(dense) % byte_width) != 0)) {
    set_error("expand: NULL or misaligned buffer");
    return ARX_INVALID;
  }
  FilterWsView v = ws_view(const_cast<void*>(ws), mask->length);
  CompactArgs a{};
  a.values = static_cast<const uint8_t*>(dense);
  a.mask = make_bits(mask->data, mask->offset, mask->length);
  a.mvalid = make_bits(effective_validity(mask), mask->offset, mask->length);
  a.length = mask->length;
  a.ntiles = num_tiles(mask->length);
  a.tile_counts = v.tile_counts;
  a.group_excl = v.group_excl;
  a.out_data = static_cast<uint8_t*>(out_data);
  const unsigned grid = static_cast<unsigned>(ceil_div(a.ntiles, kWavesPerBlock));
  hipStream_t st = as_stream(stream);
  switch (byte_width) {
    case 1: hipLaunchKernelGGL((expand_kernel<1>), dim3(grid), dim3(kBlock), 0, st, a); break;
    case 2: hipLaunchKernelGGL((expand_kernel<2>), dim3(grid), dim3(kBlock), 0, st, a); break;
    case 4: hipLaunchKernelGGL((expand_kernel<4>), dim3(grid), dim3(kBlock), 0, st, a); break;
    case 8: hipLaunchKernelGGL((expand_kernel<8>), dim3(grid), dim3(kBlock), 0, st, a); break;
    case 16: hipLaunchKernelGGL((expand_kernel<16>), dim3(grid), dim3(kBlock), 0, st, a); break;
    default:
      set_error("unsupported byte width %d for expand", byte_width);
      return ARX_NOT_IMPLEMENTED;
  }
  ARX_CHECK_LAUNCH("expand_kernel");
  return ARX_OK;
}

int arx_mask_to_indices(const ArxSpan* mask, int null_selection, const void* ws, int64_t out_length,
                        int index_width, void* out_indices, void* out_validity, void* stream) {
  int rc = check_mask(mask, null_selection);
  if (rc != ARX_OK) return rc;
  if (ws == nullptr) {
    set_error("ws is NULL");
    return ARX_INVALID;
  }
  if (index_width != 2 && index_width != 4 && index_width != 8) {
    set_error("index_width must be 2, 4 or 8");
    return ARX_INVALID;
  }
  if (index_width == 8 && (g_filter_sparse == 0 || null_selection == ARX_FILTER_EMIT_NULL)) {
    set_error("index_width 8 is served by the gather form with DROP only");
    return ARX_NOT_IMPLEMENTED;
  }
  if (mask->length > static_cast<int64_t>(UINT32_MAX)) {
    set_error("Filter length exceeds UINT32_MAX, consider a different strategy for selecting elements");
    return ARX_NOT_IMPLEMENTED;
  }
  if (index_width == 2 && mask->length > 65535) {
    set_error("index_width 2 requires length <= 65535");
    return ARX_INVALID;
  }
  if (mask->length == 0) return ARX_OK;
  if (out_indices == nullptr) {
    set_error("out_indices is NULL");
    return ARX_INVALID;
  }
  hipStream_t st = as_stream(stream);
  FilterWsView v = ws_view(const_cast<void*>(ws), mask->length);
  CompactArgs a{};
// ... 372 lines not shown
```

include/arrow_amd.h:

```cpp
#ifndef ARROW_AMD_H_
#define ARROW_AMD_H_

#include <stddef.h>
#include <stdint.h>

#ifdef __cplusplus
extern "C" {
#endif

#define ARX_ABI_VERSION 5

typedef enum ArxStatus {
  ARX_OK = 0,
  ARX_OUT_OF_MEMORY = -1,
  ARX_INVALID = -4,
  ARX_CAPACITY_ERROR = -6,
  ARX_INDEX_ERROR = -7,
  ARX_NOT_IMPLEMENTED = -10,
  ARX_DEVICE_ERROR = -100
} ArxStatus;

enum { ARX_FILTER_DROP = 0, ARX_FILTER_EMIT_NULL = 1 };
enum { ARX_SORT_ASCENDING = 0, ARX_SORT_DESCENDING = 1 };
enum { ARX_NULLS_AT_START = 0, ARX_NULLS_AT_END = 1 };

enum {
  ARX_UINT8 = 0, ARX_INT8 = 1, ARX_UINT16 = 2, ARX_INT16 = 3,
  ARX_UINT32 = 4, ARX_INT32 = 5, ARX_UINT64 = 6, ARX_INT64 = 7
};

typedef struct ArxSpan {
  const void* validity;
  const void* data;
  int64_t offset;
  int64_t length;
  int64_t null_count;
} ArxSpan;

const char* arx_last_error(void);
int arx_abi_version(void);
int arx_device_count(void);
int arx_set_option(const char* name, int64_t value);
int arx_get_option(const char* name, int64_t* out_value);
int64_t arx_get_counter(const char* name);


size_t arx_filter_workspace_bytes(int64_t length);

int arx_filter_count(const ArxSpan* mask, int null_selection, void* ws, size_t ws_bytes,
                     int64_t* out_length, void* stream);

int arx_filter_count_nulls(const ArxSpan* values, const ArxSpan* mask, int null_selection, void* ws, size_t ws_bytes,
                           int64_t* out_length, int64_t* out_null_count, void* stream);

int arx_filter_count_async(const ArxSpan* mask, int null_selection, void* ws,
                           size_t ws_bytes, void* stream);

int arx_filter_exec(const ArxSpan* values, int byte_width, const ArxSpan* mask,
                    int null_selection, const void* ws, int64_t out_length, void* out_data,
                    void* out_validity, void* stream);

int arx_mask_to_indices(const ArxSpan* mask, int null_selection, const void* ws,
                        int64_t out_length, int index_width, void* out_indices,
                        void* out_validity, void* stream);

enum { ARX_COMPACT_GATHER = 0, ARX_COMPACT_SWEEP_PIPELINED = 1, ARX_COMPACT_SWEEP_PLAIN = 2, ARX_COMPACT_SWEEP_UNALIGNED = 3 };

int arx_filter_compact_form(int row_numbers, int byte_width, int values_aligned16, int invert,
                            int64_t length, int64_t out_length);

size_t arx_take_workspace_bytes(void);

int arx_check_index_bounds(const ArxSpan* indices, int index_type, uint64_t upper_limit,
                           void* ws, size_t ws_bytes, void* stream);

int arx_take(const ArxSpan* values, int byte_width, const ArxSpan* indices, int index_type,
             void* out_data, void* out_validity, int64_t* valid_count, void* stream);

int arx_take_rows(const ArxSpan* values, int64_t row_bytes, const ArxSpan* indices, int index_type, void* out_data,
                  void* out_validity, int64_t* valid_count, void* stream);

int arx_take_columns(const ArxSpan* columns, const int32_t* byte_widths, int num_columns, const ArxSpan* indices,
                     int index_type, void* const* out_data, void* const* out_validity, int64_t* valid_counts,
                     void* stream);
int arx_take_bits(const ArxSpan* values, const ArxSpan* indices, int index_type, void* out_bits, void* out_validity,
                  int64_t* valid_count, void* stream);

typedef struct ArxBinarySpan {
  const void* validity;
  const int32_t* offsets;
  const void* data;
  int64_t offset;
  int64_t length;
  int64_t null_count;
} ArxBinarySpan;
size_t arx_binary_take_workspace_bytes(int64_t num_indices);
int arx_binary_take_offsets(const ArxBinarySpan* values, const ArxSpan* indices, int index_type, void* ws,
                            size_t ws_bytes, int32_t* out_offsets, void* out_validity, int64_t* valid_count,
                            int64_t* out_total_bytes, void* stream);
int arx_binary_take_data(const ArxBinarySpan* values, int64_t num_indices, const void* ws, size_t ws_bytes,
                         const int32_t* out_offsets, int64_t total_bytes, void* out_data, void* stream);
size_t arx_large_binary_take_workspace_bytes(int64_t num_indices);
int arx_large_binary_take_offsets(const ArxBinarySpan* values, const ArxSpan* indices, int index_type, void* ws,
                                  size_t ws_bytes, int64_t* out_offsets, void* out_validity, int64_t* valid_count,
                                  int64_t* out_total_bytes, void* stream);
int arx_large_binary_take_data(const ArxBinarySpan* values, int64_t num_indices, const void* ws, size_t ws_bytes,
                               const int64_t* out_offsets, int64_t total_bytes, void* out_data, void* stream);

int arx_list_take_data(const ArxBinarySpan* values, int elem_shift, int64_t num_indices, const void* ws, size_t ws_bytes,
                       const int32_t* out_offsets, int64_t total_elements, void* out_data, void* stream);
int arx_large_list_take_data(const ArxBinarySpan* values, int elem_shift, int64_t num_indices, const void* ws,
                             size_t ws_bytes, const int64_t* out_offsets, int64_t total_elements, void* out_data,
                             void* stream);

enum {
  ARX_NUM_INT8 = 0, ARX_NUM_UINT8 = 1, ARX_NUM_INT16 = 2, ARX_NUM_UINT16 = 3, ARX_NUM_INT32 = 4, ARX_NUM_UINT32 = 5,
  ARX_NUM_INT64 = 6, ARX_NUM_UINT64 = 7, ARX_NUM_FLOAT32 = 8, ARX_NUM_FLOAT64 = 9
};

int arx_cast_numeric(const ArxSpan* values, int in_type, int out_type, int allow_int_overflow, int allow_float_truncate,
                     void* ws, size_t ws_bytes, void* out, void* stream);

#define ARX_CMP_EQUAL 0
#define ARX_CMP_NOT_EQUAL 1
#define ARX_CMP_GREATER 2
#define ARX_CMP_GREATER_EQUAL 3
#define ARX_CMP_LESS 4
#define ARX_CMP_LESS_EQUAL 5
int arx_compare_numeric(int op, int num_type, const void* left, const void* left_scalar, const void* right,
                        const void* right_scalar, int64_t length, uint64_t* out_bits, void* stream);

#define ARX_ARITH_ADD 0
#define ARX_ARITH_SUBTRACT 1
#define ARX_ARITH_MULTIPLY 2
int arx_arith_numeric(int op, int checked, int num_type, const void* left, const void* left_scalar,
                      const void* left_validity, int64_t left_offset, const void* right, const void* right_scalar,
                      const void* right_validity, int64_t right_offset, int64_t length, void* out,
                      uint32_t* overflow_flag, void* stream);
int arx_divide_numeric(int checked, int num_type, const void* left, const void* left_scalar, const void* left_validity,
                       int64_t left_offset, const void* right, const void* right_scalar, const void* right_validity,
                       int64_t right_offset, int64_t length, void* out, uint64_t* errors, void* stream);

enum { ARX_UNARY_NEGATE = 0, ARX_UNARY_ABS = 1, ARX_UNARY_SIGN = 2, ARX_UNARY_FLOOR = 3, ARX_UNARY_CEIL = 4, ARX_UNARY_TRUNC = 5 };
int arx_unary_numeric(int op, int checked, int num_type, const ArxSpan* values, void* out, uint64_t* errors, void* stream);

enum { ARX_ROUND_DIGITS = 0, ARX_ROUND_MULTIPLE = 1 };
enum {
  ARX_ROUND_DOWN = 0, ARX_ROUND_UP = 1, ARX_ROUND_TOWARDS_ZERO = 2, ARX_ROUND_TOWARDS_INFINITY = 3, ARX_ROUND_HALF_DOWN = 4,
  ARX_ROUND_HALF_UP = 5, ARX_ROUND_HALF_TOWARDS_ZERO = 6, ARX_ROUND_HALF_TOWARDS_INFINITY = 7, ARX_ROUND_HALF_TO_EVEN = 8,
  ARX_ROUND_HALF_TO_ODD = 9
};
int arx_round_numeric(int kind, int mode, int num_type, const ArxSpan* values, int64_t ndigits, const void* multiple, void* out,
                      uint64_t* errors, void* stream);
int arx_round_status(int kind, int mode, int num_type, const ArxSpan* values, int64_t ndigits, const void* multiple,
                     const uint64_t* errors, void* stream);

int arx_buffer_copy(const void* src, void* dst, int64_t nbytes, void* stream);
int arx_bitmap_copy(const void* bits, int64_t bit_offset, int64_t length, void* out,
                    void* stream);
int arx_bitmap_and(const void* left, int64_t left_offset, const void* right,
                   int64_t right_offset, int64_t length, void* out, void* stream);
int arx_bitmap_copy_at(const void* bits, int64_t bit_offset, int64_t length, void* out,
                       int64_t out_bit_offset, void* stream);

typedef struct ArxCopySeg {
  const void* src;
  void* dst;
  uint64_t nbytes;
} ArxCopySeg;
int arx_copy_segments(const ArxCopySeg* segments, int64_t num_segments, uint64_t max_segment_bytes, void* stream);
typedef struct ArxBitSeg {
  const void* src;
  int64_t src_bit_offset;
  void* dst;
  int64_t dst_bit_offset;
  int64_t nbits;
} ArxBitSeg;
int arx_bitmap_copy_segments(const ArxBitSeg* segments, int64_t num_segments, int64_t max_segment_bits, void* stream);
int arx_binary_rebase_offsets(const int32_t* offsets, int64_t length, int32_t base, int32_t* out,
                              void* stream);
int arx_reduce_i64_init(void* acc, void* stream);
int arx_reduce_i64_consume(const ArxSpan* values, void* acc, void* stream);
int arx_coalesce2(int byte_width, const ArxSpan* values, const ArxSpan* fill, const void* fill_scalar, int64_t length,
                  void* out_data, void* out_validity, void* stream);
int arx_reduce_float_minmax(const ArxSpan* values, int num_type, void* acc, void* stream);
size_t arx_sum_float_workspace_bytes(int64_t length, int64_t null_count);
int arx_sum_float(const ArxSpan* values, int num_type, void* ws, size_t ws_bytes, double* out_sum, int64_t* out_count,
                  void* stream);

#define ARX_AND_KLEENE 0
#define ARX_OR_KLEENE 1
int arx_boolean_kleene(int op, const ArxSpan* left, const ArxSpan* right, void* out_data, void* out_validity,
                       void* stream);
int arx_boolean_invert(const void* bits, int64_t bit_offset, int64_t length, void* out, void* stream);
int arx_bytes_to_bitmap(const uint8_t* bytes, int64_t length, void* out_bits, int64_t* set_count, void* stream);
int arx_bitmap_popcount(const void* bits, int64_t bit_offset, int64_t length, void* ws,
                        size_t ws_bytes, int64_t* out_count, void* stream);

int arx_ree_bool_expand(const void* run_ends, int run_end_width, int64_t num_runs, const ArxSpan* values,
                        int64_t logical_offset, int64_t length, void* out_bits, void* out_validity, void* stream);

enum {
  ARX_KEY_UINT64 = 0, ARX_KEY_INT64 = 1, ARX_KEY_UINT32 = 2, ARX_KEY_INT32 = 3,
  ARX_KEY_FLOAT64 = 4, ARX_KEY_FLOAT32 = 5
};
size_t arx_sort_indices_workspace_bytes(int64_t length);
int arx_sort_indices(const ArxSpan* values, int key_type, int order, int null_placement, void* ws,
                     size_t ws_bytes, uint64_t* out_indices, void* stream);
enum { ARX_RANK_MIN = 0, ARX_RANK_MAX = 1, ARX_RANK_FIRST = 2, ARX_RANK_DENSE = 3, ARX_RANK_QUANTILE = 4, ARX_RANK_NORMAL = 5 };
// ... 505 lines not shown
```

Before: 290,900 Mrows/s.

## Write filter sizes to pinned host line and restructure count kernel loads

```diff
diff --git a/arrow_amd/_lib.py b/arrow_amd/_lib.py
--- a/arrow_amd/_lib.py
+++ b/arrow_amd/_lib.py
@@ -122,6 +122,7 @@
     "arx_filter_count": (_int, [_span, _int, _p, _sz, C.POINTER(_i64), _p]),
     "arx_filter_count_async": (_int, [_span, _int, _p, _sz, _p]),
     "arx_filter_count_nulls": (_int, [_span, _span, _int, _p, _sz, C.POINTER(_i64), C.POINTER(_i64), _p]),
+    "arx_filter_size": (_int, [_span, _span, _int, _p, _sz, _p, _p]),
     "arx_filter_exec": (_int, [_span, _int, _span, _int, _p, _i64, _p, _p, _p]),
     "arx_mask_to_indices": (_int, [_span, _int, _p, _i64, _int, _p, _p, _p]),
     "arx_filter_compact_form": (_int, [_int, _int, _int, _int, _i64, _i64]),
diff --git a/arrow_amd/csrc/plugin/common.inc b/arrow_amd/csrc/plugin/common.inc
--- a/arrow_amd/csrc/plugin/common.inc
+++ b/arrow_amd/csrc/plugin/common.inc
@@ -182,6 +182,45 @@
 
 enum Slot { kValues = 0, kValidity, kArg2, kArg2Validity, kOutData, kOutValidity, kWs, kCounter, kBinWs, kFlag };
 
+class ResultLine {
+ public:
+  ~ResultLine() {
+    if (line_) (void)hipHostFree(line_);
+  }
+  Status Get(volatile int64_t** out) {
+    if (!line_) {
+      void* p = nullptr;
+      HIP_RETURN_NOT_OK(hipHostMalloc(&p, 64, hipHostMallocDefault));
+      line_ = static_cast<int64_t*>(p);
+    }
+    *out = line_;
+    return Status::OK();
+  }
+
+ private:
+  int64_t* line_ = nullptr;
+};
+thread_local ResultLine t_result;
+
+Status SizeSelection(const ArxSpan& dm, int null_sel, const ArxSpan* values_or_null, void* ws, size_t ws_bytes, hipStream_t st,
+                     int64_t* out_len, int64_t* out_nulls = nullptr) {
+  volatile int64_t* line = nullptr;
+  ARROW_RETURN_NOT_OK(t_result.Get(&line));
+  ARROW_RETURN_NOT_OK(FromArx(arx_filter_size(values_or_null, &dm, null_sel, ws, ws_bytes, const_cast<int64_t*>(line), st)));
+  HIP_RETURN_NOT_OK(hipStreamSynchronize(st));
+  *out_len = line[0];
+  if (out_nulls != nullptr) *out_nulls = values_or_null != nullptr ? line[0] - line[1] : 0;
+  return Status::OK();
+}
+
+Status FetchTakeCounter(const void* d_counter, hipStream_t st, volatile int64_t** where) {
+  volatile int64_t* line = nullptr;
+  ARROW_RETURN_NOT_OK(t_result.Get(&line));
+  HIP_RETURN_NOT_OK(hipMemcpyAsync(const_cast<int64_t*>(line + 2), d_counter, 8, hipMemcpyDeviceToHost, st));
+  *where = line + 2;
+  return Status::OK();
+}
+
 Status Upload(const ArraySpan& a, int byte_width_or_0_for_bool, int data_slot, int validity_slot,
               hipStream_t st, ArxSpan* out) {
   const int64_t o8 = a.offset % 8;
diff --git a/arrow_amd/csrc/plugin/parquet.inc b/arrow_amd/csrc/plugin/parquet.inc
--- a/arrow_amd/csrc/plugin/parquet.inc
+++ b/arrow_amd/csrc/plugin/parquet.inc
@@ -239,7 +239,7 @@
   const size_t ws_bytes = arx_filter_workspace_bytes(rows);
   ARROW_RETURN_NOT_OK(t_scratch.Get(kBinWs, ws_bytes, ws));
   int64_t counted = 0;
-  ARROW_RETURN_NOT_OK(FromArx(arx_filter_count(mask, ARX_FILTER_DROP, *ws, ws_bytes, &counted, st)));
+  ARROW_RETURN_NOT_OK(SizeSelection(*mask, ARX_FILTER_DROP, nullptr, *ws, ws_bytes, st, &counted));
   if (counted != dense) return Status::Invalid("Parquet: ", counted, " non-null levels but ", dense, " values");
   return Status::OK();
 }
@@ -1155,7 +1155,7 @@
     void* ws = nullptr;
     ARROW_RETURN_NOT_OK(t_scratch.Get(kBinWs, ws_bytes, &ws));
     int64_t counted = 0;
-    ARROW_RETURN_NOT_OK(FromArx(arx_filter_count(&mask, ARX_FILTER_DROP, ws, ws_bytes, &counted, st)));
+    ARROW_RETURN_NOT_OK(SizeSelection(mask, ARX_FILTER_DROP, nullptr, ws, ws_bytes, st, &counted));
     if (counted != dense) return Status::Invalid("Parquet: ", counted, " non-null levels but ", dense, " values");
     ARROW_ASSIGN_OR_RAISE(values, AllocDevice(rows * width));
     ARROW_RETURN_NOT_OK(FromArx(arx_expand_by_mask(d_dense, width, &mask, ws,
diff --git a/arrow_amd/csrc/plugin/selection.inc b/arrow_amd/csrc/plugin/selection.inc
--- a/arrow_amd/csrc/plugin/selection.inc
+++ b/arrow_amd/csrc/plugin/selection.inc
@@ -30,10 +30,10 @@
   }
   ARROW_RETURN_NOT_OK(FromArx(arx_take_bits(&dv, &di, tid, reinterpret_cast<void*>(out_arr->buffers[1]->mutable_address()),
                                             d_valid, static_cast<int64_t*>(d_counter), st)));
-  int64_t valid_count = m;
-  if (allocate_validity) HIP_RETURN_NOT_OK(hipMemcpyAsync(&valid_count, d_counter, 8, hipMemcpyDeviceToHost, st));
+  volatile int64_t* valid_count = nullptr;
+  if (allocate_validity) ARROW_RETURN_NOT_OK(FetchTakeCounter(d_counter, st, &valid_count));
   HIP_RETURN_NOT_OK(hipStreamSynchronize(st));
-  out_arr->null_count = m - valid_count;
+  out_arr->null_count = allocate_validity ? m - *valid_count : 0;
   return Status::OK();
 }
 
@@ -92,7 +92,7 @@
       void* ws = nullptr;
       ARROW_RETURN_NOT_OK(t_scratch.Get(kWs, ws_bytes, &ws));
       int64_t out_len = 0;
-      ARROW_RETURN_NOT_OK(FromArx(arx_filter_count(&dm, null_sel, ws, ws_bytes, &out_len, st)));
+      ARROW_RETURN_NOT_OK(SizeSelection(dm, null_sel, nullptr, ws, ws_bytes, st, &out_len));
       const bool emit = null_sel == ARX_FILTER_EMIT_NULL && dm.null_count != 0;
       void* d_idx = nullptr;
       void* d_idx_valid = nullptr;
@@ -124,7 +124,9 @@
     const bool allocate_validity = dv.null_count != 0 || dm.null_count != 0;
     if (filter.length > 0 && filter.length <= g_filter_morsel_rows.load()) {
       const int64_t n = filter.length;
-      ARROW_RETURN_NOT_OK(FromArx(arx_filter_count_async(&dm, null_sel, ws, ws_bytes, st)));
+      volatile int64_t* sizes = nullptr;
+      ARROW_RETURN_NOT_OK(t_result.Get(&sizes));
+      ARROW_RETURN_NOT_OK(FromArx(arx_filter_size(nullptr, &dm, null_sel, ws, ws_bytes, const_cast<int64_t*>(sizes), st)));
       out_arr->buffers.resize(2);
       ARROW_ASSIGN_OR_RAISE(out_arr->buffers[1], AllocDevice(n * w));
       out_arr->buffers[0] = nullptr;
@@ -136,8 +138,7 @@
       ARROW_RETURN_NOT_OK(FromArx(arx_filter_exec(&dv, w, &dm, null_sel, ws, n,
                                                   reinterpret_cast<void*>(out_arr->buffers[1]->mutable_address()),
                                                   d_valid, st)));
-      int64_t selected = 0, set_bits = 0;
-      HIP_RETURN_NOT_OK(hipMemcpyAsync(&selected, ws, 8, hipMemcpyDeviceToHost, st));
+      int64_t set_bits = 0;
       if (allocate_validity) {
         void* cws = nullptr;
         ARROW_RETURN_NOT_OK(t_scratch.Get(kCounter, 64, &cws));
@@ -145,6 +146,7 @@
       } else {
         HIP_RETURN_NOT_OK(hipStreamSynchronize(st));
       }
+      const int64_t selected = sizes[0];
       out_arr->length = selected;
       out_arr->null_count = allocate_validity ? selected - set_bits : 0;
       static_cast<RocmBuffer*>(out_arr->buffers[1].get())->Shrink(selected * w);
@@ -153,11 +155,7 @@
       return Status::OK();
     }
     int64_t out_len = 0, out_nulls = 0;
-    if (allocate_validity) {
-      ARROW_RETURN_NOT_OK(FromArx(arx_filter_count_nulls(&dv, &dm, null_sel, ws, ws_bytes, &out_len, &out_nulls, st)));
-    } else {
-      ARROW_RETURN_NOT_OK(FromArx(arx_filter_count(&dm, null_sel, ws, ws_bytes, &out_len, st)));
-    }
+    ARROW_RETURN_NOT_OK(SizeSelection(dm, null_sel, allocate_validity ? &dv : nullptr, ws, ws_bytes, st, &out_len, &out_nulls));
     out_arr->length = out_len;
     out_arr->buffers.resize(2);
     ARROW_ASSIGN_OR_RAISE(out_arr->buffers[1], AllocDevice(out_len * w));
@@ -188,7 +186,7 @@
   void* ws = nullptr;
   ARROW_RETURN_NOT_OK(t_scratch.Get(kWs, ws_bytes, &ws));
   int64_t out_len = 0;
-  ARROW_RETURN_NOT_OK(FromArx(arx_filter_count(&dm, null_sel, ws, ws_bytes, &out_len, st)));
+  ARROW_RETURN_NOT_OK(SizeSelection(dm, null_sel, nullptr, ws, ws_bytes, st, &out_len));
 
   ArrayData* out_arr = out->array_data().get();
   const bool filter_null_count_is_zero = filter.null_count == 0;
@@ -320,12 +318,10 @@
   } else {
     ARROW_RETURN_NOT_OK(FromArx(arx_binary_take_data(&dv, m, ws, ws_bytes, static_cast<const int32_t*>(d_off), total, d_data, st)));
   }
-  int64_t valid_count = m;
-  if (allocate_validity) {
-    HIP_RETURN_NOT_OK(hipMemcpyAsync(&valid_count, d_counter, 8, hipMemcpyDeviceToHost, st));
-  }
+  volatile int64_t* valid_count = nullptr;
+  if (allocate_validity) ARROW_RETURN_NOT_OK(FetchTakeCounter(d_counter, st, &valid_count));
   HIP_RETURN_NOT_OK(hipStreamSynchronize(st));
-  out_arr->null_count = m - valid_count;
+  out_arr->null_count = allocate_validity ? m - *valid_count : 0;
   return Status::OK();
 }
 
@@ -382,7 +378,7 @@
   void* ws = nullptr;
   ARROW_RETURN_NOT_OK(t_scratch.Get(kWs, ws_bytes, &ws));
   int64_t out_len = 0;
-  ARROW_RETURN_NOT_OK(FromArx(arx_filter_count(&dm, null_sel, ws, ws_bytes, &out_len, st)));
+  ARROW_RETURN_NOT_OK(SizeSelection(dm, null_sel, nullptr, ws, ws_bytes, st, &out_len));
   const bool emit = null_sel == ARX_FILTER_EMIT_NULL && dm.null_count != 0;
   void* d_idx = nullptr;
   void* d_idx_valid = nullptr;
@@ -468,12 +464,10 @@
     ARROW_RETURN_NOT_OK(FromArx(arx_take(&dv, w, &di, tid,
                                          reinterpret_cast<void*>(out_arr->buffers[1]->mutable_address()), d_valid,
                                          static_cast<int64_t*>(d_counter), st)));
-    int64_t valid_count = m;
-    if (allocate_validity) {
-      HIP_RETURN_NOT_OK(hipMemcpyAsync(&valid_count, d_counter, 8, hipMemcpyDeviceToHost, st));
-    }
+    volatile int64_t* valid_count = nullptr;
+    if (allocate_validity) ARROW_RETURN_NOT_OK(FetchTakeCounter(d_counter, st, &valid_count));
     HIP_RETURN_NOT_OK(hipStreamSynchronize(st));
-    out_arr->null_count = m - valid_count;
+    out_arr->null_count = allocate_validity ? m - *valid_count : 0;
     CountGpu(kFnTake);
     return Status::OK();
   }
@@ -508,15 +502,15 @@
                                        static_cast<int64_t*>(d_counter), st)));
   HIP_RETURN_NOT_OK(hipMemcpyAsync(out_arr->buffers[1]->mutable_data(), d_out, static_cast<size_t>(m) * w,
                                    hipMemcpyDeviceToHost, st));
-  int64_t valid_count = m;
+  volatile int64_t* valid_count = nullptr;
   if (allocate_validity) {
     HIP_RETURN_NOT_OK(hipMemcpyAsync(out_arr->buffers[0]->mutable_data(), d_out_valid,
                                      static_cast<size_t>(arrow::bit_util::BytesForBits(m)),
                                      hipMemcpyDeviceToHost, st));
-    HIP_RETURN_NOT_OK(hipMemcpyAsync(&valid_count, d_counter, 8, hipMemcpyDeviceToHost, st));
+    ARROW_RETURN_NOT_OK(FetchTakeCounter(d_counter, st, &valid_count));
   }
   HIP_RETURN_NOT_OK(hipStreamSynchronize(st));
-  out_arr->null_count = m - valid_count;
+  out_arr->null_count = allocate_validity ? m - *valid_count : 0;
   CountGpu(kFnTake);
   return Status::OK();
 }
diff --git a/arrow_amd/csrc/plugin/selection_nested.inc b/arrow_amd/csrc/plugin/selection_nested.inc
--- a/arrow_amd/csrc/plugin/selection_nested.inc
+++ b/arrow_amd/csrc/plugin/selection_nested.inc
@@ -120,9 +120,10 @@
     ARROW_RETURN_NOT_OK(FromArx(arx_take_rows(&dv, row_bytes, &di, tid, reinterpret_cast<void*>(data->mutable_address()), d_valid,
                                               static_cast<int64_t*>(d_counter), st)));
   }
-  int64_t valid_count = m;
-  if (allocate_validity) HIP_RETURN_NOT_OK(hipMemcpyAsync(&valid_count, d_counter, 8, hipMemcpyDeviceToHost, st));
+  volatile int64_t* counted = nullptr;
+  if (allocate_validity) ARROW_RETURN_NOT_OK(FetchTakeCounter(d_counter, st, &counted));
   HIP_RETURN_NOT_OK(hipStreamSynchronize(st));
+  const int64_t valid_count = allocate_validity ? *counted : m;
   const auto& fsl = static_cast<const arrow::FixedSizeListType&>(*values.type);
   out_arr->length = m;
   out_arr->offset = 0;
@@ -185,9 +186,10 @@
   } else {
     ARROW_RETURN_NOT_OK(FromArx(arx_list_take_data(&dv, shift, m, ws, ws_bytes, static_cast<const int32_t*>(d_off), total, d_data, st)));
   }
-  int64_t valid_count = m;
-  if (allocate_validity) HIP_RETURN_NOT_OK(hipMemcpyAsync(&valid_count, d_counter, 8, hipMemcpyDeviceToHost, st));
+  volatile int64_t* counted = nullptr;
+  if (allocate_validity) ARROW_RETURN_NOT_OK(FetchTakeCounter(d_counter, st, &counted));
   HIP_RETURN_NOT_OK(hipStreamSynchronize(st));
+  const int64_t valid_count = allocate_validity ? *counted : m;
   out_arr->length = m;
   out_arr->offset = 0;
   out_arr->buffers = {valid_buf, off_buf};
@@ -244,7 +246,7 @@
   void* ws = nullptr;
   ARROW_RETURN_NOT_OK(t_scratch.Get(kWs, ws_bytes, &ws));
   int64_t out_len = 0;
-  ARROW_RETURN_NOT_OK(FromArx(arx_filter_count(&dm, null_sel, ws, ws_bytes, &out_len, st)));
+  ARROW_RETURN_NOT_OK(SizeSelection(dm, null_sel, nullptr, ws, ws_bytes, st, &out_len));
   const bool emit = null_sel == ARX_FILTER_EMIT_NULL && dm.null_count != 0;
   void* d_idx = nullptr;
   void* d_idx_valid = nullptr;
diff --git a/arrow_amd/csrc/plugin/vector_hash.inc b/arrow_amd/csrc/plugin/vector_hash.inc
--- a/arrow_amd/csrc/plugin/vector_hash.inc
+++ b/arrow_amd/csrc/plugin/vector_hash.inc
@@ -195,7 +195,7 @@
   void* ws = nullptr;
   ARROW_RETURN_NOT_OK(t_scratch.Get(kWs, ws_bytes, &ws));
   int64_t out_len = 0;
-  ARROW_RETURN_NOT_OK(FromArx(arx_filter_count(&dm, ARX_FILTER_DROP, ws, ws_bytes, &out_len, st)));
+  ARROW_RETURN_NOT_OK(SizeSelection(dm, ARX_FILTER_DROP, nullptr, ws, ws_bytes, st, &out_len));
   ARROW_ASSIGN_OR_RAISE(*out_values, AllocDevice(std::max<int64_t>(out_len, 1) * width));
   void* d_valid = nullptr;
   *out_validity = nullptr;
@@ -234,7 +234,7 @@
     void* ws = nullptr;
     ARROW_RETURN_NOT_OK(t_scratch.Get(kWs, ws_bytes, &ws));
     int64_t cnt = 0;
-    ARROW_RETURN_NOT_OK(FromArx(arx_filter_count(&dm, ARX_FILTER_DROP, ws, ws_bytes, &cnt, st)));
+    ARROW_RETURN_NOT_OK(SizeSelection(dm, ARX_FILTER_DROP, nullptr, ws, ws_bytes, st, &cnt));
     if (cnt != 1) return Status::Invalid("arrow_amd: internal error (", cnt, " null entries among the unique values)");
     ARROW_RETURN_NOT_OK(FromArx(arx_mask_to_indices(&dm, ARX_FILTER_DROP, ws, cnt, 4, d_idx, nullptr, st)));
     uint32_t pos = 0;
@@ -339,15 +339,15 @@
   void* ws = nullptr;
   ARROW_RETURN_NOT_OK(t_scratch.Get(kWs, ws_bytes, &ws));
   int64_t cnt = 0;
-  if (n > 0) ARROW_RETURN_NOT_OK(FromArx(arx_filter_count(&dm, ARX_FILTER_DROP, ws, ws_bytes, &cnt, st)));
-  void* d_idx = nullptr;
-  ARROW_RETURN_NOT_OK(t_scratch.Get(kArg2, static_cast<size_t>(cnt) * 4 + 64, &d_idx));
+  if (n > 0) ARROW_RETURN_NOT_OK(SizeSelection(dm, ARX_FILTER_DROP, nullptr, ws, ws_bytes, st, &cnt));
   ARROW_ASSIGN_OR_RAISE(auto out_values, AllocDevice(std::max<int64_t>(cnt, 1) * 8));
   bool direct = false;
   if (cnt > 0) {
     direct = arx_mask_to_indices(&dm, ARX_FILTER_DROP, ws, cnt, 8, reinterpret_cast<void*>(out_values->mutable_address()), nullptr, st) == ARX_OK;
   }
   if (cnt > 0 && !direct) {
+    void* d_idx = nullptr;
+    ARROW_RETURN_NOT_OK(t_scratch.Get(kArg2, static_cast<size_t>(cnt) * 4 + 64, &d_idx));
     ARROW_RETURN_NOT_OK(FromArx(arx_mask_to_indices(&dm, ARX_FILTER_DROP, ws, cnt, 4, d_idx, nullptr, st)));
     ArxSpan di{nullptr, d_idx, 0, cnt, 0};
     void* flag = nullptr;
diff --git a/arrow_amd/csrc/selection.hip b/arrow_amd/csrc/selection.hip
--- a/arrow_amd/csrc/selection.hip
+++ b/arrow_amd/csrc/selection.hip
@@ -56,34 +56,91 @@
   return m & mv;
 }
 
+constexpr int kCountPairs = 8;
+
+struct RawPair {
+  uint64_t w0, w1, w2;
+};
+__device__ __forceinline__ RawPair load_raw_pair(const Bits& b, int64_t w) {
+  RawPair r{~uint64_t(0), ~uint64_t(0), 0};
+  if (b.base != nullptr) {
+    const uint4 q = load16_unaligned(reinterpret_cast<const uint8_t*>(b.base + w));
+    r.w0 = (static_cast<uint64_t>(q.y) << 32) | q.x;
+    r.w1 = (static_cast<uint64_t>(q.w) << 32) | q.z;
+    if (b.shift != 0) r.w2 = b.base[w + 2];
+  }
+  return r;
+}
+__device__ __forceinline__ uint64_t funnel(uint64_t lo, uint64_t hi, int shift) {
+  return (lo >> shift) | ((hi << 1) << (63 - shift));
+}
+
 template <bool VALID>
 __global__ __launch_bounds__(kBlock) void count_kernel(Bits mask, Bits mvalid, Bits vvalid, int emit_null,
-                                                       int invert, int64_t ntiles,
-                                                       uint32_t* tile_counts,
+                                                       int invert, uint32_t* tile_counts,
                                                        int64_t* group_total, int64_t* group_valid) {
   __shared__ uint32_t wave_sums[kWavesPerBlock];
   __shared__ uint32_t wave_valid[kWavesPerBlock];
   const int lane = lane_id();
   const int wave = threadIdx.x >> 6;
   const int64_t group = blockIdx.x;
-  const int64_t t0 = group * kTilesPerGroup + wave * 16;
-  uint32_t mine = 0;
+  const int64_t t0 = group * kTilesPerGroup + wave * (2 * kCountPairs);
+  const int64_t w0 = t0 * 64 + 2 * lane;
+  uint64_t packed[2] = {0, 0};
   uint32_t kv = 0;
-#pragma unroll 4
-  for (int i = 0; i < 16; ++i) {
-    const int64_t t = t0 + i;
-    uint32_t k = 0;
-    if (t < ntiles) {
-      uint64_t mv;
-      const uint64_t e = emit_word(mask, mvalid, t * 64 + lane, emit_null != 0, invert != 0, &mv);
-      k = __popcll(e);
-      if constexpr (VALID) kv += __popcll(e & mv & load_word(vvalid, t * 64 + lane));
-    }
-    const uint32_t s = wave_reduce_sum_u32(k);
-    if (lane == i) mine = s;
-  }
-  if (lane < 16) tile_counts[t0 + lane] = mine;
-  const uint32_t wsum = wave_reduce_sum_u32(lane < 16 ? mine : 0u);
+  if ((t0 + 2 * kCountPairs) * kTileRows <= mask.length) {
+    RawPair rm[kCountPairs], rv[kCountPairs], rx[kCountPairs];
+#pragma unroll
+    for (int i = 0; i < kCountPairs; ++i) {
+      rm[i] = load_raw_pair(mask, w0 + 128 * i);
+      rv[i] = load_raw_pair(mvalid, w0 + 128 * i);
+      if constexpr (VALID) rx[i] = load_raw_pair(vvalid, w0 + 128 * i);
+    }
+#pragma unroll
+    for (int i = 0; i < kCountPairs; ++i) {
+      uint32_t k = 0;
+#pragma unroll
+      for (int h = 0; h < 2; ++h) {
+        uint64_t m = funnel(h == 0 ? rm[i].w0 : rm[i].w1, h == 0 ? rm[i].w1 : rm[i].w2, mask.shift);
+        const uint64_t mv = funnel(h == 0 ? rv[i].w0 : rv[i].w1, h == 0 ? rv[i].w1 : rv[i].w2, mvalid.shift);
+        if (invert) m = ~m;
+        const uint64_t e = emit_null ? (m | ~mv) : (m & mv);
+        k += __popcll(e);
+        if constexpr (VALID) {
+          const uint64_t vv = funnel(h == 0 ? rx[i].w0 : rx[i].w1, h == 0 ? rx[i].w1 : rx[i].w2, vvalid.shift);
+          kv += __popcll(e & mv & vv);
+        }
+      }
+      packed[i >> 2] += static_cast<uint64_t>(k) << (16 * (i & 3));
+    }
+  } else {
+#pragma unroll 1
+    for (int i = 0; i < kCountPairs; ++i) {
+      uint32_t k = 0;
+      for (int h = 0; h < 2; ++h) {
+        const int64_t w = w0 + 128 * i + h;
+        uint64_t mv;
+        const uint64_t e = emit_word(mask, mvalid, w, emit_null != 0, invert != 0, &mv);
+        k += __popcll(e);
+        if constexpr (VALID) kv += __popcll(e & mv & load_word(vvalid, w));
+      }
+      packed[i >> 2] += static_cast<uint64_t>(k) << (16 * (i & 3));
+    }
+  }
+#pragma unroll
+  for (int d = 16; d >= 1; d >>= 1) {
+    packed[0] += __shfl_xor(packed[0], d, 64);
+    packed[1] += __shfl_xor(packed[1], d, 64);
+  }
+  const int half = lane >> 5, sub = lane & 31;
+  uint32_t half_sum = 0;
+#pragma unroll
+  for (int i = 0; i < kCountPairs; ++i) {
+    const uint32_t c = static_cast<uint32_t>(packed[i >> 2] >> (16 * (i & 3))) & 0xFFFFu;
+    half_sum += c;
+    if (sub == i) tile_counts[t0 + 2 * i + half] = c;
+  }
+  const uint32_t wsum = half_sum + __shfl_xor(half_sum, 32, 64);
   if (lane == 0) wave_sums[wave] = wsum;
   if constexpr (VALID) {
     const uint32_t vsum = wave_reduce_sum_u32(kv);
@@ -103,7 +160,8 @@
 
 __global__ __launch_bounds__(1024) void scan_kernel(const int64_t* group_total, int64_t ngroups,
                                                     int64_t* group_excl, FilterWsHeader* hdr,
-                                                    const int64_t* group_valid = nullptr) {
+                                                    const int64_t* group_valid, int64_t ntiles, int64_t length,
+                                                    int64_t* result_slot) {
   __shared__ int64_t wave_tot[16];
   __shared__ int64_t carry_s;
   __shared__ unsigned long long valid_s;
@@ -141,8 +199,18 @@
     __syncthreads();
   }
   if (tid == 0) {
-    hdr->total = carry_s;
-    hdr->valid = static_cast<int64_t>(valid_s);
+    const int64_t total = carry_s;
+    const int64_t valid = static_cast<int64_t>(valid_s);
+    hdr->total = total;
+    hdr->ntiles = ntiles;
+    hdr->ngroups = ngroups;
+    hdr->length = length;
+    hdr->valid = valid;
+    hdr->pad[0] = hdr->pad[1] = hdr->pad[2] = 0;
+    if (result_slot != nullptr) {
+      result_slot[0] = total;
+      result_slot[1] = valid;
+    }
   }
 }
 
@@ -1051,7 +1119,8 @@
 }
 
 static int launch_count(const ArxSpan* mask, int null_selection, void* ws, size_t ws_bytes,
-                        hipStream_t st, int invert = 0, const ArxSpan* values = nullptr) {
+                        hipStream_t st, int invert = 0, const ArxSpan* values = nullptr,
+                        int64_t* result_slot = nullptr) {
   const int rc = check_mask(mask, null_selection);
   if (rc != ARX_OK) return rc;
   const size_t need = arx_filter_workspace_bytes(mask->length);
@@ -1066,28 +1135,26 @@
   FilterWsView v = ws_view(ws, mask->length);
   const int64_t nt = num_tiles(mask->length);
   const int64_t ng = num_groups(mask->length);
-  FilterWsHeader h{};
-  h.total = 0;
-  h.ntiles = nt;
-  h.ngroups = ng;
-  h.length = mask->length;
-  ARX_HIP(hipMemcpyAsync(v.hdr, &h, sizeof(h), hipMemcpyHostToDevice, st));
-  if (mask->length == 0) return ARX_OK;
+  if (mask->length == 0) {
+    ARX_HIP(hipMemsetAsync(v.hdr, 0, sizeof(FilterWsHeader), st));
+    if (result_slot != nullptr) ARX_HIP(hipMemsetAsync(result_slot, 0, 2 * sizeof(int64_t), st));
+    return ARX_OK;
+  }
   const Bits mb = make_bits(mask->data, mask->offset, mask->length);
   const Bits mvb = make_bits(effective_validity(mask), mask->offset, mask->length);
   if (values != nullptr) {
     const Bits vvb = make_bits(effective_validity(values), values->offset, mask->length);
     hipLaunchKernelGGL((count_kernel<true>), dim3(static_cast<unsigned>(ng)), dim3(kBlock), 0, st, mb, mvb, vvb,
-                       null_selection, invert, nt, v.tile_counts, v.group_total, v.group_valid);
+                       null_selection, invert, v.tile_counts, v.group_total, v.group_valid);
     ARX_CHECK_LAUNCH("count_kernel");
     hipLaunchKernelGGL(scan_kernel, dim3(1), dim3(1024), 0, st, v.group_total, ng, v.group_excl, v.hdr,
-                       static_cast<const int64_t*>(v.group_valid));
+                       static_cast<const int64_t*>(v.group_valid), nt, mask->length, result_slot);
   } else {
     hipLaunchKernelGGL((count_kernel<false>), dim3(static_cast<unsigned>(ng)), dim3(kBlock), 0, st, mb, mvb, mvb,
-                       null_selection, invert, nt, v.tile_counts, v.group_total, static_cast<int64_t*>(nullptr));
+                       null_selection, invert, v.tile_counts, v.group_total, static_cast<int64_t*>(nullptr));
     ARX_CHECK_LAUNCH("count_kernel");
     hipLaunchKernelGGL(scan_kernel, dim3(1), dim3(1024), 0, st, v.group_total, ng, v.group_excl, v.hdr,
-                       static_cast<const int64_t*>(nullptr));
+                       static_cast<const int64_t*>(nullptr), nt, mask->length, result_slot);
   }
   ARX_CHECK_LAUNCH("scan_kernel");
   return ARX_OK;
@@ -1275,6 +1342,20 @@
   return launch_count(mask, null_selection, ws, ws_bytes, as_stream(stream));
 }
 
+int arx_filter_size(const ArxSpan* values, const ArxSpan* mask, int null_selection, void* ws, size_t ws_bytes,
+                    int64_t* result_slot, void* stream) {
+  if (result_slot == nullptr || (reinterpret_cast<uint64_t>(result_slot) & 7) != 0) {
+    set_error("result_slot is NULL or not 8-byte aligned");
+    return ARX_INVALID;
+  }
+  if (values != nullptr && mask != nullptr && values->length != mask->length) {
+    set_error("filter values and mask differ in length (%lld vs %lld)", static_cast<long long>(values->length),
+              static_cast<long long>(mask->length));
+    return ARX_INVALID;
+  }
+  return launch_count(mask, null_selection, ws, ws_bytes, as_stream(stream), 0, values, result_slot);
+}
+
 int arx_filter_count_nulls(const ArxSpan* values, const ArxSpan* mask, int null_selection, void* ws, size_t ws_bytes,
                            int64_t* out_length, int64_t* out_null_count, void* stream) {
   if (out_length == nullptr || out_null_count == nullptr || values == nullptr) {
diff --git a/include/arrow_amd.h b/include/arrow_amd.h
--- a/include/arrow_amd.h
+++ b/include/arrow_amd.h
@@ -55,6 +55,9 @@
 
 int arx_filter_count_async(const ArxSpan* mask, int null_selection, void* ws,
                            size_t ws_bytes, void* stream);
+
+int arx_filter_size(const ArxSpan* values, const ArxSpan* mask, int null_selection, void* ws, size_t ws_bytes,
+                    int64_t* result_slot, void* stream);
 
 int arx_filter_exec(const ArxSpan* values, int byte_width, const ArxSpan* mask,
                     int null_selection, const void* ws, int64_t out_length, void* out_data,
```

New measurement: 297,200 Mrows/s, median of 6. +2.1%, better.
